# zzbuzzard/PATHS

Hardware: AMD Instinct MI355X
Metric: slides_per_sec_5level_K2048_D1024 (higher is better)
Workload: dtype f32 (products as 2 fp16 planes per operand = 22 bits, 3 fp16 MFMAs per block, fp32 accumulate); 1 GPU; 5-level PATHS recursion (forward, eval): K=2048 patches/level (level-0 grid 32x64, top_k 512, 10% background), D=1024 features, trans_dim 128 x 4 heads x 2 layers, LSTM ctx 256; 8 HBM-resident slides per GPU; slides_per_gpu=8, global_batch=8, levels=5, resident_batches_rotated=3, parallelism=slide-sharded x1 (no data-path collective)

## Files before the change

### include/paths_hip.h

```cpp
#ifndef PATHS_HIP_H
#define PATHS_HIP_H

#include <stddef.h>
#include <stdint.h>

#ifdef __cplusplus
extern "C" {
#endif

typedef void* paths_stream_t;

const char* paths_last_error(void);
const char* paths_build_info(void);
int paths_abi_version(void);

void* paths_event_create(void);
void* paths_stream_create_masked(const uint32_t* cu_mask, int words);
int paths_event_destroy(void* event);
int paths_stream_wait(paths_stream_t dst, paths_stream_t src, void* event);
int paths_set_stop_event(void* event);
int paths_flush_stop_event(paths_stream_t src);
int paths_stop_event_pending(void);
int paths_clear_stop_event(void);
int paths_record_event(void* event, paths_stream_t stream);
int paths_stream_wait_event(paths_stream_t dst, void* event);
int paths_memset_zero(void* p, size_t bytes, paths_stream_t stream);

int paths_lstm_cell(const float* x, int64_t ldx, const float* h0, int64_t ldh0, const float* c0, int64_t ldc0,
                    const float* w_gates, const float* b_gates, const float* w_mem, const float* b_mem,
                    float* state_out, int64_t ldso, float* y, int64_t ldy, float* ws_o, float* save_frm, float* save_tc,
                    const float* hp, const int* hp_row,
                    int M, int D, int Hc, const int64_t* num_ims, int rows_per_slide, int phases, paths_stream_t stream);

int paths_pe_table(const float* div_term, int pe_mode, int d, int rows, float* out, paths_stream_t stream);
int paths_importance_proj(const float* y, int64_t ldy, const float* w_ip, const float* b1, const float* w2, const float* b2 ,
                          const float* bp, const float* special, const float* div_term, const float* pe_table, int pe_rows,
                          const int64_t* locs,
                          const int64_t* num_ims, int rows_per_slide, int patch_size, int pe_mode, int imp_mul,
                          float* importance, float* tokens, float* save_hid, float* save_pproj, int M, int D, int Hi, int d,
                          int skip_padding, paths_stream_t stream);

int64_t paths_x6_packed_bytes(int Npad, int K, int planes);
int paths_x6_pack_weights(const float* w, int64_t ldw, void* out, int N, int Npad, int K, int planes, float w_scale,
                          paths_stream_t stream);
int paths_x6_pack_weights_t(const float* w, int64_t ldw, void* out, int N, int Npad, int K, int Kvalid, int planes, paths_stream_t stream);
int paths_lstm_cell_x6(const float* x, int64_t ldx, const int64_t* x_rows, const float* h0, int64_t ldh0, const float* c0, int64_t ldc0,
                       const void* w_gates_x6, const float* b_gates, const void* w_mem_x6, const float* b_mem,
                       float* state_out, int64_t ldso, float* y, int64_t ldy, float* ws_o, float* save_frm, float* save_tc,
                       const float* hp, const int* hp_row,
                       int M, int D, int Hc, const int64_t* num_ims, int rows_per_slide, int phases,
                       int planes, float wg_scale, float wm_scale, float a_scale, paths_stream_t stream);
int paths_lstm_cell_x6_h16(const float* x, int64_t ldx, const int64_t* x_rows, const float* h0, int64_t ldh0, const float* c0, int64_t ldc0,
                           const void* w_gates_x6, const float* b_gates, const void* w_mem_x6, const float* b_mem,
                           float* state_out, int64_t ldso, float* y, int64_t ldy, float* ws_o, float* save_frm, float* save_tc,
                           const float* hp, const int* hp_row,
                           int M, int D, int Hc, const int64_t* num_ims, int rows_per_slide, int phases,
                           int planes, float wg_scale, float wm_scale, float a_scale, paths_stream_t stream);
int paths_importance_proj_x6(const float* y, int64_t ldy, const int64_t* y_rows, const float* y_add, int64_t ldya, const void* w_ip_x6, const float* b1, const float* w2, const float* b2 ,
                             const float* bp, const float* special, const float* div_term, const float* pe_table, int pe_rows,
                             const int64_t* locs,
                             const int64_t* num_ims, int rows_per_slide, int patch_size, int pe_mode, int imp_mul,
                             float* importance, float* tokens, float* save_hid, float* save_pproj, int M, int D, int Hi, int d,
                             int skip_padding, int planes, float w_scale, float a_scale, float* splitk_ws, paths_stream_t stream);
int paths_importance_proj_x6_h16(const float* y, int64_t ldy, const int64_t* y_rows, const float* y_add, int64_t ldya, const void* w_ip_x6, const float* b1, const float* w2, const float* b2 ,
                                 const float* bp, const float* special, const float* div_term, const float* pe_table, int pe_rows,
                                 const int64_t* locs,
                                 const int64_t* num_ims, int rows_per_slide, int patch_size, int pe_mode, int imp_mul,
                                 float* importance, float* tokens, float* save_hid, float* save_pproj, int M, int D, int Hi, int d,
                                 int skip_padding, int planes, float w_scale, float a_scale, float* splitk_ws, paths_stream_t stream);
int64_t paths_importance_proj_x6_workspace(int M);
int paths_importance_qkv_x6(const float* y, int64_t ldy, const int64_t* y_rows, const float* y_add, int64_t ldya, const void* w_ip_x6,
                            const float* b1, const float* w2, const float* b2 , const float* bp, const float* special,
                            const float* pe_table, int pe_rows, const int64_t* locs, const int64_t* num_ims, int B, int N,
                            int patch_size, int pe_mode, int imp_mul, float* importance, float* tokens, int D, int skip_padding,
                            float w_scale, float a_scale, float* splitk_ws, const void* w_qkv, const float* bqkv, float s_wqkv,
                            float qscale, void* qkv_images, int phases, int alpha_from_importance, paths_stream_t stream);
int paths_importance_qkv_x6_h16(const float* y, int64_t ldy, const int64_t* y_rows, const float* y_add, int64_t ldya, const void* w_ip_x6,
                                const float* b1, const float* w2, const float* b2 , const float* bp, const float* special,
                                const float* pe_table, int pe_rows, const int64_t* locs, const int64_t* num_ims, int B, int N,
                                int patch_size, int pe_mode, int imp_mul, float* importance, float* tokens, int D, int skip_padding,
                                float w_scale, float a_scale, float* splitk_ws, const void* w_qkv, const float* bqkv, float s_wqkv,
                                float qscale, void* qkv_images, int phases, int alpha_from_importance, paths_stream_t stream);
int paths_gemm_nt_x6(const float* a, int64_t lda, const void* w_x6, int Kpacked, int k0, const float* b, float* out, int64_t ldo,
                     int M, int N, int Npad, int K, int act, const float* residual, int64_t ldr, const float* mask,
                     int64_t ldm, int accumulate, int planes, float w_scale, float a_scale, paths_stream_t stream);
int paths_gemm_add_nt_x6(const float* a, int64_t lda, const int64_t* a_rows, const float* a_add, int64_t ld_add, const void* w_x6, int Kpacked,
                         const float* b, float* out, int64_t ldo, int M, int N, int Npad, int K, int act, const int64_t* num_ims,
                         int rows_per_slide, float w_scale, float a_scale, paths_stream_t stream);
int paths_gemm_add_nt_x6_h16(const float* a, int64_t lda, const int64_t* a_rows, const float* a_add, int64_t ld_add, const void* w_x6, int Kpacked,
                             const float* b, float* out, int64_t ldo, int M, int N, int Npad, int K, int act, const int64_t* num_ims,
                             int rows_per_slide, float w_scale, float a_scale, paths_stream_t stream);
int paths_gemm_rows_nt_x6(const int64_t* a_rows, const void* w_x6, int Kpacked, int k0, float* out, int64_t ldo,
                          int M, int Npad, int K, int planes, float w_scale, float a_scale, paths_stream_t stream);

int paths_gemm_nt_f32(const float* a, int64_t lda, const float* w, int64_t ldw, const float* b, float* out, int64_t ldo,
                      int M, int N, int Npad, int K, int act, const float* residual, int64_t ldr, const float* mask,
                      int64_t ldm, int accumulate, paths_stream_t stream);
int64_t paths_gemm_tn_workspace(int N1, int N2, int splits);
int paths_gemm_tn_f32(const float* a, int64_t lda, const float* b0, int64_t ldb0, int nb0, const float* b1, int64_t ldb1,
                      float* out, int64_t ldo, int M, int N1, int N2, int splits, int accumulate, float* workspace,
                      paths_stream_t stream);
int paths_gemm_tn_x6(const float* a, int64_t lda, const float* b0, int64_t ldb0, int nb0, const float* b1, int64_t ldb1,
                     float* out, int64_t ldo, int M, int N1, int N2, int splits, int accumulate, float* workspace, int planes,
                     paths_stream_t stream);
int paths_colsum_f32(const float* a, int64_t lda, int M, int N, float* out, int splits, int accumulate, float* workspace,
                     paths_stream_t stream);
int paths_transpose_f32(const float* in, int64_t ldi, int R, int C, float* out, int64_t ldo, paths_stream_t stream);

int paths_adamw_chunk(void);
int paths_adamw_multi(const int64_t* table, const int64_t* numel, const int32_t* blocks, int nblocks, const float* step_size,
                      const float* bc2_sqrt, float wd_scale, int has_wd, float lerp_w, float beta2, float value, float eps, int flavor,
                      paths_stream_t stream);

int paths_lstm_bwd_a(const float* dh1, int64_t ldd, const float* dh1b, int64_t lddb, const float* o, const float* tc,
                     const int64_t* num_ims, int rows_per_slide, int64_t M, int D, float* dpre_o, int64_t ldo,
                     float* dpre_h, paths_stream_t stream);
int paths_lstm_bwd_b(const float* dc1_h, const float* dc1_ext, int64_t lde, const float* frm, const float* c0, int64_t ldc0,
                     const int64_t* num_ims, int rows_per_slide, int64_t M, int Hc, float* dg, int64_t ldg, float* dc0,
                     int64_t lddc0, paths_stream_t stream);
int paths_importance_bwd(const float* dtok, const float* pproj, const float* hid, const float* alpha, const float* w2,
                         const int64_t* num_ims, int rows_per_slide, int64_t M, int imp_mul, float* du, float* da, float* dah,
                         paths_stream_t stream);
int paths_layernorm_fwd_stats(const float* x, const float* add, const float* gamma, const float* beta, float* y, float* xhat,
                              float* rstd, int64_t rows, int d, float eps, paths_stream_t stream);
int paths_layernorm_bwd(const float* dy, const float* xhat, const float* rstd, const float* gamma, float* dx, float* dyxhat,
                        int64_t rows, int d, paths_stream_t stream);
int paths_layernorm_bwd_sums(const float* dy, const float* xhat, const float* rstd, const float* gamma, float* dx, float* slabs,
                             int64_t rows, int d, int rows_per_block, paths_stream_t stream);
int paths_reduce_slabs_f32(const float* slabs, int splits, int n, float* out, int accumulate, paths_stream_t stream);
int paths_defer_reductions(int on);
int paths_flush_reductions(int* n_entries, paths_stream_t stream);

int paths_attention_bwd_f32(const float* q, const float* k, const float* v, const float* o, const float* d_o, const float* lse,
                            const int64_t* num_ims, float* dqkv, float* ws_dsum, int B, int T, int H, int head_dim,
                            paths_stream_t stream);
int64_t paths_attention_token0_workspace(int B, int T, int H);
int paths_attention_token0_any(const float* qkv, int64_t ld, const int64_t* num_ims, float* a0, float* ws, int B, int T, int H, int head_dim,
                               float qscale, paths_stream_t stream);
int paths_attention_token0_fwd(const float* q, const float* k, const float* v, const int64_t* num_ims, float* a0, float* lse0, float* ws,
                               int B, int T, int H, int head_dim, uint64_t drop_key, float drop_p, paths_stream_t stream);
int paths_attention_token0_bwd(const float* q, const float* k, const float* v, const float* a0, const float* da0, const float* lse0,
                               const int64_t* num_ims, float* dqkv, float* ws, int B, int T, int H, int head_dim, uint64_t drop_key,
                               float drop_p, paths_stream_t stream);
int64_t paths_token0_attention_workspace(int B, int T, int d, int H);
int paths_token0_attention(const float* x, const int64_t* num_ims, const float* in_proj_weight, const float* in_proj_bias, float* attn_patch,
                           int64_t patch_ld, float* attn_self, int64_t self_ld, float* ws, int B, int T, int d, int H, int special_last,
                           paths_stream_t stream);
int64_t paths_attention_rollout_workspace(int B, int T, int d, int H);
int paths_attention_rollout_prepare(const float* x, const int64_t* num_ims, const float* in_proj_weight, const float* in_proj_bias, float* ws,
                                    int B, int T, int d, int H, int special_last, paths_stream_t stream);
int paths_attention_rollout_seed(const float* attn_patch, int64_t patch_ld, const float* attn_self, int64_t self_ld, const int64_t* num_ims,
                                 float* r, float* rollout, int64_t rollout_ld, float* rollout_self, int B, int T, int H, paths_stream_t stream);
int paths_attention_rollout_step(const float* ws, const int64_t* num_ims, const float* r_in, float* r_out, float* rollout, int64_t rollout_ld,
                                 float* rollout_self, int B, int T, int d, int H, paths_stream_t stream);

int paths_linear_f32(const float* a, int64_t lda, const float* w, const float* b, float* out, int64_t ldo,
                     int M, int N, int Npad, int K, int act, paths_stream_t stream);

int paths_attention_f32(const float* q, const float* k, const float* v, float* o, float* lse, const int64_t* num_ims,
                        int B, int T, int H, int head_dim, int max_queries, paths_stream_t stream);

int64_t paths_attention_x6_workspace(int B, int T, int H, int head_dim, int planes);
int paths_attention_x6(const float* q, const float* k, const float* v, float* o, float* lse, const int64_t* num_ims,
                       int B, int T, int H, int head_dim, int max_queries, void* workspace, int planes, int images_ready,
                       paths_stream_t stream);

int paths_token_layer_f32(const float* x_in, const float* attn, float* x_out,
                          const float* wo, const float* bo, const float* ln1g, const float* ln1b, const float* cab,
                          const float* ln2g, const float* ln2b, const float* w1, const float* b1, const float* w2,
                          const float* b2, const float* ln3g, const float* ln3b, const float* wqkv, const float* bqkv,
                          float* q, float* k, float* v, const int64_t* num_ims, int B, int T, int d, int H,
                          int do_post, int do_qkv, int skip_padding, float qscale, float eps, int max_tokens,
                          paths_stream_t stream);

int64_t paths_tlayer_h3_image_bytes(int part);
int paths_tlayer_pack_h3(int part, const float* wa, const float* wb, const float* wc, float s_a, float s_b, float s_c, void* out,
                         paths_stream_t stream);
int paths_token_layer_h3(const float* x_in, const float* attn, float* x_out, const void* w_post, const void* w_qkv,
                         const float* bo, const float* ln1g, const float* ln1b, const float* cab, const float* ln2g, const float* ln2b,
                         const float* b1, const float* b2, const float* ln3g, const float* ln3b, const float* bqkv,
                         float s_wo, float s_w1, float s_w2, float s_wqkv,
                         float* q, float* k, float* v, const int64_t* num_ims, int B, int T, int d, int H,
                         int do_post, int do_qkv, int skip_padding, float qscale, float eps, int max_tokens, void* qkv_images,
                         paths_stream_t stream);

int64_t paths_tlayer_ws_image_bytes(int part, int d);
int paths_tlayer_pack_ws(int part, const float* wa, const float* wb, const float* wc, float s_a, float s_b, float s_c, void* out, int d,
                         paths_stream_t stream);
int paths_token_layer_ws(const float* x_in, const float* attn, const void* attn_img, float* x_out, const void* w_post, const void* w_qkv,
                         const float* bo, const float* ln1g, const float* ln1b, const float* cab, const float* ln2g, const float* ln2b,
                         const float* b1, const float* b2, const float* ln3g, const float* ln3b, const float* bqkv,
                         float s_wo, float s_w1, float s_w2, float s_wqkv, void* qkv_images, const int64_t* num_ims,
                         int B, int T, int d, int H, int do_post, int do_qkv, int skip_padding, float qscale, float eps,
                         int* zero_words, int n_zero, paths_stream_t stream);
int paths_token_layer_ws_rows(const float* x_in, const float* attn, float* x_out, const void* w_post, const void* w_qkv,
                              const float* bo, const float* ln1g, const float* ln1b, const float* cab, const float* ln2g, const float* ln2b,
                              const float* b1, const float* b2, const float* ln3g, const float* ln3b, const float* bqkv,
                              float s_wo, float s_w1, float s_w2, float s_wqkv, float* qkv_rows, int64_t ld_qkv, const int64_t* num_ims,
                              int B, int T, int d, int do_post, int do_qkv, int skip_padding, float eps, paths_stream_t stream);
int paths_attention_h3_img(void* o_img, const int64_t* num_ims, int B, int T, int H, int head_dim, void* workspace, paths_stream_t stream);

int64_t paths_token0_ws_image_bytes(void);
int64_t paths_token0_ws_image_bytes_d(int d);
int64_t paths_token0_ws_partials(int B, int T);
int64_t paths_token0_ws_partials_d(int B, int T, int d);
int paths_token0_ws_supported(int B, int T, int d, int H);
int paths_token0_pack_ws(const float* wqkv, const float* bqkv, const float* wo, const float* bo, const float* w1, const float* w2, float qscale,
                         void* out, paths_stream_t stream);
int paths_token0_pack_ws_d(const float* wqkv, const float* bqkv, const float* wo, const float* bo, const float* w1, const float* w2, float qscale,
                           int d, void* out, paths_stream_t stream);
int paths_token0_tail_ws(const float* x1, const int64_t* num_ims, const void* img, const float* bv, const float* bo,
                         const float* ln1g, const float* ln1b, const float* cab, const float* ln2g, const float* ln2b,
                         const float* b1, const float* b2, const float* ln3g, const float* ln3b, const float* lnfg, const float* lnfb,
                         const float* ctx_prev, int64_t ctx_stride, const float* ctx_all, int ctx_depth,
                         const float* wcls, const float* bcls, int num_logits, int cls_in,
                         float* ctx_out, float* logits, float* partials, int* counters, int* status, int B, int T, int d, int H,
                         float eps, float eps_final, int special_last , paths_stream_t stream);

int paths_attention_any(const float* qkv, int64_t ld, float* o, const int64_t* num_ims, int B, int T, int H, int head_dim, float qscale,
                        int max_queries, paths_stream_t stream);
int64_t paths_attention_h3_any_workspace(int B, int T, int H, int head_dim);
int paths_attention_h3_any(const float* qkv, int64_t ld, float* o, const int64_t* num_ims, int B, int T, int H, int head_dim, float qscale,
                           void* workspace, paths_stream_t stream);
int paths_attention_h3_any_img(float* o, const int64_t* num_ims, int B, int T, int H, int head_dim, void* workspace, paths_stream_t stream);
int paths_layernorm_rows(const float* x, int64_t ldx, const float* add, const float* gamma, const float* beta, float* y, int64_t ldy,
                         int64_t rows, int d, float eps, paths_stream_t stream);
int paths_layernorm2_rows(const float* x, int64_t ldx, const float* g1, const float* b1, const float* add, const float* g2, const float* b2,
                          float* y, int64_t ldy, int64_t rows, int d, float eps, paths_stream_t stream);
int paths_importance_rows(const float* hid, int64_t ldh, const float* w2, const float* b2, const int64_t* num_ims, int rows_per_slide,
                          int64_t M, int Hi, float* importance, int relu , paths_stream_t stream);
int paths_tokens_assemble(const float* P, int64_t ldp, const float* importance, int imp_mul, const float* bp, const float* special,
                          const float* div_term, const int64_t* locs, int rows_per_slide, int patch_size, int pe_mode, int d, int B,
                          float* tokens, paths_stream_t stream);
int paths_importance_tokens_rows(const float* hid, int64_t ldh, const float* w2, const float* b2, const int64_t* num_ims, int rows_per_slide,
                                 int64_t M, int Hi, float* importance, int relu, int imp_mul, const float* bp, const float* special,
                                 const float* pe_table, int pe_rows, const int64_t* locs, int patch_size, int pe_mode, int d, float* tokens,
                                 paths_stream_t stream);
int paths_final_head_any(const float* x, int64_t slide_stride, const float* lng, const float* lnb, const float* ctx_prev, int64_t ctx_stride,
                         const float* ctx_all, int ctx_depth, const float* wcls, const float* bcls, int num_logits, int cls_in,
                         float* ctx_out, float* logits, int B, int d, float eps, paths_stream_t stream);

int paths_attention_any_train(const float* qkv, int64_t ld, float* o, float* lse, const int64_t* num_ims, int B, int T, int H, int head_dim,
                              float qscale, int max_queries, uint64_t drop_key, float drop_p, paths_stream_t stream);
int paths_attention_bwd_any(const float* qkv, int64_t ld, const float* o, const float* d_o, const float* lse, const int64_t* num_ims,
                            float* dqkv, float* ws_dsum, int B, int T, int H, int head_dim, float qscale, int max_queries,
                            uint64_t drop_key, float drop_p, paths_stream_t stream);
// ... 168 lines not shown
```

### paths_amd/_lib.py

```python
from __future__ import annotations

import ctypes as C
import os
from typing import Optional

import torch

_HERE = os.path.dirname(os.path.abspath(__file__))
LIB_PATH = os.environ.get("PATHS_HIP_LIB") or os.path.join(_HERE, "libpaths_hip.so")

_i64, _i32, _f32, _vp, _u32, _u64 = C.c_int64, C.c_int, C.c_float, C.c_void_p, C.c_uint32, C.c_uint64

SIGNATURES = {
    "paths_lstm_cell": [_vp, _i64, _vp, _i64, _vp, _i64, _vp, _vp, _vp, _vp, _vp, _i64, _vp, _i64, _vp, _vp, _vp, _vp, _vp,
                        _i32, _i32, _i32, _vp, _i32, _i32, _vp],
    "paths_pe_table": [_vp, _i32, _i32, _i32, _vp, _vp],
    "paths_importance_proj": [_vp, _i64, _vp, _vp, _vp, _vp, _vp, _vp, _vp, _vp, _i32, _vp, _vp, _i32, _i32, _i32, _i32,
                              _vp, _vp, _vp, _vp, _i32, _i32, _i32, _i32, _i32, _vp],
    "paths_gemm_nt_f32": [_vp, _i64, _vp, _i64, _vp, _vp, _i64, _i32, _i32, _i32, _i32, _i32, _vp, _i64, _vp, _i64, _i32, _vp],
    "paths_x6_pack_weights": [_vp, _i64, _vp, _i32, _i32, _i32, _i32, _f32, _vp],
    "paths_x6_pack_weights_t": [_vp, _i64, _vp, _i32, _i32, _i32, _i32, _i32, _vp],
    "paths_lstm_cell_x6": [_vp, _i64, _vp, _vp, _i64, _vp, _i64, _vp, _vp, _vp, _vp, _vp, _i64, _vp, _i64, _vp, _vp, _vp, _vp, _vp,
                           _i32, _i32, _i32, _vp, _i32, _i32, _i32, _f32, _f32, _f32, _vp],
    "paths_importance_proj_x6": [_vp, _i64, _vp, _vp, _i64, _vp, _vp, _vp, _vp, _vp, _vp, _vp, _vp, _i32, _vp, _vp, _i32, _i32, _i32, _i32,
                                 _vp, _vp, _vp, _vp, _i32, _i32, _i32, _i32, _i32, _i32, _f32, _f32, _vp, _vp],
    "paths_importance_qkv_x6": [_vp, _i64, _vp, _vp, _i64, _vp, _vp, _vp, _vp, _vp, _vp, _vp, _i32, _vp, _vp, _i32, _i32, _i32, _i32, _i32,
                                _vp, _vp, _i32, _i32, _f32, _f32, _vp, _vp, _vp, _f32, _f32, _vp, _i32, _i32, _vp],
    "paths_gemm_nt_x6": [_vp, _i64, _vp, _i32, _i32, _vp, _vp, _i64, _i32, _i32, _i32, _i32, _i32, _vp, _i64, _vp, _i64, _i32,
                         _i32, _f32, _f32, _vp],
    "paths_gemm_add_nt_x6": [_vp, _i64, _vp, _vp, _i64, _vp, _i32, _vp, _vp, _i64, _i32, _i32, _i32, _i32, _i32, _vp, _i32, _f32, _f32, _vp],
    "paths_gemm_tn_f32": [_vp, _i64, _vp, _i64, _i32, _vp, _i64, _vp, _i64, _i32, _i32, _i32, _i32, _i32, _vp, _vp],
    "paths_attention_fp8": [_vp, _vp, _vp, _vp, _vp, _i32, _i32, _i32, _i32, _vp, _vp],
    "paths_gemm_tn_x6": [_vp, _i64, _vp, _i64, _i32, _vp, _i64, _vp, _i64, _i32, _i32, _i32, _i32, _i32, _vp, _i32, _vp],
    "paths_colsum_f32": [_vp, _i64, _i32, _i32, _vp, _i32, _i32, _vp, _vp],
    "paths_transpose_f32": [_vp, _i64, _i32, _i32, _vp, _i64, _vp],
    "paths_attention_wide_fwd": [_vp, _i64, _vp, _vp, _vp, _i32, _i32, _i32, _i32, _f32, _i32, _u64, _f32, _vp, _vp],
    "paths_attention_wide_bwd": [_vp, _i64, _vp, _vp, _vp, _vp, _vp, _i32, _i32, _i32, _i32, _f32, _i32, _u64, _f32, _vp, _vp],
    "paths_sibling_sum": [_vp, _i64, _vp, _vp, _vp, _i64, _i64, _i32, _vp, _i64, _i64, _i32, _vp],
    "paths_scatter_kept_rows": [_vp, _i64, _i64, _vp, _vp, _vp, _i64, _i64, _i32, _i32, _vp],
    "paths_adamw_multi": [_vp, _vp, _vp, _i32, _vp, _vp, _f32, _i32, _f32, _f32, _f32, _f32, _i32, _vp],
    "paths_lstm_bwd_a": [_vp, _i64, _vp, _i64, _vp, _vp, _vp, _i32, _i64, _i32, _vp, _i64, _vp, _vp],
    "paths_lstm_bwd_b": [_vp, _vp, _i64, _vp, _vp, _i64, _vp, _i32, _i64, _i32, _vp, _i64, _vp, _i64, _vp],
    "paths_importance_bwd": [_vp, _vp, _vp, _vp, _vp, _vp, _i32, _i64, _i32, _vp, _vp, _vp, _vp],
    "paths_layernorm_fwd_stats": [_vp, _vp, _vp, _vp, _vp, _vp, _vp, _i64, _i32, _f32, _vp],
    "paths_attention_bwd_f32": [_vp, _vp, _vp, _vp, _vp, _vp, _vp, _vp, _vp, _i32, _i32, _i32, _i32, _vp],
    "paths_attention_token0_any": [_vp, _i64, _vp, _vp, _vp, _i32, _i32, _i32, _i32, _f32, _vp],
    "paths_attention_token0_fwd": [_vp, _vp, _vp, _vp, _vp, _vp, _vp, _i32, _i32, _i32, _i32, _u64, _f32, _vp],
    "paths_attention_token0_bwd": [_vp, _vp, _vp, _vp, _vp, _vp, _vp, _vp, _vp, _i32, _i32, _i32, _i32, _u64, _f32, _vp],
    "paths_token0_attention": [_vp, _vp, _vp, _vp, _vp, _i64, _vp, _i64, _vp, _i32, _i32, _i32, _i32, _i32, _vp],
    "paths_attention_rollout_prepare": [_vp, _vp, _vp, _vp, _vp, _i32, _i32, _i32, _i32, _i32, _vp],
    "paths_attention_rollout_seed": [_vp, _i64, _vp, _i64, _vp, _vp, _vp, _i64, _vp, _i32, _i32, _i32, _vp],
    "paths_attention_rollout_step": [_vp, _vp, _vp, _vp, _vp, _i64, _vp, _i32, _i32, _i32, _i32, _vp],
    "paths_layernorm_bwd": [_vp, _vp, _vp, _vp, _vp, _vp, _i64, _i32, _vp],
    "paths_layernorm_bwd_sums": [_vp, _vp, _vp, _vp, _vp, _vp, _i64, _i32, _i32, _vp],
    "paths_reduce_slabs_f32": [_vp, _i32, _i32, _vp, _i32, _vp],
    "paths_defer_reductions": [_i32],
    "paths_flush_reductions": [_vp, _vp],
    "paths_linear_f32": [_vp, _i64, _vp, _vp, _vp, _i64, _i32, _i32, _i32, _i32, _i32, _vp],
    "paths_attention_f32": [_vp, _vp, _vp, _vp, _vp, _vp, _i32, _i32, _i32, _i32, _i32, _vp],
    "paths_attention_x6": [_vp, _vp, _vp, _vp, _vp, _vp, _i32, _i32, _i32, _i32, _i32, _vp, _i32, _i32, _vp],
    "paths_tlayer_pack_h3": [_i32, _vp, _vp, _vp, _f32, _f32, _f32, _vp, _vp],
    "paths_token_layer_h3": [_vp] * 16 + [_f32, _f32, _f32, _f32, _vp, _vp, _vp, _vp, _i32, _i32, _i32, _i32, _i32, _i32, _i32, _f32, _f32, _i32, _vp, _vp],
    "paths_tlayer_pack_ws": [_i32, _vp, _vp, _vp, _f32, _f32, _f32, _vp, _i32, _vp],
    "paths_token_layer_ws": [_vp] * 17 + [_f32, _f32, _f32, _f32, _vp, _vp, _i32, _i32, _i32, _i32, _i32, _i32, _i32, _f32, _f32, _vp, _i32, _vp],
    "paths_token_layer_ws_rows": [_vp] * 16 + [_f32, _f32, _f32, _f32, _vp, _i64, _vp, _i32, _i32, _i32, _i32, _i32, _i32, _f32, _vp],
    "paths_token0_pack_ws": [_vp, _vp, _vp, _vp, _vp, _vp, _f32, _vp, _vp],
    "paths_token0_pack_ws_d": [_vp, _vp, _vp, _vp, _vp, _vp, _f32, _i32, _vp, _vp],
    "paths_token0_tail_ws": [_vp] * 16 + [_vp, _i64, _vp, _i32, _vp, _vp, _i32, _i32, _vp, _vp, _vp, _vp, _vp, _i32, _i32, _i32, _i32, _f32, _f32, _i32, _vp],
    "paths_attention_any": [_vp, _i64, _vp, _vp, _i32, _i32, _i32, _i32, _f32, _i32, _vp],
    "paths_attention_any_train": [_vp, _i64, _vp, _vp, _vp, _i32, _i32, _i32, _i32, _f32, _i32, _u64, _f32, _vp],
    "paths_layernorm_fwd_stats_any": [_vp, _vp, _vp, _vp, _vp, _vp, _vp, _i64, _i32, _f32, _vp],
    "paths_layernorm_bwd_any": [_vp, _vp, _vp, _vp, _vp, _vp, _i64, _i32, _vp],
    "paths_layernorm_bwd_sums_any": [_vp, _vp, _vp, _vp, _vp, _vp, _i64, _i32, _i32, _vp],
    "paths_importance_bwd_any": [_vp, _vp, _vp, _vp, _vp, _vp, _i32, _i64, _i32, _i32, _i32, _i64, _vp, _vp, _vp, _vp],
    "paths_importance_rows_bwd_any": [_vp, _vp, _i32, _vp, _vp, _vp, _vp, _i32, _i64, _i32, _vp, _vp, _vp, _vp],
    "paths_attention_bwd_any": [_vp, _i64, _vp, _vp, _vp, _vp, _vp, _vp, _i32, _i32, _i32, _i32, _f32, _i32, _u64, _f32, _vp],
    "paths_fp8_scale": [_vp, _i64, _i64, _i32, _vp, _vp, _vp, _i32, _vp],
    "paths_fp8_pack_weight": [_vp, _i64, _i32, _i32, _vp, _vp, _vp, _vp],
    "paths_fp8_quantize": [_vp, _i64, _i32, _i32, _vp, _vp, _vp],
    "paths_gemm_nt_fp8_out8": [_vp, _vp, _vp, _vp, _vp, _vp, _vp, _vp, _i32, _i32, _i32, _i32, _vp],
    "paths_gemm_nt_fp8": [_vp, _vp, _vp, _vp, _vp, _vp, _i64, _i32, _i32, _i32, _i32, _vp, _i64, _vp],
    "paths_attention_fp8_qkv": [_vp, _i64, _vp, _vp, _i32, _i32, _i32, _i32, _f32, _vp, _vp],
    "paths_attention_h3_any": [_vp, _i64, _vp, _vp, _i32, _i32, _i32, _i32, _f32, _vp, _vp],
    "paths_attention_h3_any_img": [_vp, _vp, _i32, _i32, _i32, _i32, _vp, _vp],
    "paths_layernorm_rows": [_vp, _i64, _vp, _vp, _vp, _vp, _i64, _i64, _i32, _f32, _vp],
    "paths_layernorm2_rows": [_vp, _i64, _vp, _vp, _vp, _vp, _vp, _vp, _i64, _i64, _i32, _f32, _vp],
    "paths_importance_rows": [_vp, _i64, _vp, _vp, _vp, _i32, _i64, _i32, _vp, _i32, _vp],
    "paths_importance_tokens_rows": [_vp, _i64, _vp, _vp, _vp, _i32, _i64, _i32, _vp, _i32, _i32, _vp, _vp, _vp, _i32, _vp, _i32, _i32, _i32, _vp, _vp],
    "paths_tokens_assemble": [_vp, _i64, _vp, _i32, _vp, _vp, _vp, _vp, _i32, _i32, _i32, _i32, _i32, _vp, _vp],
    "paths_final_head_any": [_vp, _i64, _vp, _vp, _vp, _i64, _vp, _i32, _vp, _vp, _i32, _i32, _vp, _vp, _i32, _i32, _f32, _vp],
    "paths_attention_h3_img": [_vp, _vp, _i32, _i32, _i32, _i32, _vp, _vp],
    "paths_token_layer_f32": [_vp] * 21 + [_vp, _i32, _i32, _i32, _i32, _i32, _i32, _i32, _f32, _f32, _i32, _vp],
    "paths_token0_tail": [_vp] * 20 + [_vp, _i64, _vp, _i32, _vp, _vp, _i32, _i32, _vp, _vp, _vp, _i32, _i32, _i32, _i32, _f32, _f32, _vp],
    "paths_final_head": [_vp, _i64, _vp, _vp, _vp, _i64, _vp, _i32, _vp, _vp, _i32, _i32, _vp, _vp, _i32, _i32, _f32, _vp],
    "paths_layernorm_f32": [_vp, _vp, _vp, _vp, _i64, _i32, _f32, _vp],
    "paths_topk": [_vp, _i64, _vp, _i32, _i32, _i32, _vp, _i64, _vp, _vp],
    "paths_topk_rows": [_vp, _i64, _vp, _i32, _i32, _i32, _vp, _i64, _vp, _vp, _i64, _i64, _vp, _vp, _vp],
    "paths_gemm_rows_nt_x6": [_vp, _vp, _i32, _i32, _vp, _i64, _i32, _i32, _i32, _i32, _f32, _f32, _vp],
    "paths_expand_children": [_vp, _i64, _vp, _vp, _i64, _i32, _vp, _vp, _vp, _i32, _i64, _vp, _vp, _vp, _vp, _vp, _vp, _vp, _vp, _vp],
    "paths_candidate_children": [_vp, _i64, _vp, _vp, _i64, _i32, _vp, _vp, _i32, _vp, _vp, _vp, _vp],
    "paths_admit_children": [_vp, _vp, _vp, _vp, _vp, _i64, _vp, _i32, _i32, _i64, _vp, _vp, _vp, _vp, _vp, _vp, _vp, _vp, _vp],
    "paths_gather_kept_rows": [_vp, _i64, _i64, _vp, _i64, _vp, _i32, _i32, _vp, _vp],
    "paths_gather_rows_bwd": [_vp, _i64, _vp, _vp, _vp, _i64, _i32, _vp, _i64, _i32, _vp],
    "paths_fallback_all_cells": [_vp, _vp, _vp, _i32, _i32, _i64, _vp, _vp, _vp, _vp, _vp, _vp, _vp, _vp],
    "paths_gather_rows": [_vp, _vp, _i32, _vp, _i64, _i64, _vp, _i32, _vp, _i32, _i64, _vp, _vp, _i32, _vp, _vp, _vp],
    "paths_level0_batch": [_vp, _vp, _vp, _i32, _i32, _i32, _i64, _vp, _vp, _vp, _vp, _i32, _vp, _vp, _vp],
    "paths_scale_add_rows": [_vp, _vp, _vp, _vp, _i32, _i32, _i64, _i32, _vp, _vp],
    "paths_importance_rows_bwd": [_vp, _vp, _i32, _vp, _vp, _vp, _vp, _i32, _i64, _vp, _vp, _vp, _vp],
    "paths_dropout_rows": [_vp, _i64, _vp, _vp, _i64, _vp, _i64, _i64, _i32, _u64, _f32, _vp],
    "paths_dropout_mask": [_vp, _i64, _u64, _f32, _vp],
    "paths_attention_x6_dropout": [_vp, _vp, _vp, _vp, _vp, _vp, _i32, _i32, _i32, _i32, _i32, _vp, _i32, _u64, _f32, _vp],
    "paths_attention_bwd_f32_dropout": [_vp, _vp, _vp, _vp, _vp, _vp, _vp, _vp, _vp, _i32, _i32, _i32, _i32, _u64, _f32, _vp],
    "paths_attention_bwd_x6_dropout": [_vp, _vp, _vp, _vp, _vp, _vp, _vp, _vp, _vp, _vp, _i32, _i32, _i32, _i32, _u64, _f32, _vp],
    "paths_attention_bwd_x6_planes": [_vp, _vp, _vp, _vp, _vp, _vp, _vp, _vp, _vp, _vp, _i32, _i32, _i32, _i32, _u64, _f32, _i32, _vp],
    "paths_stream_wait": [_vp, _vp, _vp],
    "paths_set_stop_event": [_vp],
    "paths_flush_stop_event": [_vp],
    "paths_stream_wait_event": [_vp, _vp],
    "paths_record_event": [_vp, _vp],
    "paths_event_destroy": [_vp],
    "paths_memset_zero": [_vp, C.c_size_t, _vp],
    "paths_tissue_mask": [_vp, _i64, _i32, _vp, _vp],
    "paths_tissue_mask_absmax": [_vp, _i64, _i32, _vp, _vp, _vp],
    "paths_synth_grid": [_vp, _i32, _i32, _i32, _u32, _i32, _u64, _vp],
    "paths_stage_rows": [_vp, _i64, _i32, _vp, _vp, _vp],
    "paths_saliency_rows": [_vp, _i64, _vp, _i64, _vp, _i32, _i32, _i32, _vp, _vp, _vp],
    "paths_path_points": [_vp, _i64, _vp, _vp, _vp, _vp, _vp, _i32, _i32, _i32, _i32, _vp, _vp],
    "paths_path_accumulate": [_vp, _i64, _vp, _i64, _vp, _vp, _vp, _i32, _i32, _i32, _i32, _i32, _vp, _vp, _vp, _vp],
    "paths_rank_joint": [_vp, _vp, _vp, _vp, _i32, _i32, _i32, _i32, _vp, _vp, _vp],
    "paths_path_mask_points": [_vp, _i64, _vp, _vp, _i64, _vp, _vp, _vp, _i32, _i32, _i32, _i32, _vp, _vp],
    "paths_removal_masks": [_vp, _vp, _vp, _i64, _vp, _i32, _vp, _vp, _i64, _vp, _i32, _i32, _i32, _i32, _vp, _i64, _vp, _vp],
    "paths_visited_overlap": [_vp, _i64, _vp, _vp, _vp, _vp, _i32, _i32, _i32, _i32, _vp, _vp],
    "paths_level0_mask_rows": [_vp, _vp, _vp, _i32, _i32, _i64, _vp, _vp, _vp, _vp],
}
for _n in ("paths_lstm_cell_x6", "paths_importance_proj_x6", "paths_importance_qkv_x6", "paths_gemm_add_nt_x6", "paths_gather_rows",
           "paths_level0_batch", "paths_tissue_mask_absmax", "paths_synth_grid"):
    SIGNATURES[_n + "_h16"] = SIGNATURES[_n]
_PLAIN = {"paths_gemm_tn_workspace": (C.c_int64, [_i32, _i32, _i32]), "paths_x6_packed_bytes": (C.c_int64, [_i32, _i32, _i32]), "paths_tlayer_h3_image_bytes": (C.c_int64, [_i32]), "paths_tlayer_ws_image_bytes": (C.c_int64, [_i32, _i32]), "paths_token0_ws_image_bytes": (C.c_int64, []), "paths_token0_ws_partials": (C.c_int64, [_i32, _i32]), "paths_token0_ws_image_bytes_d": (C.c_int64, [_i32]), "paths_token0_ws_partials_d": (C.c_int64, [_i32, _i32, _i32]), "paths_token0_ws_supported": (_i32, [_i32, _i32, _i32, _i32]), "paths_attention_x6_workspace": (C.c_int64, [_i32, _i32, _i32, _i32, _i32]), "paths_attention_fp8_workspace": (C.c_int64, [_i32, _i32, _i32, _i32]), "paths_attention_bwd_x6_workspace": (C.c_int64, [_i32, _i32, _i32, _i32]), "paths_attention_token0_workspace": (C.c_int64, [_i32, _i32, _i32]), "paths_token0_attention_workspace": (C.c_int64, [_i32, _i32, _i32, _i32]), "paths_attention_rollout_workspace": (C.c_int64, [_i32, _i32, _i32, _i32]), "paths_attention_h3_any_workspace": (C.c_int64, [_i32, _i32, _i32, _i32]), "paths_importance_proj_x6_workspace": (C.c_int64, [_i32]), "paths_last_error": (C.c_char_p, []), "paths_build_info": (C.c_char_p, []), "paths_abi_version": (_i32, []), "paths_stop_event_pending": (_i32, []), "paths_clear_stop_event": (_i32, []), "paths_adamw_chunk": (_i32, []), "paths_rank_joint_tile": (_i32, []), "paths_attention_wide_workspace": (C.c_int64, [_i32, _i32]), "paths_event_create": (_vp, []), "paths_stream_create_masked": (_vp, [_vp, _i32])}

ABI_VERSION = 3
_lib: Optional[C.CDLL] = None


class PathsHipError(RuntimeError):
    pass


def load() -> C.CDLL:
    global _lib
    if _lib is None:
        if not os.path.isfile(LIB_PATH):
            raise PathsHipError(f"{LIB_PATH} not found: the HIP extension is not built (run __graft_entry__.build()); "
                                "paths_amd has no CPU fallback")
        lib = C.CDLL(LIB_PATH)
        lib.paths_abi_version.restype = _i32
        if lib.paths_abi_version() != ABI_VERSION:
            raise PathsHipError(f"{LIB_PATH} has ABI version {lib.paths_abi_version()}, this binding needs {ABI_VERSION}: rebuild it "
                                "(__graft_entry__.build())")
        for name, args in SIGNATURES.items():
            fn = getattr(lib, name)
            fn.argtypes, fn.restype = args, _i32
        for name, (res, args) in _PLAIN.items():
            fn = getattr(lib, name)
            fn.argtypes, fn.restype = args, res
        _lib = lib
    return _lib


def ptr(t):
    if t is None or type(t) is int:
        return t
    return t.data_ptr()


_RAW_STREAM = getattr(torch._C, "_cuda_getCurrentRawStream", None)
_GET_DEVICE = getattr(torch._C, "_cuda_getDevice", None)


def stream() -> int:
    if _RAW_STREAM is not None and _GET_DEVICE is not None:
        return _RAW_STREAM(_GET_DEVICE())
    return torch.cuda.current_stream().cuda_stream


TAPE = None
TAPE_EVENTS = None


def call(name: str, *args):
    lib = load()
    fn = getattr(lib, name)
    rc = fn(*args)
    if rc != 0:
        raise PathsHipError(f"{name} failed ({rc}): {lib.paths_last_error().decode()}")
    if TAPE is not None:
        TAPE.append((fn, args, name))
        fb = fork_behind.active
        if fb is not None and fb.taken_at is None and name != "paths_set_stop_event" and not lib.paths_stop_event_pending():
            fb.taken_at = len(TAPE) - 1


def stream_wait(dst: "torch.cuda.Stream", src: "torch.cuda.Stream"):
    dst.wait_stream(src)
    if TAPE is not None:
        lib = load()
        pool = TAPE_EVENTS if TAPE_EVENTS is not None else [[], 0]
        if pool[1] == len(pool[0]):
            ev = lib.paths_event_create()
            if not ev:
                raise PathsHipError("paths_event_create failed")
            pool[0].append(ev)
        ev = pool[0][pool[1]]
        pool[1] += 1
        TAPE.append((lib.paths_stream_wait, (dst.cuda_stream, src.cuda_stream, ev), "paths_stream_wait"))


STOP_EVENTS = __import__("os").environ.get("PATHS_STOP_EVENTS", "1") != "0"


_TAPE_PLUMBING = {"paths_set_stop_event", "paths_flush_stop_event", "paths_stream_wait_event", "paths_stream_wait", "paths_record_event",
                  "paths_clear_stop_event"}


class fork_behind:

    active = None

    def __init__(self, dsts, src):
        self.dsts, self.src = list(dsts), src
        self.ev = None
        self.taken_at = None

    def __enter__(self):
        if TAPE is not None and STOP_EVENTS:
            lib = load()
            pool = TAPE_EVENTS if TAPE_EVENTS is not None else [[], 0]
            if pool[1] == len(pool[0]):
                e = lib.paths_event_create()
                if not e:
                    raise PathsHipError("paths_event_create failed")
                pool[0].append(e)
            self.ev = pool[0][pool[1]]
            pool[1] += 1
            call("paths_set_stop_event", self.ev)
            self.prev, fork_behind.active = fork_behind.active, self
        return self

    def __exit__(self, et, ev, tb):
        if self.ev is not None:
            fork_behind.active = self.prev
            if et is not None:
                load().paths_clear_stop_event()
                return False
            call("paths_flush_stop_event", self.src.cuda_stream)
            if self.taken_at is not None and any(nm not in _TAPE_PLUMBING for _, _, nm in TAPE[self.taken_at + 1:]):
                call("paths_record_event", self.ev, self.src.cuda_stream)
            for d in self.dsts:
                call("paths_stream_wait_event", d.cuda_stream, self.ev)
        elif et is None:
            for d in self.dsts:
                stream_wait(d, self.src)
        return False


def zeros(shape, **kw) -> torch.Tensor:
    t = torch.zeros(shape, **kw)
    if TAPE is not None:
        TAPE.append((load().paths_memset_zero, (t.data_ptr(), t.numel() * t.element_size(), stream()), "paths_memset_zero"))
    return t


def require_cuda(*tensors: torch.Tensor):
    for t in tensors:
        if t is not None and not t.is_cuda:
            raise PathsHipError("paths_amd runs on the GPU only: got a CPU tensor (no CPU fallback)")


def float_from_bits(bits: int) -> float:
    import struct
    bits &= 0xFFFFFFFF
    return float("inf") if bits >= 0x7F800000 else struct.unpack("<f", struct.pack("<I", bits))[0]


def absmax(t: torch.Tensor) -> float:
    require_cuda(t)
    assert t.dtype == torch.float32 and t.is_contiguous() and t.numel() % 4 == 0
    bits = torch.zeros((1,), dtype=torch.int32, device=t.device)
    D = t.shape[-1] if (t.dim() > 1 and t.shape[-1] % 4 == 0) else 4
# ... 3 lines not shown
```

### paths_amd/csrc/gemm_epi.h

```cpp
#pragma once
#include "common.h"

namespace paths_epi {



struct TileView {
  char* base; int64_t ldb; uint32_t lane_off;
  __device__ TileView(const float* p, int64_t ld, int lane)
      : base(reinterpret_cast<char*>(const_cast<float*>(p))), ldb(ld * 4), lane_off((uint32_t)((4 * (lane >> 5)) * ld + (lane & 31)) * 4u) {}
  __device__ float* at(int trow, int tcol, int r) const {
    char* tile = base + (int64_t)trow * ldb + (int64_t)tcol * 4;
    const uint32_t off = lane_off + (uint32_t)((r & 3) + 8 * (r >> 2)) * (uint32_t)ldb;
    return reinterpret_cast<float*>(tile + off);
  }
  __device__ char* tile(int trow, int tcol) const { return base + (int64_t)trow * ldb + (int64_t)tcol * 4; }
  __device__ float* elem(char* tile_origin, int r) const {
    return reinterpret_cast<float*>(tile_origin + (lane_off + (uint32_t)((r & 3) + 8 * (r >> 2)) * (uint32_t)ldb));
  }
  __device__ float* at_clamped(int trow, int tcol, int r, int lane, int M) const {
    const int row = min(trow + c32_row(r, lane), M - 1);
    return reinterpret_cast<float*>(base + (int64_t)row * ldb + (int64_t)(tcol + (lane & 31)) * 4);
  }
};
template <bool FULL>
__device__ __forceinline__ float* tile_elem(const TileView& v, int trow, int tcol, int r, int lane, int M) {
  if constexpr (FULL) return v.at(trow, tcol, r);
  else return v.at_clamped(trow, tcol, r, lane, M);
}
template <bool FULL>
__device__ __forceinline__ float* tile_elem_o(const TileView& v, char* origin, int trow, int tcol, int r, int lane, int M) {
  if constexpr (FULL) return v.elem(origin, r);
  else return v.at_clamped(trow, tcol, r, lane, M);
}
template <bool FULL>
__device__ __forceinline__ bool tile_row_ok(int trow, int r, int lane, int M) {
  if constexpr (FULL) return true;
  else return trow + c32_row(r, lane) < M;
}

struct EpiLstmC {
  const float* bias;
  const float* c0; int64_t ldc0;
  float* c1; int64_t ldc1;
  float* frm; int64_t ldfrm;
  const float* hp; int64_t ldhp; const int* hp_row;
  float acc_scale = 1.0f;
  template <int WTM, int WTN>
  __device__ __forceinline__ void init(f32x16 (&acc)[WTM][WTN], int row0, int col0, int lane, int M) const {
    const int jj = lane & 31;
    const float seed = 1.0f / acc_scale;
    if (hp == nullptr) {
#pragma unroll
      for (int i = 0; i < WTM; ++i)
#pragma unroll
        for (int r = 0; r < 16; ++r) { acc[i][0][r] = 0.f; acc[i][1][r] = 0.f; acc[i][2][r] = 0.f; }
      return;
    }
    int pr[WTM][16];
#pragma unroll
    for (int i = 0; i < WTM; ++i)
#pragma unroll
      for (int r = 0; r < 16; ++r) pr[i][r] = hp_row[min(row0 + 32 * i + c32_row(r, lane), M - 1)];
    float t[2][3][16];
    auto issue = [&](auto ic) __attribute__((always_inline)) {
      constexpr int i = decltype(ic)::value;
#pragma unroll
      for (int r = 0; r < 16; ++r) {
        const float* ph = hp + (int64_t)max(pr[i][r], 0) * ldhp + col0 + jj;
        t[i & 1][0][r] = ph[0]; t[i & 1][1][r] = ph[32]; t[i & 1][2][r] = ph[64];
      }
    };
    issue(std::integral_constant<int, 0>{});
    static_for<0, WTM>([&](auto ic) __attribute__((always_inline)) {
      constexpr int i = decltype(ic)::value;
      __builtin_amdgcn_sched_barrier(0);
      if constexpr (i + 1 < WTM) issue(std::integral_constant<int, i + 1>{});
      __builtin_amdgcn_sched_barrier(0);
#pragma unroll
      for (int r = 0; r < 16; ++r) {
        const bool has = pr[i][r] >= 0;
        acc[i][0][r] = has ? t[i & 1][0][r] * seed : 0.f; acc[i][1][r] = has ? t[i & 1][1][r] * seed : 0.f; acc[i][2][r] = has ? t[i & 1][2][r] * seed : 0.f;
      }
    });
    __builtin_amdgcn_sched_barrier(0);
  }
  template <bool FULL, bool WITH_FRM, int WTM, int WTN>
  __device__ __forceinline__ void run_impl(f32x16 (&acc)[WTM][WTN], int row0, int col0, int lane, int M) const {
    const int jj = lane & 31;
    const int tcol = (col0 / 96) * 32;
    const float bf = bias[col0 + jj], br = bias[col0 + 32 + jj], bm = bias[col0 + 64 + jj];
    const TileView c0v(c0, ldc0, lane), c1v(c1, ldc1, lane), fv(frm, ldfrm, lane);
    static_for<0, WTM>([&](auto ic) __attribute__((always_inline)) {
      constexpr int i = decltype(ic)::value;
      const int trow = row0 + 32 * i;
      char* o0 = c0v.tile(trow, tcol); char* o1 = c1v.tile(trow, tcol); char* of = fv.tile(trow, col0);
      float cp[16];
#pragma unroll
      for (int r = 0; r < 16; ++r) cp[r] = c0 ? *tile_elem_o<FULL>(c0v, o0, trow, tcol, r, lane, M) : 0.f;
#pragma unroll
      for (int r = 0; r < 16; ++r) {
        const float f = sigmoid_acc(fmaf(acc[i][0][r], acc_scale, bf));
        const float rg = sigmoid_acc(fmaf(acc[i][1][r], acc_scale, br));
        const float mp = tanh_acc(fmaf(acc[i][2][r], acc_scale, bm));
        const float v = cp[r] * f + rg * mp;
        if (tile_row_ok<FULL>(trow, r, lane, M)) {
          *tile_elem_o<FULL>(c1v, o1, trow, tcol, r, lane, M) = v;
          if constexpr (WITH_FRM) {
            float* fr = tile_elem_o<FULL>(fv, of, trow, col0, r, lane, M);
            fr[0] = f; fr[32] = rg; fr[64] = mp;
          }
        }
      }
      __builtin_amdgcn_sched_barrier(0);
    });
  }
  template <int WTM, int WTN, int WGM, int WGN>
  __device__ __forceinline__ void run(f32x16 (&acc)[WTM][WTN], int row0, int col0, int lane, int, int, int M, float*) const {
    static_assert(WTN == 3, "LSTM c epilogue wants f|r|m tiles");
    const bool full = row0 + 32 * WTM <= M;
    if (frm == nullptr) {
      if (full) run_impl<true, false>(acc, row0, col0, lane, M);
      else run_impl<false, false>(acc, row0, col0, lane, M);
    } else {
      if (full) run_impl<true, true>(acc, row0, col0, lane, M);
      else run_impl<false, true>(acc, row0, col0, lane, M);
    }
  }
};

template <bool RAW>
struct EpiLstmO_ {
  const float* bias; float* o; int64_t ldo; int N;
  const float* hp; int64_t ldhp; const int* hp_row; int hp_col0;
  float acc_scale = 1.0f;
  template <int WTM, int WTN>
  __device__ __forceinline__ void init(f32x16 (&acc)[WTM][WTN], int row0, int col0, int lane, int M) const {
    const float seed = 1.0f / acc_scale;
    if (hp == nullptr) {
#pragma unroll
      for (int i = 0; i < WTM; ++i)
#pragma unroll
        for (int j = 0; j < WTN; ++j)
#pragma unroll
          for (int r = 0; r < 16; ++r) acc[i][j][r] = 0.f;
      return;
    }
    int pr[WTM][16];
#pragma unroll
    for (int i = 0; i < WTM; ++i)
#pragma unroll
      for (int r = 0; r < 16; ++r) pr[i][r] = hp_row[min(row0 + 32 * i + c32_row(r, lane), M - 1)];
    float t[2][WTN][16];
    auto issue = [&](auto ic) __attribute__((always_inline)) {
      constexpr int i = decltype(ic)::value;
#pragma unroll
      for (int r = 0; r < 16; ++r) {
        const float* ph = hp + (int64_t)max(pr[i][r], 0) * ldhp + hp_col0 + (lane & 31);
#pragma unroll
        for (int j = 0; j < WTN; ++j) t[i & 1][j][r] = ph[min(col0 + 32 * j, N - 32)];
      }
    };
    issue(std::integral_constant<int, 0>{});
    static_for<0, WTM>([&](auto ic) __attribute__((always_inline)) {
      constexpr int i = decltype(ic)::value;
      __builtin_amdgcn_sched_barrier(0);
      if constexpr (i + 1 < WTM) issue(std::integral_constant<int, i + 1>{});
      __builtin_amdgcn_sched_barrier(0);
#pragma unroll
      for (int r = 0; r < 16; ++r)
#pragma unroll
        for (int j = 0; j < WTN; ++j) acc[i][j][r] = pr[i][r] >= 0 ? t[i & 1][j][r] * seed : 0.f;
    });
    __builtin_amdgcn_sched_barrier(0);
  }
  template <bool FULL, int WTM, int WTN>
  __device__ __forceinline__ void run_impl(f32x16 (&acc)[WTM][WTN], int row0, int col0, int lane, int M) const {
    const TileView ov(o, ldo, lane);
    static_for<0, WTM * WTN>([&](auto tc) __attribute__((always_inline)) {
      constexpr int t = decltype(tc)::value, i = t % WTM, j = t / WTM;
      const int trow = row0 + 32 * i, tcol = col0 + 32 * j;
      if (tcol < N) {
        const float b = bias[tcol + (lane & 31)];
        char* origin = ov.tile(trow, tcol);
#pragma unroll
        for (int r = 0; r < 16; ++r) {
          const float v = sigmoid_acc(fmaf(acc[i][j][r], acc_scale, b));
          if (tile_row_ok<FULL>(trow, r, lane, M)) *tile_elem_o<FULL>(ov, origin, trow, tcol, r, lane, M) = v;
        }
      }
    });
  }
  template <int WTM, int WTN, int WGM, int WGN>
  __device__ __forceinline__ void run(f32x16 (&acc)[WTM][WTN], int row0, int col0, int lane, int, int, int M, float*) const {
    if constexpr (RAW) {
      const int ntn = N >> 5;
#pragma unroll
      for (int j = 0; j < WTN; ++j) {
        const int tcol = col0 + 32 * j;
        if (tcol < N) {
          const float b = bias[tcol + (lane & 31)];
#pragma unroll
          for (int i = 0; i < WTM; ++i) {
            f32x4* t = reinterpret_cast<f32x4*>(o + ((int64_t)((row0 >> 5) + i) * ntn + (tcol >> 5)) * 1024) + lane;
#pragma unroll
            for (int q = 0; q < 4; ++q)
              t[64 * q] = f32x4{fmaf(acc[i][j][4 * q], acc_scale, b), fmaf(acc[i][j][4 * q + 1], acc_scale, b),
                                fmaf(acc[i][j][4 * q + 2], acc_scale, b), fmaf(acc[i][j][4 * q + 3], acc_scale, b)};
          }
        }
      }
    } else {
      if (row0 + 32 * WTM <= M) run_impl<true>(acc, row0, col0, lane, M);
      else run_impl<false>(acc, row0, col0, lane, M);
    }
  }
};
typedef EpiLstmO_<false> EpiLstmO;
typedef EpiLstmO_<true> EpiLstmORaw;

template <bool WITH_Y, bool WITH_TC = false, bool RAW_O = false>
struct EpiLstmH {
  template <int WTM, int WTN>
  __device__ __forceinline__ void init(f32x16 (&acc)[WTM][WTN], int, int, int, int) const {
#pragma unroll
    for (int i = 0; i < WTM; ++i)
#pragma unroll
      for (int j = 0; j < WTN; ++j)
#pragma unroll
        for (int r = 0; r < 16; ++r) acc[i][j][r] = 0.f;
  }

  const float* bias; const float* o; int64_t ldo; const float* x; int64_t ldx;
  float* h1; int64_t ldh; float* y; int64_t ldy; int N;
  float* tc_out;
  float acc_scale = 1.0f;
  template <bool FULL, int WTM, int WTN>
  __device__ __forceinline__ void run_impl(f32x16 (&acc)[WTM][WTN], int row0, int col0, int lane, int M) const {
    constexpr int NT = WTM * WTN, PD = (NT >= 4 && !WITH_Y) ? 3 : 1, NB = PD + 1;
    const TileView ovw(o, ldo, lane), xvw(x, ldx, lane), hv(h1, ldh, lane), yv(y, ldy, lane), tv(tc_out, N, lane);
    float ov[NB][16], xv[WITH_Y ? NB : 1][16];
    auto load = [&](auto tc) __attribute__((always_inline)) {
      constexpr int t = decltype(tc)::value, i = t % WTM, j = t / WTM, s = t % NB;
      const int trow = row0 + 32 * i, tcol = min(col0 + 32 * j, N - 32);
      char* to = ovw.tile(trow, tcol); char* tx = xvw.tile(trow, tcol);
      if constexpr (RAW_O) {
        const f32x4* t4 = reinterpret_cast<const f32x4*>(o + ((int64_t)(trow >> 5) * (N >> 5) + (tcol >> 5)) * 1024) + lane;
#pragma unroll
        for (int q = 0; q < 4; ++q) {
          const f32x4 v = t4[64 * q];
          ov[s][4 * q] = v[0]; ov[s][4 * q + 1] = v[1]; ov[s][4 * q + 2] = v[2]; ov[s][4 * q + 3] = v[3];
        }
      }
      static_for<0, 16>([&](auto rc) __attribute__((always_inline)) {
        constexpr int r = decltype(rc)::value;
        if constexpr (FULL) {
          if constexpr (!RAW_O) ov[s][r] = *ovw.elem(to, r);
          if constexpr (WITH_Y) xv[s][r] = *xvw.elem(tx, r);
        } else {
          if constexpr (!RAW_O) ov[s][r] = *ovw.at_clamped(trow, tcol, r, lane, M);
          if constexpr (WITH_Y) xv[s][r] = *xvw.at_clamped(trow, tcol, r, lane, M);
        }
      });
    };
    static_for<0, (PD < NT ? PD : NT)>([&](auto tc) __attribute__((always_inline)) { load(tc); });
    static_for<0, NT>([&](auto tc) __attribute__((always_inline)) {
      constexpr int t = decltype(tc)::value, i = t % WTM, j = t / WTM, s = t % NB;
      if constexpr (t + PD < NT) load(std::integral_constant<int, t + PD>{});
      const int trow = row0 + 32 * i, tcol = col0 + 32 * j;
      if (tcol < N) {
        const float b = bias[tcol + (lane & 31)];
        char* th = hv.tile(trow, tcol); char* ty = yv.tile(trow, tcol); char* tt = tv.tile(trow, tcol);
        static_for<0, 16>([&](auto rc) __attribute__((always_inline)) {
          constexpr int r = decltype(rc)::value;
          const float tcv = tanh_acc(fmaf(acc[i][j][r], acc_scale, b));
          const float h = (RAW_O ? sigmoid_acc(ov[s][r]) : ov[s][r]) * tcv;
          if constexpr (FULL) {
            if constexpr (WITH_TC) *tv.elem(tt, r) = tcv;
            *hv.elem(th, r) = h;
            if constexpr (WITH_Y) *yv.elem(ty, r) = xv[s][r] + h;
          } else if (tile_row_ok<false>(trow, r, lane, M)) {
            if constexpr (WITH_TC) *tv.at_clamped(trow, tcol, r, lane, M) = tcv;
            *hv.at_clamped(trow, tcol, r, lane, M) = h;
            if constexpr (WITH_Y) *yv.at_clamped(trow, tcol, r, lane, M) = xv[s][r] + h;
          }
        });
      }
      __builtin_amdgcn_sched_barrier(0);
    });
  }
  template <int WTM, int WTN, int WGM, int WGN>
  __device__ __forceinline__ void run(f32x16 (&acc)[WTM][WTN], int row0, int col0, int lane, int, int, int M, float*) const {
    if (row0 + 32 * WTM <= M) run_impl<true>(acc, row0, col0, lane, M);
    else run_impl<false>(acc, row0, col0, lane, M);
  }
};

struct EpiBias {
// ... 240 lines not shown
```

### paths_amd/csrc/gemm_x6.hip

```cpp
#include "common.h"
#include "gemm_epi.h"
#include "finish_qkv.h"
#include "split.h"

#ifndef PATHS_X6_PART
#define PATHS_X6_PART 0
#endif

namespace {
using namespace paths_epi;

constexpr int FRAG = 1024;
template <int NP> constexpr int planes_of() { return NP == 4 ? 2 : NP; }
template <int NP> constexpr int subt() { return planes_of<NP>() * FRAG; }

struct X6Operands {
  const float* A0; int64_t lda0; int K0;
  const int64_t* A0rows;
  const float* A1; int64_t lda1; int K1;
  const float* Aadd; int64_t ldadd;
  const char* Wt;
  int64_t w_group_stride;
  int M;
  const int64_t* num_ims;
// ... 341 lines not shown
  const int64_t i = blockIdx.x * (int64_t)blockDim.x + threadIdx.x;
  if (i >= (int64_t)Npad * (K >> 3)) return;
  const int n = (int)(i % Npad), k0 = (int)(i / Npad) * 8;
  uint16_t h[8], m[8], l[8];
#pragma unroll
  for (int j = 0; j < 8; ++j) {
    const int k = k0 + j;
    const float v = (n < N && k < Kvalid) ? w[(int64_t)k * ldw + n] : 0.f;
    const __bf16 hh = (__bf16)v; const float r1 = v - (float)hh;
    const __bf16 mm = (__bf16)r1; const float r2 = r1 - (float)mm;
    const __bf16 ll = (__bf16)r2;
    h[j] = __builtin_bit_cast(uint16_t, hh); m[j] = __builtin_bit_cast(uint16_t, mm); l[j] = __builtin_bit_cast(uint16_t, ll);
  }
  uint16_t* o = out + ((int64_t)(n >> 5) * (K >> 4) + (k0 >> 4)) * (subt<NP>() / 2) + ((k0 >> 3) & 1) * 256 + (n & 31) * 8;
  typedef uint16_t u16x8 __attribute__((ext_vector_type(8)));
  *reinterpret_cast<u16x8*>(o) = u16x8{h[0], h[1], h[2], h[3], h[4], h[5], h[6], h[7]};
  *reinterpret_cast<u16x8*>(o + FRAG / 2) = u16x8{m[0], m[1], m[2], m[3], m[4], m[5], m[6], m[7]};
  if constexpr (NP == 3) *reinterpret_cast<u16x8*>(o + FRAG) = u16x8{l[0], l[1], l[2], l[3], l[4], l[5], l[6], l[7]};
}

template <int NP, int WTM, int WTN, int PF, bool ADD, bool ROWS, class Epi, int OCC = 1, bool A16 = false>
int launch_x6_np(const X6Operands& g, int Npad, const Epi& epi, hipStream_t stream, const char* name) {
  constexpr int BM = WTM * 64, BN = WTN * 64;
  constexpr size_t lds = 2ull * (2 * WTM * ((A16 && !ADD) ? FRAG : subt<NP>()) + 2 * WTN * subt<NP>());
  const int K = g.K0 + g.K1;
  PATHS_REQUIRE(g.M > 0, "%s: M must be > 0", name);
  PATHS_REQUIRE(g.K0 > 0 && g.K0 % 16 == 0 && g.K1 % 16 == 0 && K % 32 == 0 && K >= 128, "%s: K panels (%d,%d): multiples of 16, total a multiple of 32, >= 128", name, g.K0, g.K1);
  PATHS_REQUIRE(Npad % BN == 0, "%s: packed N (%d) must be a multiple of %d", name, Npad, BN);
  PATHS_REQUIRE(g.lda0 % 4 == 0 && g.lda1 % 4 == 0, "%s: leading dims must be multiples of 4 floats", name);
  PATHS_REQUIRE(((uintptr_t)g.A0 % 16 == 0) && ((uintptr_t)g.A1 % 16 == 0) && ((uintptr_t)g.Wt % 16 == 0), "%s: operands must be 16-byte aligned", name);
  PATHS_REQUIRE(ROWS == (g.A0rows != nullptr) && (!ROWS || g.K1 == 0), "%s: row-pointer form is single-panel", name);
  PATHS_REQUIRE((int64_t)g.M * (g.lda0 > g.lda1 ? (g.lda0 > g.ldadd ? g.lda0 : g.ldadd) : (g.lda1 > g.ldadd ? g.lda1 : g.ldadd)) * 4 < (int64_t)1 << 32, "%s: A panel larger than 4 GiB", name);
  auto kern = gemm_x6_kernel<NP, WTM, WTN, PF, ADD, ROWS, Epi, OCC, A16>;
  PATHS_LDS_OPT_IN(kern, lds, name);
  PATHS_REQUIRE(g.ksplit == 1 || (g.ksplit > 1 && g.K1 == 0 && g.K0 % (32 * g.ksplit) == 0 && g.K0 / g.ksplit >= 128), "%s: split-K needs a single panel and k windows that are multiples of 32, >= 128", name);
  dim3 grid(Npad / BN, (g.M + BM - 1) / BM, g.ksplit);
  hipLaunchKernelGGL(kern, grid, dim3(256), lds, stream, g, epi);
  PATHS_LAUNCH_CHECK(name);
  return PATHS_OK;
}

struct EpiRaw {
  float* ws; int64_t zstride; int ntn;
  template <int WTM, int WTN>
  __device__ __forceinline__ void init(f32x16 (&acc)[WTM][WTN], int, int, int, int) const {
#pragma unroll
    for (int i = 0; i < WTM; ++i)
#pragma unroll
      for (int j = 0; j < WTN; ++j)
#pragma unroll
        for (int r = 0; r < 16; ++r) acc[i][j][r] = 0.f;
  }
  template <int WTM, int WTN, int WGM, int WGN>
  __device__ __forceinline__ void run(f32x16 (&acc)[WTM][WTN], int row0, int col0, int lane, int, int, int, float*) const {
    float* base = ws + (int64_t)blockIdx.z * zstride;
#pragma unroll
    for (int i = 0; i < WTM; ++i)
#pragma unroll
      for (int j = 0; j < WTN; ++j) {
        f32x4* t = reinterpret_cast<f32x4*>(base + ((int64_t)((row0 >> 5) + i) * ntn + (col0 >> 5) + j) * 1024) + lane;
#pragma unroll
        for (int q = 0; q < 4; ++q) {
          const f32x4 v = f32x4{acc[i][j][4 * q], acc[i][j][4 * q + 1], acc[i][j][4 * q + 2], acc[i][j][4 * q + 3]};
          t[64 * q] = v;
        }
      }
  }
};

template <int NZ, class Epi>
__global__ void __launch_bounds__(256)
x6_finish_kernel(const float* __restrict__ ws, int64_t zstride, int ntn, int M, const int64_t* __restrict__ num_ims, int rows_per_slide, Epi epi) {
  extern __shared__ __attribute__((aligned(16))) char smem[];
  const int tid = threadIdx.x, lane = tid & 63, wave = __builtin_amdgcn_readfirstlane(tid >> 6), wm = wave >> 1, wn = wave & 1;
  const int m0 = blockIdx.x * 64;
  if (block_all_padding(num_ims, rows_per_slide, m0, 64, M)) return;
  const int row0 = m0 + wm * 32, col0 = wn * 128;
  f32x16 acc[1][4];
#pragma unroll
  for (int j = 0; j < 4; ++j) {
    const f32x4* t = reinterpret_cast<const f32x4*>(ws + ((int64_t)(row0 >> 5) * ntn + (col0 >> 5) + j) * 1024) + lane;
#pragma unroll
    for (int q = 0; q < 4; ++q) {
      f32x4 v = t[64 * q];
#pragma unroll
      for (int z = 1; z < NZ; ++z) v += *reinterpret_cast<const f32x4*>(reinterpret_cast<const float*>(t + 64 * q) + z * zstride);
      acc[0][j][4 * q] = v[0]; acc[0][j][4 * q + 1] = v[1]; acc[0][j][4 * q + 2] = v[2]; acc[0][j][4 * q + 3] = v[3];
    }
  }
  epi.template run<1, 4, 2, 2>(acc, row0, col0, lane, wm, wn, M, reinterpret_cast<float*>(smem));
}

template <int WTM, int WTN, int PF, bool ADD, class Epi>
int launch_x6(int planes, const X6Operands& g, int Npad, const Epi& epi, hipStream_t stream, const char* name) {
  if (g.A0rows != nullptr) {
    if (planes == 2) return launch_x6_np<2, WTM, WTN, PF, ADD, true>(g, Npad, epi, stream, name);
    return paths_set_error(PATHS_EUNSUPPORTED, "%s: row pointers need planes = 2", name);
  }
  if constexpr (std::is_same<Epi, EpiBias>::value && !ADD) {
    if (planes == 4) return launch_x6_np<4, WTM, WTN, PF, ADD, false>(g, Npad, epi, stream, name);
  }
  if (planes == 3) return launch_x6_np<3, WTM, WTN, PF, ADD, false>(g, Npad, epi, stream, name);
  if (planes == 2) return launch_x6_np<2, WTM, WTN, PF, ADD, false>(g, Npad, epi, stream, name);
  return paths_set_error(PATHS_EINVAL, "%s: planes must be 3 (bf16 x6) or 2 (fp16 x3), got %d", name, planes);
}

constexpr int H_OCC = 3;
constexpr int H_TRAIN_OCC = 2;

inline int plane_count(int planes) { return planes == 4 ? 2 : planes; }
inline int64_t group_stride(int planes, int Kpacked) { return (int64_t)(Kpacked / 16) * plane_count(planes) * FRAG; }
inline bool pow2(float x) { int e; return x > 0.f && frexpf(x, &e) == 0.5f; }
inline bool h16_scale_ok(float a_scale) { return pow2(a_scale) && a_scale >= 1.0f && a_scale <= 32768.0f; }

}

extern "C" {

#if PATHS_X6_PART == 0 || PATHS_X6_PART == 1
int64_t paths_x6_packed_bytes(int Npad, int K, int planes) { return (int64_t)Npad * K * 2 * plane_count(planes); }

int paths_x6_pack_weights(const float* w, int64_t ldw, void* out, int N, int Npad, int K, int planes, float w_scale, hipStream_t stream) {
  PATHS_REQUIRE(N > 0 && Npad >= N && Npad % 32 == 0 && K % 16 == 0, "x6_pack_weights: bad shape N=%d Npad=%d K=%d", N, Npad, K);
  PATHS_REQUIRE((uintptr_t)out % 16 == 0, "x6_pack_weights: out must be 16-byte aligned");
  PATHS_REQUIRE(((planes == 3 || planes == 4) && w_scale == 1.0f) || (planes == 2 && pow2(w_scale)), "x6_pack_weights: planes 3 / 4 (bf16) with w_scale 1, or planes 2 with a power-of-two w_scale");
  const int64_t n = (int64_t)Npad * K;
  const dim3 grid((unsigned)((n + 255) / 256));
  if (planes == 4) hipLaunchKernelGGL(x6_pack_kernel<4>, grid, dim3(256), 0, stream, w, ldw, reinterpret_cast<uint16_t*>(out), N, Npad, K, 1.0f);
  else if (planes == 3) hipLaunchKernelGGL(x6_pack_kernel<3>, grid, dim3(256), 0, stream, w, ldw, reinterpret_cast<uint16_t*>(out), N, Npad, K, 1.0f);
  else hipLaunchKernelGGL(x6_pack_kernel<2>, grid, dim3(256), 0, stream, w, ldw, reinterpret_cast<uint16_t*>(out), N, Npad, K, w_scale);
  PATHS_LAUNCH_CHECK("x6_pack_weights");
  return PATHS_OK;
}

int paths_x6_pack_weights_t(const float* w, int64_t ldw, void* out, int N, int Npad, int K, int Kvalid, int planes, hipStream_t stream) {
  PATHS_REQUIRE(N > 0 && Npad >= N && Npad % 32 == 0 && K % 16 == 0 && Kvalid > 0 && Kvalid <= K, "x6_pack_weights_t: bad shape N=%d Npad=%d K=%d Kvalid=%d", N, Npad, K, Kvalid);
  PATHS_REQUIRE(w != nullptr && out != nullptr && (uintptr_t)out % 16 == 0, "x6_pack_weights_t: null / unaligned operand");
  PATHS_REQUIRE(planes == 3 || planes == 4, "x6_pack_weights_t: planes 3 or 4 (bf16)");
  const int64_t n = (int64_t)Npad * (K / 8);
  const dim3 grid((unsigned)((n + 255) / 256));
  if (planes == 4) hipLaunchKernelGGL(x6_pack_t_kernel<4>, grid, dim3(256), 0, stream, w, ldw, reinterpret_cast<uint16_t*>(out), N, Npad, K, Kvalid);
  else hipLaunchKernelGGL(x6_pack_t_kernel<3>, grid, dim3(256), 0, stream, w, ldw, reinterpret_cast<uint16_t*>(out), N, Npad, K, Kvalid);
  PATHS_LAUNCH_CHECK("x6_pack_weights_t");
  return PATHS_OK;
}

}
namespace {
template <bool A16>
int lstm_cell_x6(const float* x, int64_t ldx, const int64_t* x_rows, const float* h0, int64_t ldh0, const float* c0, int64_t ldc0,
                 const void* w_gates_x6, const float* b_gates, const void* w_mem_x6, const float* b_mem,
                 float* state_out, int64_t ldso, float* y, int64_t ldy, float* ws_o, float* save_frm, float* save_tc,
                 const float* hp, const int* hp_row, int M, int D, int Hc, const int64_t* num_ims, int rows_per_slide,
                 int phases, int planes, float wg_scale, float wm_scale, float a_scale, hipStream_t stream) {
  PATHS_REQUIRE(D % 256 == 0 && Hc % 64 == 0, "lstm_cell_x6: D (%d) must be a multiple of 256 and Hc (%d) of 64", D, Hc);
  if constexpr (A16) {
    PATHS_REQUIRE(x_rows != nullptr && x == nullptr && planes == 2, "lstm_cell_x6_h16: fp16 rows are given as x_rows (planes = 2)");
    PATHS_REQUIRE(h16_scale_ok(a_scale), "lstm_cell_x6_h16: a_scale must be a power of two in [1, 2^15]");
  }
  PATHS_REQUIRE(hp != nullptr || (h0 == nullptr) == (c0 == nullptr), "lstm_cell_x6: h0 and c0 must both be given or both be null");
  PATHS_REQUIRE((hp == nullptr) == (hp_row == nullptr) && (hp == nullptr || h0 == nullptr),
                "lstm_cell_x6: hp/hp_row come together and replace h0 (the h half of the gate GEMM was done per parent)");
  PATHS_REQUIRE(planes == 3 || (pow2(wg_scale) && pow2(wm_scale) && pow2(a_scale)), "lstm_cell_x6: scales must be powers of two");
  PATHS_REQUIRE(x_rows == nullptr || (h0 == nullptr && y == nullptr && save_tc == nullptr), "lstm_cell_x6: x_rows (rows addressed in place) excludes h0, y and the training saves");
  if (planes == 3) wg_scale = wm_scale = a_scale = 1.0f;
  const char* wg = reinterpret_cast<const char*>(w_gates_x6);
  const int64_t gs = group_stride(planes, 2 * D);
  const float sg = 1.0f / (wg_scale * a_scale), sm = 1.0f / (wm_scale * a_scale);
  X6Operands g{x, ldx, D, x_rows, h0, h0 ? ldh0 : 0, h0 ? D : 0, nullptr, 0, wg, gs, M, num_ims, rows_per_slide, a_scale};
  const bool small_m = planes == 2 && M <= 8192 && (h0 == nullptr);
  if (phases & 1) {
    EpiLstmC e{b_gates, c0, ldc0, state_out + D, ldso, save_frm, (int64_t)3 * Hc, hp, (int64_t)3 * Hc + D, hp_row, sg};
    int rc;
    if constexpr (A16) {
      rc = small_m ? launch_x6_np<2, 2, 3, 2, false, true, decltype(e), 1, true>(g, 3 * Hc, e, stream, "lstm_cell_x6_h16(c, 128-row tiles)")
                   : launch_x6_np<2, 4, 3, 1, false, true, decltype(e), 1, true>(g, 3 * Hc, e, stream, "lstm_cell_x6_h16(c)");
    } else if (small_m) rc = x_rows ? launch_x6_np<2, 2, 3, 2, false, true>(g, 3 * Hc, e, stream, "lstm_cell_x6(c, 128-row tiles)")
                             : launch_x6_np<2, 2, 3, 2, false, false>(g, 3 * Hc, e, stream, "lstm_cell_x6(c, 128-row tiles)");
    else rc = launch_x6<4, 3, 1, false>(planes, g, 3 * Hc, e, stream, "lstm_cell_x6(c)");
    if (rc) return rc;
  }
  const bool o_raw = y == nullptr && save_tc == nullptr && save_frm == nullptr;
  if (phases & 2) {
    X6Operands go = g;
    go.Wt = wg + (int64_t)(3 * Hc / 32) * gs;
    int rc;
    if (o_raw) {
      EpiLstmORaw e{b_gates + 3 * Hc, ws_o, D, D, hp, (int64_t)3 * Hc + D, hp_row, 3 * Hc, sg};
      if constexpr (A16) {
        rc = small_m ? launch_x6_np<2, 2, 4, 2, false, true, decltype(e), 1, true>(go, D, e, stream, "lstm_cell_x6_h16(o, raw, 128-row tiles)")
                     : launch_x6_np<2, 4, 4, 1, false, true, decltype(e), 1, true>(go, D, e, stream, "lstm_cell_x6_h16(o, raw)");
      } else if (small_m) rc = x_rows ? launch_x6_np<2, 2, 4, 2, false, true>(go, D, e, stream, "lstm_cell_x6(o, raw, 128-row tiles)")
                               : launch_x6_np<2, 2, 4, 2, false, false>(go, D, e, stream, "lstm_cell_x6(o, raw, 128-row tiles)");
      else rc = launch_x6<4, 4, 1, false>(planes, go, D, e, stream, "lstm_cell_x6(o, raw)");
    } else {
      EpiLstmO e{b_gates + 3 * Hc, ws_o, D, D, hp, (int64_t)3 * Hc + D, hp_row, 3 * Hc, sg};
      if constexpr (A16) rc = launch_x6_np<2, 4, 4, 1, false, true, decltype(e), 1, true>(go, D, e, stream, "lstm_cell_x6_h16(o)");
      else rc = launch_x6<4, 4, 1, false>(planes, go, D, e, stream, "lstm_cell_x6(o)");
    }
    if (rc) return rc;
  }
  if (phases & 4) {
    X6Operands gh{state_out + D, ldso, Hc, nullptr, nullptr, 0, 0, nullptr, 0, reinterpret_cast<const char*>(w_mem_x6), group_stride(planes, Hc), M, num_ims, rows_per_slide, a_scale};
    int rc;
    PATHS_REQUIRE(save_tc == nullptr || y != nullptr, "lstm_cell_x6: save_tc (training) needs y");
    PATHS_REQUIRE(planes == 2 || planes == 3, "lstm_cell_x6: planes must be 3 (bf16 x6) or 2 (fp16 x3), got %d", planes);
    if (save_tc != nullptr) {
      EpiLstmH<true, true> e{b_mem, ws_o, D, x, ldx, state_out, ldso, y, ldy, D, save_tc, sm};
      if (planes == 2) rc = launch_x6_np<2, 2, 2, 2, false, false, decltype(e), H_TRAIN_OCC>(gh, D, e, stream, "lstm_cell_x6(h, save, 128x128)");
      else rc = launch_x6_np<3, 4, 4, 1, false, false>(gh, D, e, stream, "lstm_cell_x6(h, save)");
    } else if (y != nullptr) {
      EpiLstmH<true, false> e{b_mem, ws_o, D, x, ldx, state_out, ldso, y, ldy, D, nullptr, sm};
      rc = launch_x6<4, 4, 1, false>(planes, gh, D, e, stream, "lstm_cell_x6(h)");
    } else if (o_raw) {
      EpiLstmH<false, false, true> e{b_mem, ws_o, D, x, ldx, state_out, ldso, nullptr, 0, D, nullptr, sm};
      if (planes == 2) rc = launch_x6_np<2, 2, 2, 2, false, false, decltype(e), H_OCC>(gh, D, e, stream, "lstm_cell_x6(h, raw o, 128x128)");
      else rc = launch_x6_np<3, 4, 4, 1, false, false>(gh, D, e, stream, "lstm_cell_x6(h, raw o)");
    } else {
      EpiLstmH<false, false> e{b_mem, ws_o, D, x, ldx, state_out, ldso, nullptr, 0, D, nullptr, sm};
      if (planes == 2) rc = launch_x6_np<2, 2, 2, 2, false, false, decltype(e), H_OCC>(gh, D, e, stream, "lstm_cell_x6(h, no y, 128x128)");
      else rc = launch_x6_np<3, 4, 4, 1, false, false>(gh, D, e, stream, "lstm_cell_x6(h, no y)");
    }
    if (rc) return rc;
  }
  return PATHS_OK;
}
}
extern "C" {

int paths_lstm_cell_x6(const float* x, int64_t ldx, const int64_t* x_rows, const float* h0, int64_t ldh0, const float* c0, int64_t ldc0,
                       const void* w_gates_x6, const float* b_gates, const void* w_mem_x6, const float* b_mem,
                       float* state_out, int64_t ldso, float* y, int64_t ldy, float* ws_o, float* save_frm, float* save_tc,
                       const float* hp, const int* hp_row, int M, int D, int Hc, const int64_t* num_ims, int rows_per_slide,
                       int phases, int planes, float wg_scale, float wm_scale, float a_scale, hipStream_t stream) {
  return lstm_cell_x6<false>(x, ldx, x_rows, h0, ldh0, c0, ldc0, w_gates_x6, b_gates, w_mem_x6, b_mem, state_out, ldso, y, ldy, ws_o, save_frm,
                             save_tc, hp, hp_row, M, D, Hc, num_ims, rows_per_slide, phases, planes, wg_scale, wm_scale, a_scale, stream);
}

int paths_lstm_cell_x6_h16(const float* x, int64_t ldx, const int64_t* x_rows, const float* h0, int64_t ldh0, const float* c0, int64_t ldc0,
                           const void* w_gates_x6, const float* b_gates, const void* w_mem_x6, const float* b_mem,
                           float* state_out, int64_t ldso, float* y, int64_t ldy, float* ws_o, float* save_frm, float* save_tc,
                           const float* hp, const int* hp_row, int M, int D, int Hc, const int64_t* num_ims, int rows_per_slide,
                           int phases, int planes, float wg_scale, float wm_scale, float a_scale, hipStream_t stream) {
  return lstm_cell_x6<true>(x, ldx, x_rows, h0, ldh0, c0, ldc0, w_gates_x6, b_gates, w_mem_x6, b_mem, state_out, ldso, y, ldy, ws_o, save_frm,
                            save_tc, hp, hp_row, M, D, Hc, num_ims, rows_per_slide, phases, planes, wg_scale, wm_scale, a_scale, stream);
}

#endif
#if PATHS_X6_PART == 0 || PATHS_X6_PART == 2
int64_t paths_importance_proj_x6_workspace(int M) { return 2ll * ((M + 127) / 128 * 4) * 8 * 1024 * 4; }

}
namespace {
template <bool A16>
int importance_proj_x6(const float* y, int64_t ldy, const int64_t* y_rows, const float* y_add, int64_t ldya, const void* w_ip_x6, const float* b1, const float* w2, const float* b2,
                       const float* bp, const float* special, const float* div_term, const float* pe_table, int pe_rows, const int64_t* locs,
                       const int64_t* num_ims, int rows_per_slide, int patch_size, int pe_mode, int imp_mul,
                       float* importance, float* tokens, float* save_hid, float* save_pproj, int M, int D, int Hi, int d,
                       int skip_padding, int planes, float w_scale, float a_scale, float* splitk_ws, hipStream_t stream) {
  if constexpr (A16) {
    PATHS_REQUIRE(y == nullptr && y_rows != nullptr && y_add != nullptr && splitk_ws != nullptr && planes == 2 && D % 64 == 0 && D >= 256,
                  "importance_proj_x6_h16: fp16 rows (y_rows) + y_add on the split-K form (splitk_ws, planes = 2, D %% 64 == 0, D >= 256)");
  }
  PATHS_REQUIRE(Hi == 128 && d == 128, "importance_proj_x6: this build supports importance_mlp_hidden_dim=128, trans_dim=128 (got %d, %d)", Hi, d);
  PATHS_REQUIRE(pe_mode == 1 || pe_mode == 2, "importance_proj_x6: pe_mode must be 1 (1d) or 2 (2d)");
  PATHS_REQUIRE(pe_mode == 1 || locs != nullptr, "importance_proj_x6: 2d positional encoding needs locs");
  PATHS_REQUIRE(num_ims != nullptr && rows_per_slide > 0 && M % rows_per_slide == 0, "importance_proj_x6: bad slide layout");
  PATHS_REQUIRE(b1 != nullptr && w2 != nullptr && b2 != nullptr, "importance_proj_x6: b1, w2 and b2 (device scalar) are required");
  PATHS_REQUIRE(y_add == nullptr || (ldya % 4 == 0 && (uintptr_t)y_add % 16 == 0), "importance_proj_x6: y_add must be 16-byte aligned with ldya %% 4 == 0");
  PATHS_REQUIRE(planes == 3 || (pow2(w_scale) && pow2(a_scale)), "importance_proj_x6: scales must be powers of two");
  if (planes == 3) w_scale = a_scale = 1.0f;
  const float sc = 1.0f / (w_scale * a_scale);
  X6Operands g{y, ldy, D, y_rows, nullptr, 0, 0, y_add, ldya, reinterpret_cast<const char*>(w_ip_x6), group_stride(planes, D), M, skip_padding ? num_ims : nullptr, rows_per_slide, a_scale};
  PATHS_REQUIRE((save_hid == nullptr) == (save_pproj == nullptr), "importance_proj_x6: save_hid and save_pproj come together");
  PATHS_REQUIRE(pe_table == nullptr || pe_rows > 0, "importance_proj_x6: pe_rows must be > 0 with a pe_table");
  auto go = [&](auto epi) {
    decltype(epi) e{b1, w2, b2, bp, special, div_term, locs, num_ims, rows_per_slide, patch_size, pe_mode, imp_mul, importance, tokens,
                    save_hid, save_pproj, pe_table, pe_table ? pe_rows : 0, sc};
    {
      if (splitk_ws != nullptr && planes == 2 && (y_add != nullptr || y_rows == nullptr) && D % 64 == 0 && D >= 256) {
        const int mt = (M + 127) / 128 * 4;
        const int64_t zstride = (int64_t)mt * 8 * 1024;
        int rc;
        if constexpr (A16) {
          X6Operands gs = g; gs.ksplit = 2;
          EpiRaw raw{splitk_ws, zstride, 8};
          rc = launch_x6_np<2, 2, 4, 2, true, true, EpiRaw, 1, true>(gs, 256, raw, stream, "importance_proj_x6_h16(split-k)");
        } else {
          X6Operands gs = g; gs.ksplit = 2;
          EpiRaw raw{splitk_ws, zstride, 8};
          rc = y_add == nullptr ? launch_x6_np<2, 2, 4, 2, false, false>(gs, 256, raw, stream, "importance_proj_x6(split-k, stored y)")
               : y_rows ? launch_x6_np<2, 2, 4, 2, true, true>(gs, 256, raw, stream, "importance_proj_x6(split-k)")
                        : launch_x6_np<2, 2, 4, 2, true, false>(gs, 256, raw, stream, "importance_proj_x6(split-k)");
        }
        if (rc != PATHS_OK) return rc;
        const int fblk = (M + 63) / 64, fdepth = (fblk + 255) / 256;
        const int flds = fdepth == 1 ? 84 * 1024 : fdepth == 2 ? 54 * 1024 : fdepth == 3 ? 41 * 1024 : 1024;
        PATHS_LDS_OPT_IN((x6_finish_kernel<2, decltype(epi)>), 84 * 1024, "importance_proj_x6(finish)");
        PATHS_LAUNCH_STOP((x6_finish_kernel<2, decltype(epi)>), dim3(fblk), dim3(256), flds, stream, splitk_ws, zstride, 8, M,
                          skip_padding ? num_ims : nullptr, rows_per_slide, e);
        PATHS_LAUNCH_CHECK("importance_proj_x6(finish)");
        return PATHS_OK;
      }
    }
    if constexpr (A16) {
      return paths_set_error(PATHS_EUNSUPPORTED, "importance_proj_x6_h16: split-K form only");
    } else {
      if (y_add != nullptr) return launch_x6<2, 4, 2, true>(planes, g, 256, e, stream, "importance_proj_x6(sum)");
      return launch_x6<2, 4, 2, false>(planes, g, 256, e, stream, "importance_proj_x6");
    }
  };
  if (pe_table != nullptr) return save_hid ? go(EpiImpProj<true, true>{}) : go(EpiImpProj<true, false>{});
  return save_hid ? go(EpiImpProj<false, true>{}) : go(EpiImpProj<false, false>{});
}
}
extern "C" {

int paths_importance_proj_x6(const float* y, int64_t ldy, const int64_t* y_rows, const float* y_add, int64_t ldya, const void* w_ip_x6, const float* b1, const float* w2, const float* b2,
                             const float* bp, const float* special, const float* div_term, const float* pe_table, int pe_rows, const int64_t* locs,
                             const int64_t* num_ims, int rows_per_slide, int patch_size, int pe_mode, int imp_mul,
                             float* importance, float* tokens, float* save_hid, float* save_pproj, int M, int D, int Hi, int d,
                             int skip_padding, int planes, float w_scale, float a_scale, float* splitk_ws, hipStream_t stream) {
  return importance_proj_x6<false>(y, ldy, y_rows, y_add, ldya, w_ip_x6, b1, w2, b2, bp, special, div_term, pe_table, pe_rows, locs, num_ims,
                                   rows_per_slide, patch_size, pe_mode, imp_mul, importance, tokens, save_hid, save_pproj, M, D, Hi, d,
                                   skip_padding, planes, w_scale, a_scale, splitk_ws, stream);
}

int paths_importance_proj_x6_h16(const float* y, int64_t ldy, const int64_t* y_rows, const float* y_add, int64_t ldya, const void* w_ip_x6, const float* b1, const float* w2, const float* b2,
                                 const float* bp, const float* special, const float* div_term, const float* pe_table, int pe_rows, const int64_t* locs,
                                 const int64_t* num_ims, int rows_per_slide, int patch_size, int pe_mode, int imp_mul,
                                 float* importance, float* tokens, float* save_hid, float* save_pproj, int M, int D, int Hi, int d,
                                 int skip_padding, int planes, float w_scale, float a_scale, float* splitk_ws, hipStream_t stream) {
  return importance_proj_x6<true>(y, ldy, y_rows, y_add, ldya, w_ip_x6, b1, w2, b2, bp, special, div_term, pe_table, pe_rows, locs, num_ims,
                                  rows_per_slide, patch_size, pe_mode, imp_mul, importance, tokens, save_hid, save_pproj, M, D, Hi, d,
                                  skip_padding, planes, w_scale, a_scale, splitk_ws, stream);
}


}
namespace {
template <bool A16>
int importance_qkv_x6(const float* y, int64_t ldy, const int64_t* y_rows, const float* y_add, int64_t ldya, const void* w_ip_x6,
                      const float* b1, const float* w2, const float* b2, const float* bp, const float* special,
                      const float* pe_table, int pe_rows, const int64_t* locs, const int64_t* num_ims, int B, int N,
                      int patch_size, int pe_mode, int imp_mul, float* importance, float* tokens, int D, int skip_padding,
                      float w_scale, float a_scale, float* splitk_ws, const void* w_qkv, const float* bqkv, float s_wqkv,
                      float qscale, void* qkv_images, int phases, int alpha_from_importance, hipStream_t stream) {
  PATHS_REQUIRE(!A16 || (phases & 1) == 0 || (y == nullptr && y_rows != nullptr), "importance_qkv_x6_h16: fp16 rows are given as y_rows");
  PATHS_REQUIRE(B > 0 && N > 0 && N % 64 == 0 && D % 64 == 0 && D >= 256, "importance_qkv_x6: bad shape B=%d N=%d (a multiple of 64) D=%d", B, N, D);
  PATHS_REQUIRE(pe_mode == 1 || pe_mode == 2, "importance_qkv_x6: pe_mode must be 1 (1d) or 2 (2d)");
  PATHS_REQUIRE(pe_table != nullptr && pe_rows > 0 && (pe_mode == 1 || locs != nullptr), "importance_qkv_x6: needs the positional-encoding table (and locs in 2d mode)");
  PATHS_REQUIRE(num_ims != nullptr && splitk_ws != nullptr && (uintptr_t)splitk_ws % 16 == 0, "importance_qkv_x6: num_ims and a 16-byte aligned workspace are required");
  PATHS_REQUIRE(phases > 0 && (phases & ~7) == 0, "importance_qkv_x6: phases is a mask of 1 (GEMM), 2 (importance finish), 4 (tokens + in_proj finish)");
  PATHS_REQUIRE(pow2(w_scale) && pow2(a_scale), "importance_qkv_x6: scales must be powers of two");
  const int64_t M64 = (int64_t)B * N;
  PATHS_REQUIRE(M64 < (1ll << 24), "importance_qkv_x6: B * N must stay below 2^24 rows");
  const int M = (int)M64, T = N + 1, Tp = (T + 63) / 64 * 64;
  const int mt = (M + 127) / 128 * 4;
  const int64_t zstride = (int64_t)mt * 8 * 1024;
  if (phases & 1) {
    PATHS_REQUIRE(w_ip_x6 != nullptr && y_add != nullptr && (y != nullptr) != (y_rows != nullptr), "importance_qkv_x6: the GEMM takes (y or y_rows) + y_add");
    PATHS_REQUIRE(ldya % 4 == 0 && (uintptr_t)y_add % 16 == 0, "importance_qkv_x6: y_add must be 16-byte aligned with ldya %% 4 == 0");
    X6Operands g{y, ldy, D, y_rows, nullptr, 0, 0, y_add, ldya, reinterpret_cast<const char*>(w_ip_x6), group_stride(2, D), M, skip_padding ? num_ims : nullptr, N, a_scale};
    g.ksplit = 2;
    EpiRaw raw{splitk_ws, zstride, 8};
    int rc;
    if constexpr (A16) rc = launch_x6_np<2, 2, 4, 2, true, true, EpiRaw, 1, true>(g, 256, raw, stream, "importance_qkv_x6_h16(split-k)");
    else rc = y_rows ? launch_x6_np<2, 2, 4, 2, true, true>(g, 256, raw, stream, "importance_qkv_x6(split-k)")
                     : launch_x6_np<2, 2, 4, 2, true, false>(g, 256, raw, stream, "importance_qkv_x6(split-k)");
    if (rc != PATHS_OK) return rc;
  }
  if (phases & 6) {
    PATHS_REQUIRE(b1 && w2 && b2 && importance, "importance_qkv_x6: b1, w2, b2 (device scalar) and importance are required");
    FinQkvParams f{splitk_ws, zstride, 2, b1, w2, b2, bp, special, pe_table, pe_rows, locs, num_ims, N, T, Tp, B, patch_size, pe_mode, imp_mul,
                   skip_padding, 1.0f / (w_scale * a_scale), alpha_from_importance, importance, tokens, w_qkv, bqkv, 1.0f / s_wqkv, qscale, qkv_images,
                   (B % 8 == 0 && (M / 128) % 8 == 0 && M % 128 == 0) ? 1 : 0};
    if (phases & 2) {
      const int rc = paths_launch_finish_importance(f, stream);
      if (rc != PATHS_OK) return rc;
    }
    if (phases & 4) {
      PATHS_REQUIRE(bp && special && tokens && w_qkv && bqkv && qkv_images && pow2(s_wqkv), "importance_qkv_x6: null operand (tokens + in_proj finish)");
      PATHS_REQUIRE(((uintptr_t)tokens | (uintptr_t)w_qkv | (uintptr_t)qkv_images) % 16 == 0, "importance_qkv_x6: buffers must be 16-byte aligned");
      return paths_launch_finish_qkv(f, stream);
    }
  }
  return PATHS_OK;
}
}
extern "C" {

int paths_importance_qkv_x6(const float* y, int64_t ldy, const int64_t* y_rows, const float* y_add, int64_t ldya, const void* w_ip_x6,
                            const float* b1, const float* w2, const float* b2, const float* bp, const float* special,
                            const float* pe_table, int pe_rows, const int64_t* locs, const int64_t* num_ims, int B, int N,
                            int patch_size, int pe_mode, int imp_mul, float* importance, float* tokens, int D, int skip_padding,
                            float w_scale, float a_scale, float* splitk_ws, const void* w_qkv, const float* bqkv, float s_wqkv,
                            float qscale, void* qkv_images, int phases, int alpha_from_importance, hipStream_t stream) {
  return importance_qkv_x6<false>(y, ldy, y_rows, y_add, ldya, w_ip_x6, b1, w2, b2, bp, special, pe_table, pe_rows, locs, num_ims, B, N, patch_size,
                                  pe_mode, imp_mul, importance, tokens, D, skip_padding, w_scale, a_scale, splitk_ws, w_qkv, bqkv, s_wqkv, qscale,
                                  qkv_images, phases, alpha_from_importance, stream);
}

int paths_importance_qkv_x6_h16(const float* y, int64_t ldy, const int64_t* y_rows, const float* y_add, int64_t ldya, const void* w_ip_x6,
                                const float* b1, const float* w2, const float* b2, const float* bp, const float* special,
                                const float* pe_table, int pe_rows, const int64_t* locs, const int64_t* num_ims, int B, int N,
                                int patch_size, int pe_mode, int imp_mul, float* importance, float* tokens, int D, int skip_padding,
                                float w_scale, float a_scale, float* splitk_ws, const void* w_qkv, const float* bqkv, float s_wqkv,
                                float qscale, void* qkv_images, int phases, int alpha_from_importance, hipStream_t stream) {
  return importance_qkv_x6<true>(y, ldy, y_rows, y_add, ldya, w_ip_x6, b1, w2, b2, bp, special, pe_table, pe_rows, locs, num_ims, B, N, patch_size,
                                 pe_mode, imp_mul, importance, tokens, D, skip_padding, w_scale, a_scale, splitk_ws, w_qkv, bqkv, s_wqkv, qscale,
                                 qkv_images, phases, alpha_from_importance, stream);
}

#endif
#if PATHS_X6_PART == 0 || PATHS_X6_PART == 3
int paths_gemm_nt_x6(const float* a, int64_t lda, const void* w_x6, int Kpacked, int k0, const float* b, float* out, int64_t ldo,
                     int M, int N, int Npad, int K, int act, const float* residual, int64_t ldr, const float* mask,
                     int64_t ldm, int accumulate, int planes, float w_scale, float a_scale, hipStream_t stream) {
  PATHS_REQUIRE(k0 % 16 == 0 && k0 >= 0 && k0 + K <= Kpacked, "gemm_nt_x6: bad k window");
  PATHS_REQUIRE(planes == 3 || planes == 4 || (planes == 2 && pow2(w_scale) && pow2(a_scale)), "gemm_nt_x6: planes 3 / 4 (bf16), or planes 2 with power-of-two scales");
  if (planes != 2) w_scale = a_scale = 1.0f;
  X6Operands g{a, lda, K, nullptr, nullptr, 0, 0, nullptr, 0, reinterpret_cast<const char*>(w_x6) + (int64_t)(k0 / 16) * plane_count(planes) * FRAG, group_stride(planes, Kpacked), M, nullptr, 0, a_scale};
  EpiBias e{b, out, ldo, N, act, residual, ldr, mask, ldm, accumulate, 1.0f / (w_scale * a_scale)};
  if (Npad % 256 != 0) {
    if (planes == 4) return launch_x6_np<4, 2, 2, 2, false, false, EpiBias, 2>(g, Npad, e, stream, "gemm_nt_x6(n128, bf16 x 2)");
    if (planes == 3) return launch_x6_np<3, 2, 2, 2, false, false, EpiBias, 2>(g, Npad, e, stream, "gemm_nt_x6(n128)");
    return launch_x6_np<2, 2, 2, 2, false, false, EpiBias, 2>(g, Npad, e, stream, "gemm_nt_x6(n128)");
  }
  return launch_x6<2, 4, 2, false>(planes, g, Npad, e, stream, "gemm_nt_x6");
}

int paths_gemm_rows_nt_x6(const int64_t* a_rows, const void* w_x6, int Kpacked, int k0, float* out, int64_t ldo,
                          int M, int Npad, int K, int planes, float w_scale, float a_scale, hipStream_t stream) {
  PATHS_REQUIRE(a_rows != nullptr && planes == 2 && pow2(w_scale) && pow2(a_scale), "gemm_rows_nt_x6: row addresses need planes = 2 with power-of-two scales");
  PATHS_REQUIRE(k0 % 16 == 0 && k0 >= 0 && k0 + K <= Kpacked, "gemm_rows_nt_x6: bad k window");
  X6Operands g{nullptr, K, K, a_rows, nullptr, 0, 0, nullptr, 0,
               reinterpret_cast<const char*>(w_x6) + (int64_t)(k0 / 16) * planes * FRAG, group_stride(planes, Kpacked), M, nullptr, 0, a_scale};
  EpiBias e{nullptr, out, ldo, Npad, 0, nullptr, 0, nullptr, 0, 0, 1.0f / (w_scale * a_scale)};
  return launch_x6<2, 4, 2, false>(planes, g, Npad, e, stream, "gemm_rows_nt_x6");
}

int paths_gemm_add_nt_x6(const float* a, int64_t lda, const int64_t* a_rows, const float* a_add, int64_t ld_add, const void* w_x6, int Kpacked,
                         const float* b, float* out, int64_t ldo, int M, int N, int Npad, int K, int act, const int64_t* num_ims,
                         int rows_per_slide, float w_scale, float a_scale, hipStream_t stream) {
  PATHS_REQUIRE((a != nullptr) != (a_rows != nullptr), "gemm_add_nt_x6: exactly one of a / a_rows");
  PATHS_REQUIRE(a_add != nullptr && ld_add % 4 == 0 && (uintptr_t)a_add % 16 == 0, "gemm_add_nt_x6: a_add must be 16-byte aligned with ld_add %% 4 == 0");
  PATHS_REQUIRE(pow2(w_scale) && pow2(a_scale) && K == Kpacked && (Npad % 256 == 0 || Npad % 192 == 0),
                "gemm_add_nt_x6: power-of-two scales, whole-K image, Npad a multiple of 256 or of 192");
  X6Operands g{a, lda, K, a_rows, nullptr, 0, 0, a_add, ld_add, reinterpret_cast<const char*>(w_x6), group_stride(2, Kpacked), M, num_ims, rows_per_slide, a_scale};
  EpiBias e{b, out, ldo, N, act, nullptr, 0, nullptr, 0, 0, 1.0f / (w_scale * a_scale)};
  if (Npad % 256 != 0) {
    return a_rows ? launch_x6_np<2, 2, 3, 2, true, true>(g, Npad, e, stream, "gemm_add_nt_x6(rows, 192-wide tiles)")
                  : launch_x6_np<2, 2, 3, 2, true, false>(g, Npad, e, stream, "gemm_add_nt_x6(192-wide tiles)");
  }
  return a_rows ? launch_x6_np<2, 2, 4, 2, true, true>(g, Npad, e, stream, "gemm_add_nt_x6(rows)")
                : launch_x6_np<2, 2, 4, 2, true, false>(g, Npad, e, stream, "gemm_add_nt_x6");
}

int paths_gemm_add_nt_x6_h16(const float* a, int64_t lda, const int64_t* a_rows, const float* a_add, int64_t ld_add, const void* w_x6, int Kpacked,
                             const float* b, float* out, int64_t ldo, int M, int N, int Npad, int K, int act, const int64_t* num_ims,
                             int rows_per_slide, float w_scale, float a_scale, hipStream_t stream) {
  PATHS_REQUIRE(a == nullptr && a_rows != nullptr, "gemm_add_nt_x6_h16: fp16 rows are given as a_rows");
  PATHS_REQUIRE(a_add != nullptr && ld_add % 4 == 0 && (uintptr_t)a_add % 16 == 0, "gemm_add_nt_x6_h16: a_add must be 16-byte aligned with ld_add %% 4 == 0");
  PATHS_REQUIRE(pow2(w_scale) && pow2(a_scale) && K == Kpacked && (Npad % 256 == 0 || Npad % 192 == 0),
                "gemm_add_nt_x6_h16: power-of-two scales, whole-K image, Npad a multiple of 256 or of 192");
  X6Operands g{nullptr, lda, K, a_rows, nullptr, 0, 0, a_add, ld_add, reinterpret_cast<const char*>(w_x6), group_stride(2, Kpacked), M, num_ims, rows_per_slide, a_scale};
  EpiBias e{b, out, ldo, N, act, nullptr, 0, nullptr, 0, 0, 1.0f / (w_scale * a_scale)};
  if (Npad % 256 != 0) return launch_x6_np<2, 2, 3, 2, true, true, EpiBias, 1, true>(g, Npad, e, stream, "gemm_add_nt_x6_h16(rows, 192-wide tiles)");
  return launch_x6_np<2, 2, 4, 2, true, true, EpiBias, 1, true>(g, Npad, e, stream, "gemm_add_nt_x6_h16(rows)");
}

#endif

}
```

### paths_amd/ops.py

```python
from __future__ import annotations

import math
import os
from typing import Dict, List, Optional

import torch

from . import _lib

LOG2E = 1.4426950408889634
QKV_IMAGES = os.environ.get("PATHS_QKV_IMAGES", "1") != "0"
TAIL_WS = os.environ.get("PATHS_TAIL_WS", "1") != "0"
TLAYER_WS = os.environ.get("PATHS_TLAYER_WS", "1") != "0"
SPLITK_IMPORTANCE = os.environ.get("PATHS_SPLITK_IMPORTANCE", "1") != "0"
FUSE_QKV = int(os.environ.get("PATHS_FUSE_QKV", "2"))
KERNEL_TIMER = None
TIMER_ALL = False


def timed(name: str, fn, meta=None, detail: bool = True):
    if KERNEL_TIMER is None or (detail and not TIMER_ALL):
        return fn()
    return KERNEL_TIMER(name, fn, meta or {})
GEMM_MODE = os.environ.get("PATHS_GEMM_MODE", "h3")
A_SCALE = float(os.environ.get("PATHS_H3_A_SCALE", "16"))
AGG_FP8 = os.environ.get("PATHS_AGG_FP8", "0") != "0"
ATTN_FP8 = os.environ.get("PATHS_ATTN_FP8", "0") != "0"
TRAIN_PLANES = int(os.environ.get("PATHS_TRAIN_PLANES", "4"))
assert TRAIN_PLANES in (3, 4), "PATHS_TRAIN_PLANES must be 3 (exact) or 4 (two bf16 planes)"
TRAIN_FWD_PLANES = int(os.environ.get("PATHS_TRAIN_FWD_PLANES", "2"))


H3_STATE_MARGIN = 8.0


def h3_in_range(feat_absmax: float) -> bool:
    return math.isfinite(feat_absmax) and (feat_absmax + H3_STATE_MARGIN) * A_SCALE < 65504.0


RANGE_FALLBACKS = [0]


class range_guard:

    def __init__(self, feat_absmax: float):
        self.amax = float(feat_absmax)
        self.saved = None

    def __enter__(self):
        global GEMM_MODE, TRAIN_FWD_PLANES
        if not math.isfinite(self.amax):
            raise _lib.PathsHipError("input features contain inf or NaN")
        if not h3_in_range(self.amax) and (GEMM_MODE == "h3" or TRAIN_FWD_PLANES == 2):
            self.saved = (GEMM_MODE, TRAIN_FWD_PLANES)
            RANGE_FALLBACKS[0] += 1
            GEMM_MODE, TRAIN_FWD_PLANES = ("x6" if GEMM_MODE == "h3" else GEMM_MODE), 3
        return self

    def __exit__(self, *exc):
        global GEMM_MODE, TRAIN_FWD_PLANES
        if self.saved is not None:
            GEMM_MODE, TRAIN_FWD_PLANES = self.saved
        return False


def split_planes() -> int:
    if GEMM_MODE not in ("h3", "x6", "f32"):
        raise ValueError(f"PATHS_GEMM_MODE must be 'h3', 'x6' or 'f32' (got {GEMM_MODE!r})")
    return 2 if GEMM_MODE == "h3" else 3


def a_scale() -> float:
    return A_SCALE if GEMM_MODE == "h3" else 1.0


def x6_pack(w: torch.Tensor, n_pad: Optional[int] = None, planes: Optional[int] = None, w_scale: Optional[float] = None):
    assert w.is_cuda and w.dtype == torch.float32 and w.dim() == 2 and w.stride(1) == 1
    planes = split_planes() if planes is None else planes
    N, K = w.shape
    n_pad = N if n_pad is None else n_pad
    if planes != 2:
        w_scale = 1.0
    elif w_scale is None:
        w_scale = _pow2_scale(w)
    out = torch.empty((n_pad * K * 2 * (2 if planes == 4 else planes),), device=w.device, dtype=torch.uint8)
    _lib.call("paths_x6_pack_weights", _lib.ptr(w), w.stride(0), _lib.ptr(out), N, n_pad, K, planes, w_scale, _lib.stream())
    return out, w_scale


def _pow2_scale(w: torch.Tensor) -> float:
    amax = float(w.abs().max())
    return 2.0 ** max(-14, min(24, math.floor(math.log2(16384.0 / amax)))) if amax > 0 and math.isfinite(amax) else 1.0


_LAGGED_EPOCH = [0]


def _lagged_store(owner) -> Dict[object, list]:
    st = owner.__dict__.get("_paths_lagged")
    if st is None or st.get("_epoch") != _LAGGED_EPOCH[0]:
        st = {"_epoch": _LAGGED_EPOCH[0]}
        object.__setattr__(owner, "_paths_lagged", st)
    return st


def _pow2_scale_lagged(w: torch.Tensor, owner, key) -> float:
    store = _lagged_store(owner)
    ent = store.get(key)
    if ent is None:
        ent = store[key] = [_pow2_scale(w), None, torch.empty((1,), dtype=torch.float32).pin_memory()]
    elif ent[1] is not None and ent[1].query():
        amax = float(ent[2][0])
        if not math.isfinite(amax) or amax * ent[0] >= 65504.0:
            store.pop(key, None)
            raise _lib.PathsHipError(f"weight {key!r}: max|w| = {amax} left the fp16 range of its lagged scale {ent[0]}; "
                                     "call paths_amd.ops.reset_lagged_scales() after replacing weights")
        if amax > 0:
            ent[0] = 2.0 ** max(-14, min(24, math.floor(math.log2(16384.0 / amax))))
        ent[1] = None
    if ent[1] is None:
        ent[2].copy_(w.detach().abs().max().reshape(1), non_blocking=True)
        ev = torch.cuda.Event()
        ev.record()
        ent[1] = ev
    return ent[0]


def reset_lagged_scales():
    _LAGGED_EPOCH[0] += 1


def _tlayer_images(layer: Dict[str, object], part: int, kind: str):
    key = f"{kind}_image_{part}"
    if key not in layer:
        ws = [layer["wo"], layer["w1"], layer["w2"]] if part == 0 else [layer["wqkv"]]
        scales = tuple(_pow2_scale(w) for w in ws)
        dims = (layer["wo"].shape[0],) if kind == "ws" else ()
        img = torch.empty((int(getattr(_lib.load(), f"paths_tlayer_{kind}_image_bytes")(part, *dims)),), device=ws[0].device, dtype=torch.uint8)
        pw = [_lib.ptr(w) for w in ws] + [None] * (3 - len(ws))
        sc = list(scales) + [1.0] * (3 - len(scales))
        _lib.call(f"paths_tlayer_pack_{kind}", part, pw[0], pw[1], pw[2], sc[0], sc[1], sc[2], _lib.ptr(img), *dims, _lib.stream())
        layer[key] = (img, scales)
    return layer[key]


def tlayer_h3_images(layer: Dict[str, object], part: int):
    return _tlayer_images(layer, part, "h3")


def tlayer_ws_images(layer: Dict[str, object], part: int):
    return _tlayer_images(layer, part, "ws")


def token0_ws_image(layer: Dict[str, object], qscale: float) -> torch.Tensor:
    if "t0_image" not in layer:
        d = int(layer["wo"].shape[0])
        img = torch.empty((int(_lib.load().paths_token0_ws_image_bytes_d(d)),), device=layer["wo"].device, dtype=torch.uint8)
        _lib.call("paths_token0_pack_ws_d", _lib.ptr(layer["wqkv"]), _lib.ptr(layer["bqkv"]), _lib.ptr(layer["wo"]), _lib.ptr(layer["bo"]),
                  _lib.ptr(layer["w1"]), _lib.ptr(layer["w2"]), qscale, d, _lib.ptr(img), _lib.stream())
        layer["t0_image"] = img
    return layer["t0_image"]


_T0_COUNTERS: Dict[tuple, torch.Tensor] = {}
_T0_RETIRED: List[torch.Tensor] = []


def token0_counters(dev, B: int) -> torch.Tensor:
    key = (dev.index if dev.index is not None else torch.cuda.current_device(), _lib.stream())
    t = _T0_COUNTERS.get(key)
    if t is None or t.numel() < 3 * B:
        if t is not None:
            _T0_RETIRED.append(t)
        t = _T0_COUNTERS[key] = torch.zeros((max(768, 3 * B),), device=dev, dtype=torch.int32)
    return t


def _x6_of(pack: Dict[str, object], key: str, planes: Optional[int] = None, lagged: bool = False):
    planes = split_planes() if planes is None else planes
    k6 = f"{key}_split{planes}"
    if k6 not in pack:
        ws = _pow2_scale_lagged(pack[key], pack["_owner"], key) if (lagged and planes == 2) else None
        pack[k6] = x6_pack(pack[key], planes=planes, w_scale=ws)
    return pack[k6]


def pe_table(lvl_pack: Dict[str, object], pe_mode: int, d: int, rows: int) -> torch.Tensor:
    div = lvl_pack["div_2d" if pe_mode == 2 else "div_1d"]
    key = (pe_mode, d, div.device)
    tab = _PE_TABLES.get(key)
    if tab is None or tab.shape[0] < rows:
        cap = 1 << max(6, (rows - 1).bit_length())
        tab = torch.empty((cap, d // 2 if pe_mode == 2 else d), device=div.device, dtype=torch.float32)
        _lib.call("paths_pe_table", _lib.ptr(div), pe_mode, d, cap, _lib.ptr(tab), _lib.stream())
        if key in _PE_TABLES:
            _PE_RETIRED.append(_PE_TABLES[key])
        _PE_TABLES[key] = tab
    return tab


_PE_TABLES: Dict[tuple, torch.Tensor] = {}
_PE_RETIRED: List[torch.Tensor] = []
_PE_DIVS: Dict[tuple, tuple] = {}


def _pe_divs(d: int, dev) -> tuple:
    key = (d, dev)
    if key not in _PE_DIVS:
        k = 10000.0
        _PE_DIVS[key] = (torch.exp(torch.arange(0, d, 2) * (-math.log(k) / d)).float().to(dev),
                         torch.exp(torch.arange(0, d // 2, 2) * (-math.log(k) / d)).float().to(dev))
    return _PE_DIVS[key]


def use_x6(D: int, Hc: int = 64) -> bool:
    split_planes()
    return GEMM_MODE != "f32" and D % 256 == 0 and Hc % 64 == 0


def _versions(params):
    return tuple((p.data_ptr(), p._version) for p in params)


def _cached_pack(owner, list_params):
    params = getattr(owner, "_paths_param_list", None)
    if params is None:
        params = list_params()
        object.__setattr__(owner, "_paths_param_list", params)
    key = _versions(params)
    cache = getattr(owner, "_paths_pack", None)
    return key, (cache[1] if cache is not None and cache[0] == key else None)


def pack_lstm(lstm) -> Dict[str, torch.Tensor]:
    srcs = [lstm.forget_gate[0], lstm.remember_gate[0], lstm.remember_map[0], lstm.out_select_gate[0], lstm.mem_to_out[0]]
    key, packed = _cached_pack(lstm, lambda: [t for m in srcs for t in (m.weight, m.bias)])
    if packed is not None:
        return packed
    with torch.no_grad():
        f, r, m, o, mo = srcs
        Hc = f.weight.shape[0]
        assert Hc % 64 == 0, "hierarchical_ctx_mlp_hidden_dim must be a multiple of 64 for this build"
        wc = torch.stack([f.weight.view(Hc // 32, 32, -1), r.weight.view(Hc // 32, 32, -1), m.weight.view(Hc // 32, 32, -1)], dim=1)
        bc = torch.stack([f.bias.view(Hc // 32, 32), r.bias.view(Hc // 32, 32), m.bias.view(Hc // 32, 32)], dim=1)
        packed = {
            "w_gates": torch.cat([wc.reshape(3 * Hc, -1), o.weight], dim=0).float().contiguous(),
            "b_gates": torch.cat([bc.reshape(3 * Hc), o.bias], dim=0).float().contiguous(),
            "w_mem": mo.weight.detach().float().contiguous(),
            "b_mem": mo.bias.detach().float().contiguous(),
            "Hc": Hc,
            "_owner": lstm,
        }
    lstm._paths_pack = (key, packed)
    return packed


def pack_level(proc) -> Dict[str, object]:
    agg = proc.global_agg
    key, packed = _cached_pack(proc, lambda: (
        list(proc.importance_mlp.parameters()) + [agg.proj_in.weight, agg.proj_in.bias, agg.special_token]
        + list(agg.transformer.decoder.parameters()) + list(proc.classification_layer.parameters())
        + (list(proc.hctx_mlp.parameters()) if hasattr(proc, "hctx_mlp") else [])))
    if packed is not None:
        return packed
    with torch.no_grad():
        c = lambda t: t.detach().float().contiguous()
        d = agg.dim
        layers = _pack_decoder_layers(agg)
        dev = agg.proj_in.weight.device
        div_1d, div_2d = _pe_divs(d, dev)
        packed = {
            "w_ip": torch.cat([proc.importance_mlp[0].weight, agg.proj_in.weight], dim=0).float().contiguous(),
            "w_ip_fwd": torch.cat([proc.importance_mlp[0].weight[:64], agg.proj_in.weight[:64],
                                   proc.importance_mlp[0].weight[64:], agg.proj_in.weight[64:]], dim=0).float().contiguous(),
            "b1": c(proc.importance_mlp[0].bias), "w2": c(proc.importance_mlp[2].weight.view(-1)),
            "b2": c(proc.importance_mlp[2].bias.view(-1)),
            "bp": c(agg.proj_in.bias), "special": c(agg.special_token),
            "div_1d": div_1d, "div_2d": div_2d,
            "layers": layers,
            "lnfg": c(agg.transformer.decoder.norm.weight), "lnfb": c(agg.transformer.decoder.norm.bias),
            "lnf_eps": float(agg.transformer.decoder.norm.eps),
            "wcls": c(proc.classification_layer.weight), "bcls": c(proc.classification_layer.bias),
            "_owner": proc,
        }
        if hasattr(proc, "hctx_mlp"):
            packed.update({"wh1": c(proc.hctx_mlp[0].weight), "bh1": c(proc.hctx_mlp[0].bias),
                           "wh2": c(proc.hctx_mlp[2].weight), "bh2": c(proc.hctx_mlp[2].bias)})
    proc._paths_pack = (key, packed)
    return packed


def _pack_decoder_layers(agg) -> List[Dict[str, object]]:
    c = lambda t: t.detach().float().contiguous()
    layers = []
    d, H = agg.dim, agg.nhead
    hd = d // H
    hdp = padded_head_dim(hd)
    pad = None
    if hdp != hd:
        dev = agg.proj_in.weight.device
        col = (torch.arange(d, device=dev) // hd) * hdp + torch.arange(d, device=dev) % hd
        row = torch.cat([col + k * H * hdp for k in range(3)])
        pad = (row, col, H * hdp)
    for lyr in agg.transformer.decoder.layers:
        layers.append({
            "wqkv": c(lyr.self_attn.in_proj_weight), "bqkv": c(lyr.self_attn.in_proj_bias),
            "wo": c(lyr.self_attn.out_proj.weight), "bo": c(lyr.self_attn.out_proj.bias),
            "cab": c(lyr.multihead_attn.out_proj.bias),
            "ln1g": c(lyr.norm1.weight), "ln1b": c(lyr.norm1.bias),
            "ln2g": c(lyr.norm2.weight), "ln2b": c(lyr.norm2.bias),
            "ln3g": c(lyr.norm3.weight), "ln3b": c(lyr.norm3.bias),
            "w1": c(lyr.linear1.weight), "b1": c(lyr.linear1.bias),
            "w2": c(lyr.linear2.weight), "b2": c(lyr.linear2.bias),
            "eps": float(lyr.norm1.eps),
        })
        layers[-1]["w_in"], layers[-1]["b_in"] = layers[-1]["wqkv"], layers[-1]["bqkv"]
        if pad is not None:
            row, col, di = pad
            lay = layers[-1]
            wq = torch.zeros((3 * di, d), device=row.device, dtype=torch.float32)
            wq[row] = lay["wqkv"]
            bq = torch.zeros((3 * di,), device=row.device, dtype=torch.float32)
            bq[row] = lay["bqkv"]
            wo = torch.zeros((d, di), device=row.device, dtype=torch.float32)
            wo[:, col] = lay["wo"]
            lay.update({"wqkv": wq, "bqkv": bq, "wo": wo, "_unpad": (row, col)})
    return layers


def pack_aggregator(agg) -> Dict[str, object]:
    key, packed = _cached_pack(agg, lambda: [agg.proj_in.weight, agg.proj_in.bias, agg.special_token] + list(agg.transformer.decoder.parameters()))
    if packed is not None:
        return packed
    with torch.no_grad():
        c = lambda t: t.detach().float().contiguous()
        d = agg.dim
        dev = agg.proj_in.weight.device
# ... 434 lines not shown


def level_forward(mc, lstm_pack, lvl_pack, fts: torch.Tensor, locs: torch.Tensor, num_ims: torch.Tensor,
                  state_prev: Optional[torch.Tensor], ctx_prev: Optional[torch.Tensor], ctx_all: Optional[torch.Tensor],
                  skip_padding: bool, return_attention: bool = False, return_rollout: bool = False) -> Dict[str, torch.Tensor]:
    sel = selection_forward(mc, lstm_pack, lvl_pack, fts, locs, num_ims, state_prev, skip_padding)
    status = torch.zeros((1,), device=fts.device, dtype=torch.int32)
    (B, N), LH = locs.shape[:2], (mc.trans_layers, mc.trans_heads)
    pair = lambda *lead: (torch.empty((B, *lead, N), device=fts.device, dtype=torch.float32), torch.empty((B, *lead), device=fts.device, dtype=torch.float32))
    attention = pair(*LH) if return_attention else None
    rollout = pair() if return_rollout else None
    agg = aggregator_forward(mc, lvl_pack, sel["tokens"], sel["num_ims"], ctx_prev, ctx_all, status=status, qkv=sel, attention=attention,
                             rollout=rollout)
    if int(status.item()) & 4:
        raise _lib.PathsHipError("a bounded in-launch hand-off wait of the token-0 tail gave up (csrc/token0_ws.hip): results invalid")
    out = {"logits": agg["logits"], "ctx_slide": agg["ctx_slide"], "ctx_patch": sel["ctx_patch"], "importance": sel["importance"]}
    if attention is not None:
        out["attention"], out["attention_self"] = attention
    if rollout is not None:
        out["rollout"], out["rollout_self"] = rollout
    return out


def selection_forward(mc, lstm_pack, lvl_pack, fts, locs, num_ims, state_prev, skip_padding: bool,
                      parent=None, max_pos: int = 0, x_rows=None, feat_dim: Optional[int] = None,
                      importance_out: Optional[torch.Tensor] = None, last_level: bool = False,
                      x_rows_h16: bool = False) -> Dict[str, torch.Tensor]:
    _lib.require_cuda(fts, locs, num_ims, state_prev, x_rows)
    if x_rows is not None:
        assert fts is None and feat_dim is not None and state_prev is None and x_rows.dtype == torch.int64 and x_rows.is_contiguous()
        (B, N), D = x_rows.shape, int(feat_dim)
    else:
        B, N, D = fts.shape
    d, H, L = mc.trans_dim, mc.trans_heads, mc.trans_layers
    T = N + 1
    M = B * N
    dev = locs.device
    st = _lib.stream()
    p = _lib.ptr
    f32 = dict(device=dev, dtype=torch.float32)
    assert fts is None or (fts.is_contiguous() and fts.dtype == torch.float32)
    locs = locs.contiguous()
    num_ims = num_ims.contiguous()
    assert locs.dtype == torch.int64 and num_ims.dtype == torch.int64
    pe_mode = 2 if mc.pos_encoding_mode == "2d" else 1
    tokens = torch.empty((B, T, d), **f32)

    x6 = use_x6(D, lstm_pack["Hc"] if mc.lstm else 64)
    assert x_rows is None or (x6 and split_planes() == 2 and mc.lstm), "row pointers need the default split mode and lstm=true"
    assert not x_rows_h16 or x_rows is not None, "x_rows_h16 describes x_rows"
    h16 = "_h16" if x_rows_h16 else ""
    pe_rows = N if pe_mode == 1 else int(max_pos)
    if pe_rows == 0 and FUSE_QKV in (1, 2) and fast_path(mc) and N % 64 == 0 and not torch.is_grad_enabled():
        top = int(locs.max().item()) // int(mc.patch_size) + 1 if locs.numel() else 0
        pe_rows = top if 0 < top <= (1 << 16) else 0
    pe_tab = pe_table(lvl_pack, pe_mode, d, pe_rows) if pe_rows > 0 else None

    generic = not fast_path(mc)
    fuse_qkv = (FUSE_QKV in (1, 2) and not generic and x6 and split_planes() == 2 and mc.lstm and GEMM_MODE == "h3" and TLAYER_WS and QKV_IMAGES
                and L > 1 and pe_tab is not None and not (ATTN_FP8 or AGG_FP8) and D % 64 == 0 and D >= 256 and N % 64 == 0 and TAIL_WS)
    fused: Dict[str, object] = {}
    generic_add = generic and x6 and split_planes() == 2 and mc.lstm and GENERIC_ADD and GENERIC_SPLIT and D % 128 == 0

    def imp_proj(src, imp_mul, imp_out, add=None):
        if generic:
            assert add is None and src is not None
            return importance_proj_generic(mc, lvl_pack, src, D, locs, num_ims, B, N, D, imp_mul, imp_out, tokens)
        splitk = x6 and SPLITK_IMPORTANCE and add is not None and split_planes() == 2 and (M + 127) // 128 <= 160
        splitk = splitk or (x6 and x_rows_h16 and src is None)
        if splitk and fuse_qkv and imp_out is importance:
            wip, wip_s = _x6_of(lvl_pack, "w_ip_fwd")
            lay0 = lvl_pack["layers"][0]
            iq, sq = tlayer_ws_images(lay0, 1)
            hd = d // H
            ws = torch.empty((int(_lib.load().paths_importance_proj_x6_workspace(M)),), device=dev, dtype=torch.uint8)
            qkv_img = torch.empty((int(_lib.load().paths_attention_x6_workspace(B, T, H, hd, 2)),), device=dev, dtype=torch.uint8)
            args = (p(src), D, p(x_rows) if src is None else None, p(add), add.stride(1), p(wip), p(lvl_pack["b1"]), p(lvl_pack["w2"]),
                    p(lvl_pack["b2"]), p(lvl_pack["bp"]), p(lvl_pack["special"]), p(pe_tab), pe_tab.shape[0], p(locs), p(num_ims), B, N,
                    mc.patch_size, pe_mode, imp_mul, p(imp_out), p(tokens), D, 1 if skip_padding else 0, wip_s, a_scale(), p(ws),
                    p(iq), p(lay0["bqkv"]), sq[0], LOG2E / math.sqrt(hd), p(qkv_img))
            if FUSE_QKV == 2 and not last_level:
                _lib.call("paths_importance_qkv_x6" + h16, *args, 3, 0, st)
                fused["finish"] = lambda: _lib.call("paths_importance_qkv_x6", *args, 4, 1, _lib.stream())
            else:
                _lib.call("paths_importance_qkv_x6" + h16, *args, 5, 0, st)
            fused["qkv_img"], fused["ws"] = qkv_img, ws
            return
        assert x6 or add is None
        importance_proj(mc, lvl_pack, src, x_rows, add, locs, num_ims, pe_tab, imp_mul, imp_out, tokens, None, None, B, N, D, skip_padding,
                        planes=split_planes() if x6 else 0, splitk=splitk, h16=h16)

    if importance_out is not None:
        assert importance_out.shape == (B, N) and importance_out.is_contiguous() and importance_out.dtype == torch.float32
        importance = importance_out
    else:
        importance = torch.zeros((B, N), **f32) if skip_padding else torch.empty((B, N), **f32)
    if mc.lstm:
        Hc = lstm_pack["Hc"]
        Dp = D + Hc
        state_out = torch.empty((B, N, Dp), **f32)
        y = None if (x6 and (not generic or generic_add)) else torch.empty((B, N, D), **f32)
        ws_o = torch.empty(((M + 255) // 256 * 256, D), **f32)
        prev = prev_state_operands(parent, state_prev, B, N, D, Hc, parent["hp"] if parent is not None else None)

        def lstm(phases):
            lstm_cell(lstm_pack, fts, x_rows, prev, state_out, y, ws_o, None, None, N, num_ims if skip_padding else None, phases,
                      planes=split_planes() if x6 else 0, h16=h16)

        if KERNEL_TIMER is None:
            lstm(7)
        else:
            timed("lstm_gate_c", lambda: lstm(1))
            timed("lstm_gate_o", lambda: lstm(2), {"rows": N, "B": B, "K": D if prev[1] is None else 2 * D, "Ncols": D, "parent_partials": parent is not None,
                                                   "x6": x6, "planes": split_planes() if x6 else 0}, detail=False)
            timed("lstm_mem_to_out", lambda: lstm(4))
        if generic_add:
            timed("importance_proj", lambda: importance_proj_generic_add(mc, lvl_pack, fts, x_rows, state_out, locs, num_ims, B, N, D,
                                                                         1 if mc.importance_mode == "mul" else 0, importance, tokens, skip_padding, pe_tab=pe_tab,
                                                                         x_rows_h16=x_rows_h16))
        elif x6 and not generic:
            timed("importance_proj", lambda: imp_proj(fts, 1 if mc.importance_mode == "mul" else 0, importance, add=state_out))
        else:
            timed("importance_proj", lambda: imp_proj(y, 1 if mc.importance_mode == "mul" else 0, importance))
        del ws_o
    else:
        imp_proj(fts, 0, importance)
        hctx = None
        if state_prev is not None and mc.hierarchical_ctx:
            assert state_prev.shape == (B, N, D) and state_prev.stride(2) == 1 and state_prev.stride(0) == N * state_prev.stride(1)
            Hh = lvl_pack["wh1"].shape[0]
            assert Hh % 128 == 0, "hierarchical_ctx_mlp_hidden_dim must be a multiple of 128 for lstm=false"
            hid = torch.empty((B, N, Hh), **f32)
            hctx = torch.empty((B, N, D), **f32)
            _lib.call("paths_linear_f32", p(state_prev), state_prev.stride(1), p(lvl_pack["wh1"]), p(lvl_pack["bh1"]), p(hid), Hh,
                      M, Hh, Hh, D, 1, st)
            _lib.call("paths_linear_f32", p(hid), Hh, p(lvl_pack["wh2"]), p(lvl_pack["bh2"]), p(hctx), D, M, D, D, Hh, 0, st)
        state_out = torch.empty((B, N, D), **f32)
        _lib.call("paths_scale_add_rows", p(fts), p(importance), p(hctx) if hctx is not None else None, p(num_ims), N, D, M,
                  1 if mc.importance_mode == "mul" else 0, p(state_out), st)
        scratch_imp = torch.empty((B, N), **f32)
        imp_proj(state_out, 0, scratch_imp)

    out = {"ctx_patch": state_out, "importance": importance, "tokens": tokens, "num_ims": num_ims}
    if "qkv_img" in fused:
        out["qkv_img"], out["qkv_finish"], out["_qkv_ws"] = fused["qkv_img"], fused.get("finish"), fused["ws"]
    return out


def prev_state_operands(parent, state_prev, B: int, N: int, D: int, Hc: int, hp=None):
    if parent is not None:
        assert state_prev is None
        c0t = parent["c0"]
        assert c0t.shape == (B, N, Hc) and c0t.is_contiguous()
        return Hc, None, c0t.data_ptr(), _lib.ptr(hp), _lib.ptr(parent["hp_row"])
    if state_prev is not None:
        assert state_prev.shape[:2] == (B, N) and state_prev.shape[2] == D + Hc and state_prev.stride(2) == 1
        assert state_prev.stride(0) == N * state_prev.stride(1), "state rows must be uniformly strided"
        return state_prev.stride(1), state_prev.data_ptr(), state_prev.data_ptr() + 4 * D, None, None
    return 0, None, None, None, None


def lstm_cell(lstm_pack, fts, x_rows, prev, state_out, y, o, frm, tc, N: int, num_ims, phases: int, planes: int = 0, lagged: bool = False,
              h16: str = ""):
    p = _lib.ptr
    ld, h0, c0, hp, hp_row = prev
    Dp = state_out.shape[2]
    Hc = lstm_pack["Hc"]
    D = Dp - Hc
    M = state_out.shape[0] * N
    if planes:
        (wg, wg_s), (wm, wm_s) = _x6_of(lstm_pack, "w_gates", planes, lagged=lagged), _x6_of(lstm_pack, "w_mem", planes, lagged=lagged)
        _lib.call("paths_lstm_cell_x6" + h16, p(fts), D, p(x_rows), h0, ld, c0, ld, p(wg), p(lstm_pack["b_gates"]), p(wm), p(lstm_pack["b_mem"]),
                  p(state_out), Dp, p(y), D, p(o), p(frm), p(tc), hp, hp_row, M, D, Hc, p(num_ims), N, phases,
                  planes, wg_s, wm_s, A_SCALE if planes == 2 else 1.0, _lib.stream())
    else:
        _lib.call("paths_lstm_cell", p(fts), D, h0, ld, c0, ld, p(lstm_pack["w_gates"]), p(lstm_pack["b_gates"]),
                  p(lstm_pack["w_mem"]), p(lstm_pack["b_mem"]), p(state_out), Dp, p(y), D,
                  p(o), p(frm), p(tc), hp, hp_row, M, D, Hc, p(num_ims), N, phases, _lib.stream())


def parent_gate_product(lstm_pack, hk, hp, planes: int = 0, lagged: bool = False):
    p = _lib.ptr
    rows, D = hk.shape
    G = hp.shape[1]
    if planes and G % 256 == 0:
        wg, wg_s = _x6_of(lstm_pack, "w_gates", planes, lagged=lagged)
        _lib.call("paths_gemm_nt_x6", p(hk), D, p(wg), 2 * D, D, None, p(hp), G, rows, G, G, D, 0, None, 0, None, 0, 0, planes, wg_s,
                  A_SCALE if planes == 2 else 1.0, _lib.stream())
    else:
        _lib.call("paths_gemm_nt_f32", p(hk), D, lstm_pack["w_gates"].data_ptr() + 4 * D, 2 * D, None, p(hp), G, rows, G, G, D, 0,
                  None, 0, None, 0, 0, _lib.stream())


def parent_partials(lstm_pack, state_out: torch.Tensor, keep_idx: torch.Tensor, keep_count: torch.Tensor,
                    kept_rows: Optional[torch.Tensor] = None) -> torch.Tensor:
    B, N, Dp = state_out.shape
    Hc = lstm_pack["Hc"]
    D = Dp - Hc
    G = 3 * Hc + D
    cap = keep_idx.shape[1]
    f32 = dict(device=state_out.device, dtype=torch.float32)
    st = _lib.stream()
    p = _lib.ptr
    hp = torch.empty((B * cap, G), **f32)
    if kept_rows is not None:
        assert use_x6(D, Hc) and G % 256 == 0 and split_planes() == 2 and kept_rows.shape == (B, cap) and kept_rows.dtype == torch.int64
        wg, wg_s = _x6_of(lstm_pack, "w_gates")
        timed("parent_gemm", lambda: _lib.call("paths_gemm_rows_nt_x6", p(kept_rows), p(wg), 2 * D, D, p(hp), G, B * cap, G, D, 2, wg_s, a_scale(), st))
        return hp
    hk = torch.empty((B * cap, D), **f32)
    _lib.call("paths_gather_kept_rows", p(state_out), N, Dp, p(keep_idx), cap, p(keep_count), D, B, p(hk), st)
    parent_gate_product(lstm_pack, hk, hp, planes=split_planes() if use_x6(D, Hc) else 0)
    return hp


def _export_attention(attention, lvl_pack, l: int, x, num_ims, H: int, special_last: int, slot: Optional[int] = None):
    patch, self_ = attention
    B, L, _, N = patch.shape
    T = N + 1
    slot = l if slot is None else slot
    lay = lvl_pack["layers"][l]
    d = lay["w_in"].shape[1]
    ws = torch.empty((int(_lib.load().paths_token0_attention_workspace(B, T, d, H)),), device=x.device, dtype=torch.float32)
    _lib.call("paths_token0_attention", _lib.ptr(x), _lib.ptr(num_ims), _lib.ptr(lay["w_in"]), _lib.ptr(lay["b_in"]),
              patch.data_ptr() + 4 * slot * H * N, L * H * N, self_.data_ptr() + 4 * slot * H, L * H, _lib.ptr(ws), B, T, d, H, special_last,
              _lib.stream())


class _Rollout:

    def __init__(self, rollout, attention, lvl_pack, tokens, num_ims, H: int, L: int):
        self.out, self.out_self = rollout
        self.attention, self.lvl_pack, self.num_ims, self.H, self.L = attention, lvl_pack, num_ims, H, L
        self.B, self.T, self.d = tokens.shape
        self.prepared: Dict[int, torch.Tensor] = {}

    def layer(self, l: int, x, special_last: int):
        B, T, d, H, L = self.B, self.T, self.d, self.H, self.L
        p = _lib.ptr
        f32 = dict(device=x.device, dtype=torch.float32)
        if l < L - 1:
            lay = self.lvl_pack["layers"][l]
            ws = torch.empty((int(_lib.load().paths_attention_rollout_workspace(B, T, d, H)),), **f32)
            _lib.call("paths_attention_rollout_prepare", p(x), p(self.num_ims), p(lay["w_in"]), p(lay["b_in"]), p(ws), B, T, d, H,
                      special_last, _lib.stream())
            self.prepared[l] = ws
            return
        att, slot = self.attention, L - 1
        if att is None:
            N = T - 1
            att, slot = (torch.empty((B, 1, H, N), **f32), torch.empty((B, 1, H), **f32)), 0
            _export_attention(att, self.lvl_pack, L - 1, x, self.num_ims, H, special_last, slot=0)
        La = att[0].shape[1]
        a_patch, a_self = att[0].data_ptr() + 4 * slot * H * (T - 1), att[1].data_ptr() + 4 * slot * H
        out, out_self = p(self.out) if T > 1 else None, p(self.out_self)
        if L == 1:
            _lib.call("paths_attention_rollout_seed", a_patch, La * H * (T - 1), a_self, La * H, p(self.num_ims), None, out, T - 1, out_self,
                      B, T, H, _lib.stream())
            return
        r = [torch.empty((B, T), **f32), torch.empty((B, T), **f32)]
        _lib.call("paths_attention_rollout_seed", a_patch, La * H * (T - 1), a_self, La * H, p(self.num_ims), p(r[0]), None, 0, None,
                  B, T, H, _lib.stream())
        for i, l2 in enumerate(range(L - 2, -1, -1)):
            last = l2 == 0
            _lib.call("paths_attention_rollout_step", p(self.prepared.pop(l2)), p(self.num_ims), p(r[i % 2]),
                      None if last else p(r[(i + 1) % 2]), out if last else None, T - 1, out_self if last else None, B, T, d, H,
                      _lib.stream())


class _Export:

    def __init__(self, attention, rollout, lvl_pack, num_ims, H: int):
        self.attention, self.rollout, self.lvl_pack, self.num_ims, self.H = attention, rollout, lvl_pack, num_ims, H

    def layer(self, l: int, x, special_last: int):
        if self.attention is not None:
            _export_attention(self.attention, self.lvl_pack, l, x, self.num_ims, self.H, special_last)
        if self.rollout is not None:
            self.rollout.layer(l, x, special_last)


def _check_attention(attention, mc, tokens):
    B, T, _ = tokens.shape
    patch, self_ = attention
    H, L = mc.trans_heads, mc.trans_layers
    assert patch.shape == (B, L, H, T - 1) and self_.shape == (B, L, H), "attention: ([B, L, H, N], [B, L, H]) tensors"
    assert all(t.dtype == torch.float32 and t.is_contiguous() and t.device == tokens.device for t in attention)
    assert tokens.is_contiguous()


def _check_rollout(rollout, tokens):
    B, T, _ = tokens.shape
    out, out_self = rollout
    assert out.shape == (B, T - 1) and out_self.shape == (B,), "rollout: ([B, N], [B]) tensors"
    assert all(t.dtype == torch.float32 and t.is_contiguous() and t.device == tokens.device for t in rollout)
    assert tokens.is_contiguous()


def aggregator_forward(mc, lvl_pack, tokens, num_ims, ctx_prev, ctx_all, status=None, qkv=None, attention=None,
                       rollout=None) -> Dict[str, torch.Tensor]:
    qkv_img, qkv_finish = (qkv.get("qkv_img"), qkv.get("qkv_finish")) if qkv is not None else (None, None)
    if attention is not None:
        _check_attention(attention, mc, tokens)
    ro = None
    if rollout is not None:
        _check_rollout(rollout, tokens)
        ro = _Rollout(rollout, attention, lvl_pack, tokens, num_ims, mc.trans_heads, mc.trans_layers)
    if qkv_finish is not None:
        timed("agg_tokens_qkv", qkv_finish)
    return timed("aggregator", lambda: _aggregator_forward(mc, lvl_pack, tokens, num_ims, ctx_prev, ctx_all, status, qkv_img, attention, ro),
                 {"T": tokens.shape[1], "d": tokens.shape[2], "L": mc.trans_layers, "planes": split_planes() if GEMM_MODE != "f32" else 0},
                 detail=False)


def _aggregator_forward_ws(mc, lvl_pack, tokens, num_ims, head, qkv_img, xb, tail_f32, export, status=None, qkv_ready: bool = False):
    B, T, d = tokens.shape
    H, L = mc.trans_heads, mc.trans_layers
    hd = d // H
    st = _lib.stream()
    p = _lib.ptr
    layers = lvl_pack["layers"]
    qscale = LOG2E / math.sqrt(hd)
    Tp = (T + 63) // 64 * 64
    o_img = torch.empty((B * Tp * d * 4,), device=tokens.device, dtype=torch.uint8)

    def token_layer(x_in, x_out, post, nxt):
        token_layer_ws(x_in, x_out, o_img, post, nxt, qkv_img, num_ims, B, T, d, H, qscale)

    xa = tokens
    if not qkv_ready:
        timed("agg_in_proj", lambda: token_layer(xa, None, None, layers[0]))
    order = 1 if qkv_ready else 0
    for l in range(L - 1):
        export.layer(l, xa, order)
        timed("agg_attention", lambda: _lib.call("paths_attention_h3_img", p(o_img), p(num_ims), B, T, H, hd, p(qkv_img), st))
        last = l + 1 == L - 1
        timed("agg_token_chain", lambda: token_layer(xa, xb, layers[l], None if last else layers[l + 1]))
        xa, xb = xb, xa
    export.layer(L - 1, xa, order)
    if TAIL_WS:
        timed("agg_token0_tail", lambda: token0_tail_ws(lvl_pack, xa, num_ims, head, status, B, T, d, H, qscale, order))
    else:
        timed("agg_token0_tail", lambda: tail_f32(xa, True))
    return {"logits": head[4], "ctx_slide": head[3]}


def _aggregator_forward(mc, lvl_pack, tokens, num_ims, ctx_prev, ctx_all, status=None, qkv_img=None, attention=None,
                        rollout=None) -> Dict[str, torch.Tensor]:
    _lib.require_cuda(tokens, num_ims, ctx_prev, ctx_all)
    export = _Export(attention, rollout, lvl_pack, num_ims, mc.trans_heads)
    if AGG_FP8:
        return _aggregator_forward_generic(mc, lvl_pack, tokens, num_ims, ctx_prev, ctx_all, export, fp8=True)
    if not fast_path(mc):
        return _aggregator_forward_generic(mc, lvl_pack, tokens, num_ims, ctx_prev, ctx_all, export, status=status)
    B, T, d = tokens.shape
    H, L = mc.trans_heads, mc.trans_layers
    st = _lib.stream()
    p = _lib.ptr
    f32 = dict(device=tokens.device, dtype=torch.float32)
    hd = d // H
    q = torch.empty((B, H, T, hd), **f32)
    k = torch.empty((B, H, T, hd), **f32)
# ... 54 lines not shown
```

### paths_amd/utils.py

```python
from __future__ import annotations

import os
from types import SimpleNamespace
from typing import Dict, List, Optional, Sequence

import contextlib
import math
import torch
import torch.nn.functional as F

from . import _lib, ops
from .data_utils.slide import DeviceSlide, DeviceSlideBatch, HostSlide, slide_batch

OVERLAP_AGGREGATOR = os.environ.get("PATHS_OVERLAP_AGGREGATOR", "1") != "0"
ROCTX_RANGES = os.environ.get("PATHS_ROCTX", "0") != "0"
ROWS_IN_PLACE = os.environ.get("PATHS_ROWS_IN_PLACE", "1") != "0"
TRAIN_PARENT = os.environ.get("PATHS_TRAIN_PARENT", "1") != "0"
STREAM_LANE = 0
_STREAMS: Dict[int, tuple] = {}


def nll_loss(hazards, y, c, alpha=0.4, eps=1e-7):
    B = hazards.shape[0]
    surv = torch.cumprod(1 - hazards, dim=1)
# ... 292 lines not shown

def _child_capacity(n: int, keep: int):
    cap_keep = n if keep < 0 else min(n, keep)
    return cap_keep, 4 * cap_keep


def _level_sizes(n0: int, keep_patches, num_levels: int) -> List[int]:
    sizes = [n0]
    for i in range(num_levels - 1):
        sizes.append(_child_capacity(sizes[-1], int(keep_patches[i]))[1])
    return sizes


def _expand_children(batch, nxt: int, patch_size: int, keep_idx, keep_count, locs, N: int, Nn: int, status, stream: int, careful: bool,
                     want_child_pos: bool, want_hp_row: bool):
    B, cap_keep, p = len(batch), keep_idx.shape[1], _lib.ptr
    i32 = dict(device=batch.device, dtype=torch.int32)
    i64 = dict(device=batch.device, dtype=torch.int64)
    child_pos = torch.empty((B, 4 * cap_keep), **i32) if want_child_pos else None
    if batch.on_demand:
        return (Nn, *_expand_on_demand(batch, nxt, patch_size, keep_idx, keep_count, locs, N, Nn, status, stream, child_pos, want_hp_row))
    gx, gy, masks = p(batch.gx[nxt]), p(batch.gy[nxt]), p(batch.mask_ptrs[nxt])

    def expand(cap):
        bufs = (torch.empty((B,), **i64), torch.empty((B, cap, 2), **i64), torch.empty((B, cap), **i64),
                torch.empty((B, cap), **i32), torch.empty((B, cap), **i32), torch.empty((B, cap), **i32) if want_hp_row else None)
        _lib.call("paths_expand_children", p(keep_idx), cap_keep, p(keep_count), p(locs), N, patch_size, gx, gy, masks, B, cap,
                  *(p(t) for t in bufs[:5]), p(status), p(child_pos), p(bufs[5]), stream)
        return bufs

    bufs = ops.timed("expand", lambda: expand(Nn))
    if careful:
        empty = (bufs[0] == 0).cpu()
        if bool(empty.any()):
            need = Nn
            for b in torch.nonzero(empty).flatten().tolist():
                tissue = int(batch.slides[b].masks[nxt].sum().item())
                X, Y = batch.slides[b].shape(nxt)
                need = max(need, tissue if tissue > 0 else X * Y)
            if need > Nn:
                Nn = need
                bufs = expand(Nn)
            _lib.call("paths_fallback_all_cells", gx, gy, masks, patch_size, B, Nn, *(p(t) for t in bufs[:5]), p(status), p(bufs[5]), stream)
    return (Nn, *bufs[:5], child_pos, bufs[5])


def _mask_supplied(batch, buf, want_mask: bool, stream: int):
    B, cap, D = buf.shape
    mask = torch.empty((B, cap), device=batch.device, dtype=torch.uint8) if want_mask else None
    _lib.call("paths_tissue_mask_absmax_h16" if batch.dtype == torch.float16 else "paths_tissue_mask_absmax", buf.data_ptr(), B * cap, D,
              _lib.ptr(mask), batch.absmax_bits.data_ptr(), stream)
    return mask


def _note_range(batch, amax_before: float):
    if batch.feat_absmax > amax_before:
        batch.guards.enter_context(ops.range_guard(batch.feat_absmax))


def _expand_on_demand(batch, nxt: int, patch_size: int, keep_idx, keep_count, locs, N: int, Nn: int, status, stream: int, child_pos,
                      want_hp_row: bool):
    assert stream == _lib.stream(), "the on-demand expansion synchronises with torch's current stream"
    B, cap_keep, p = len(batch), keep_idx.shape[1], _lib.ptr
    i32 = dict(device=batch.device, dtype=torch.int32)
    i64 = dict(device=batch.device, dtype=torch.int64)
    Nc = 4 * cap_keep
    cand_count, cand_cells, cand_slot = torch.empty((B,), **i32), torch.empty((B, Nc, 2), **i64), torch.empty((B, Nc), **i32)
    ops.timed("candidates", lambda: _lib.call("paths_candidate_children", p(keep_idx), cap_keep, p(keep_count), p(locs), N, patch_size,
                                              p(batch.gx[nxt]), p(batch.gy[nxt]), B, p(cand_count), p(cand_cells), p(cand_slot), stream))
    counts = cand_count.cpu().tolist()
    buf = batch.supply(nxt, [cand_cells[b, :counts[b]] for b in range(B)], Nc)
    mask = _mask_supplied(batch, buf, True, stream)
    bufs = (torch.empty((B,), **i64), torch.empty((B, Nn, 2), **i64), torch.empty((B, Nn), **i64),
            torch.empty((B, Nn), **i32), torch.empty((B, Nn), **i32), torch.empty((B, Nn), **i32) if want_hp_row else None)
    ops.timed("admit", lambda: _lib.call("paths_admit_children", p(cand_count), p(cand_cells), p(cand_slot), p(mask), p(keep_idx), cap_keep,
                                         p(keep_count), patch_size, B, Nn, *(p(t) for t in bufs[:5]), p(status), p(child_pos), p(bufs[5]), stream))
    before = batch.feat_absmax
    num_out = batch.read_back(bufs[0])
    empty = [b for b in range(B) if num_out[b] == 0]
    if empty:
        names = ", ".join(repr(batch.slides[b].slide_id or f"#{b}") for b in empty)
        raise _lib.PathsHipError(
            f"on-demand slide {names}: none of the {[counts[b] for b in empty]} cells requested at level {nxt} is tissue.  The reference "
            "would continue with every cell of that level's grid (data_utils/slide.py:336-352), i.e. encode the whole grid - what "
            "on-demand slides exist to avoid; preprocess such a slide (DeviceSlide / HostSlide) or keep more patches")
    _note_range(batch, before)
    return (*bufs[:5], child_pos, bufs[5])


def _stage_rows(batch, rows, n: int, zero_row, stream: int):
    buf = torch.empty((len(batch), n, batch.dim), device=batch.device, dtype=batch.dtype)
    p = _lib.ptr
    ops.timed("stage", lambda: _lib.call("paths_stage_rows", p(rows), len(batch) * n, batch.dim * buf.element_size(), p(buf), p(zero_row), stream))
    return buf


def _rows_in_place(r) -> bool:
    mc, D, Dp = r.mc, r.D, r.Dp
    return bool(r.share_parent and ops.use_x6(D, Dp - D) and ops.split_planes() == 2 and ROWS_IN_PLACE
                and (ops.fast_path(mc) or (ops.GENERIC_ADD and ops.GENERIC_SPLIT and D % 128 == 0)))


def _level0(r) -> SimpleNamespace:
    B, N, D, p = r.B, r.batch.n0, r.D, _lib.ptr
    lv = SimpleNamespace(N=N, state_prev=None, parent=None, staged=None)
    lv.fts = None if r.rows_in_place else torch.empty((B, N, D), **r.f32)
    lv.x_rows = torch.empty((B, N), **r.i64) if r.rows_in_place else None
    lv.locs = torch.empty((B, N, 2), **r.i64)
    lv.parent_inds = torch.empty((B, N), **r.i64)
    lv.num_ims = torch.empty((B,), **r.i64)
    _lib.call("paths_level0_batch" + r.sfx, p(r.batch.grid_ptrs[0]), p(r.batch.gx[0]), p(r.batch.gy[0]), B, D, r.mc.patch_size, N,
              p(lv.fts), p(lv.locs), p(lv.parent_inds), p(lv.num_ims), 0, p(lv.x_rows), p(r.zero_row), r.st)
    if getattr(r.batch, "masked", False):
        _lib.call("paths_level0_mask_rows", p(r.batch.mask_ptrs[0]), p(r.batch.gx[0]), p(r.batch.gy[0]), B, D, N, p(lv.fts), p(lv.x_rows),
                  p(r.zero_row), r.st)
    if r.stage_host:
        lv.staged = _stage_rows(r.batch, lv.x_rows, N, r.zero_row, r.st)
    return lv


def _aggregate(r, lvl_pack, sel, ctx_hist, N: int):
    mc, B, f32 = r.mc, r.B, r.f32
    ctx_prev = ctx_hist[-1] if (ctx_hist and mc.slide_ctx_mode == "residual") else None
    ctx_all = torch.stack(ctx_hist, dim=1) if (ctx_hist and mc.slide_ctx_mode == "concat") else None
    att = None
    if r.attention:
        Hh, Lt = mc.trans_heads, mc.trans_layers
        att = (torch.empty((B, Lt, Hh, N), **f32), torch.empty((B, Lt, Hh), **f32))
    ro = (torch.empty((B, N), **f32), torch.empty((B,), **f32)) if r.rollout else None
    agg = ops.aggregator_forward(mc, lvl_pack, sel["tokens"], sel["num_ims"], ctx_prev, ctx_all, status=r.status, qkv=sel, attention=att,
                                 rollout=ro)
    if att is not None:
        agg = dict(agg, attention=att[0], attention_self=att[1])
    if ro is not None:
        agg = dict(agg, rollout=ro[0], rollout_self=ro[1])
    return agg


def _child_step(r, i: int, lv, out, keep: int):
    B, D, Dp, N, p, st = r.B, r.D, r.Dp, lv.N, _lib.ptr, r.st
    batch, share_parent, rows_in_place = r.batch, r.share_parent, r.rows_in_place
    cap_keep, Nn = _child_capacity(N, keep)
    forked = r.overlap and share_parent
    keep_idx = torch.empty((B, cap_keep), **r.i32)
    keep_count = torch.empty((B,), **r.i32)
    kept_rows = None
    with (_lib.fork_behind([r.par_stream], r.main_stream) if forked else contextlib.nullcontext()):
        if rows_in_place:
            kept_rows = torch.empty((B, cap_keep), **r.i64)
            ops.timed("topk", lambda: _lib.call("paths_topk_rows", p(out["importance"]), N, p(lv.num_ims), B, N, keep, p(keep_idx), cap_keep,
                                                p(keep_count), p(out["ctx_patch"]), Dp, N, p(kept_rows), p(r.zero_row), st))
        else:
            _lib.call("paths_topk", p(out["importance"]), N, p(lv.num_ims), B, N, keep, p(keep_idx), cap_keep, p(keep_count), st)
    hp = ops.parent_partials(r.lstm_pack, out["ctx_patch"], keep_idx, keep_count, kept_rows) if share_parent else None
    st2 = r.par_stream.cuda_stream if forked else st
    nx = SimpleNamespace(fts=None, x_rows=None, staged=None, state_prev=None, parent=None)
    with (torch.cuda.stream(r.par_stream) if forked else contextlib.nullcontext()):
        Nn, num_next, locs_next, parent_next, src_row, src_cell, _, hp_row = _expand_children(
            batch, i + 1, r.mc.patch_size, keep_idx, keep_count, lv.locs, N, Nn, r.status, st2, r.careful, False, share_parent)
        nx.N, nx.num_ims, nx.locs, nx.parent_inds = Nn, num_next, locs_next, parent_next
        if batch.on_demand:
            rows_in_place = r.rows_in_place = _rows_in_place(r)
        grid = p(batch.grid_ptrs[i + 1])
        if share_parent:
            Hc = Dp - D
            c0 = torch.empty((B, Nn, Hc), **r.f32)
            if rows_in_place:
                nx.x_rows = torch.empty((B, Nn), **r.i64)
                ops.timed("gather", lambda: _lib.call(
                    "paths_gather_rows" + r.sfx, grid, p(src_cell), D, out["ctx_patch"].data_ptr() + 4 * D, N, Dp,
                    p(src_row), Hc, p(num_next), B, Nn, None, p(c0), 0, p(nx.x_rows), p(r.zero_row), st2))
                if r.stage_host:
                    nx.staged = _stage_rows(batch, nx.x_rows, Nn, r.zero_row, st2)
            else:
                nx.fts = torch.empty((B, Nn, D), **r.f32)
                _lib.call("paths_gather_rows" + r.sfx, grid, p(src_cell), D, out["ctx_patch"].data_ptr() + 4 * D, N, Dp,
                          p(src_row), Hc, p(num_next), B, Nn, p(nx.fts), p(c0), 0, None, None, st2)
            nx.parent = {"hp": hp, "hp_row": hp_row, "c0": c0}
        else:
            nx.fts = torch.empty((B, Nn, D), **r.f32)
            nx.state_prev = torch.empty((B, Nn, Dp), **r.f32)
            _lib.call("paths_gather_rows" + r.sfx, grid, p(src_cell), D, p(out["ctx_patch"]), N, Dp, p(src_row), Dp,
                      p(num_next), B, Nn, p(nx.fts), p(nx.state_prev), 0, None, None, st2)
        if forked:
            r.keepalive.append((nx, src_row, src_cell))
    return nx, keep_idx, keep_count


def _recurse_body(model, batch, keep_patches: Sequence[int], num_levels: int, trace: Optional[list], careful: bool, agg_stream,
                  par_stream, attention: bool = False, rollout: bool = False) -> Dict[str, torch.Tensor]:
    mc = model.procs[0].config
    ops.check_supported(mc)
    assert batch.num_levels >= num_levels
    B, dev, D = len(batch), batch.device, batch.dim
    Dp = model.procs[0].ctx_dim()[1]
    f32 = dict(device=dev, dtype=torch.float32)
    h16 = batch.dtype == torch.float16
    lstm_pack = ops.pack_lstm(model.lstm) if model.use_lstm else None
    share_parent = model.use_lstm
    overlap = agg_stream is not None
    main_stream = torch.cuda.current_stream(dev) if overlap else None
    keepalive = []
    r = SimpleNamespace(mc=mc, batch=batch, B=B, D=D, Dp=Dp, st=_lib.stream(), sfx="_h16" if h16 else "", f32=f32,
                        i32=dict(device=dev, dtype=torch.int32), i64=dict(device=dev, dtype=torch.int64),
                        lstm_pack=lstm_pack, share_parent=share_parent,
                        careful=careful, attention=attention, rollout=rollout, overlap=overlap, main_stream=main_stream,
                        par_stream=par_stream, keepalive=keepalive, status=None)
    if batch.on_demand:
        _mask_supplied(batch, batch.supply(0, batch.cells0, batch.n0), False, r.st)
        batch.read_back(None)
        _note_range(batch, 0.0)
    r.rows_in_place = rows_in_place = _rows_in_place(r)
    r.zero_row = torch.zeros((D,), **f32) if rows_in_place else None
    r.stage_host = batch.host_resident and rows_in_place
    lv = _level0(r)
    sizes = _level_sizes(lv.N, keep_patches, num_levels)
    zbuf = _lib.zeros((B * sum(sizes) + 64,), **f32)
    imp_all = zbuf[:B * sum(sizes)]
    r.status = status = zbuf[B * sum(sizes) + 32:B * sum(sizes) + 33].view(torch.int32)
    imp_off = [B * sum(sizes[:i]) for i in range(num_levels)]
    out, ctx_hist, fork_pending = None, [], False
    for i in range(num_levels):
        lvl_pack = ops.pack_level(model.procs[i])
        if fork_pending:
            _lib.stream_wait(main_stream, par_stream)
        N = lv.N
        imp_buf = imp_all[imp_off[i]:imp_off[i] + B * N].view(B, N) if N == sizes[i] else None
        last = i == num_levels - 1
        with _Range(f"level {i}: selection chain (LSTM gates, importance, projection)"), \
                (_lib.fork_behind([agg_stream], main_stream) if overlap else contextlib.nullcontext()):
            sel = ops.selection_forward(mc, lstm_pack, lvl_pack, lv.fts, lv.locs, lv.num_ims, lv.state_prev, True, parent=lv.parent,
                                        max_pos=batch.max_dim[i], x_rows=lv.x_rows, feat_dim=D, importance_out=imp_buf,
                                        last_level=last, x_rows_h16=h16 and r.rows_in_place)
        if overlap:
            keepalive.append((sel["tokens"], sel["num_ims"], sel.get("qkv_img"), sel.get("_qkv_ws")))
        with (torch.cuda.stream(agg_stream) if overlap else contextlib.nullcontext()), \
                _Range(f"level {i}: aggregator (second stream)" if overlap else f"level {i}: aggregator"):
            agg = _aggregate(r, lvl_pack, sel, ctx_hist, N)
        out = {"logits": agg["logits"], "ctx_slide": agg["ctx_slide"], "ctx_patch": sel["ctx_patch"], "importance": sel["importance"]}
        ctx_hist.append(out["ctx_slide"])
        rec = None
        if trace is not None:
            rec = {"num_ims": lv.num_ims, "locs": lv.locs, "parent_inds": lv.parent_inds, "importance": out["importance"],
                   "logits": out["logits"], "ctx_slide": out["ctx_slide"]}
            if attention:
                rec["attention"], rec["attention_self"] = agg["attention"], agg["attention_self"]
            if rollout:
                rec["rollout"], rec["rollout_self"] = agg["rollout"], agg["rollout_self"]
            trace.append(rec)
        if last:
            break
        lv, keep_idx, keep_count = _child_step(r, i, lv, out, int(keep_patches[i]))
        fork_pending = overlap and share_parent
        if rec is not None:
            rec["keep_idx"], rec["keep_count"] = keep_idx, keep_count
    if overlap:
        _lib.stream_wait(main_stream, agg_stream)
        _lib.stream_wait(main_stream, par_stream)
        keepalive.clear()
    out = dict(out)
    out["status"] = status
    return out


def recurse_train(model, slides, keep_patches: Sequence[int], num_levels: int, careful: bool = False,
                  trace: Optional[list] = None, path: Optional[Sequence] = None, points=None) -> Dict[str, torch.Tensor]:
    batch = _stored_batch(slides, "recurse_train")
    with ops.range_guard(batch.feat_absmax):
        return _recurse_train_body(model, batch, keep_patches, num_levels, careful, trace, path, points)


def _recurse_train_body(model, batch, keep_patches, num_levels, careful, trace=None, path=None, points=None):
    from . import autograd as pag
    mc = model.procs[0].config
    ops.check_supported(mc, training=True)
    B, dev, D = len(batch), batch.device, batch.dim
    st = _lib.stream()
    p = _lib.ptr
    i32 = dict(device=dev, dtype=torch.int32)
    i64 = dict(device=dev, dtype=torch.int64)
    f32 = dict(device=dev, dtype=torch.float32)
    status = torch.zeros(1, **i32)
    N = batch.n0
    fts = torch.empty((B, N, D), **f32)
    locs = torch.empty((B, N, 2), **i64)
    parent = torch.empty((B, N), **i64)
    num_ims = torch.empty((B,), **i64)
    h16 = batch.dtype == torch.float16
    _lib.call("paths_level0_batch_h16" if h16 else "paths_level0_batch", p(batch.grid_ptrs[0]), p(batch.gx[0]), p(batch.gy[0]), B, D, mc.patch_size, N,
              p(fts), p(locs), p(parent), p(num_ims), 1, None, None, st)
    if batch.masked:
        _lib.call("paths_level0_mask_rows", p(batch.mask_ptrs[0]), p(batch.gx[0]), p(batch.gy[0]), B, D, N, p(fts), None, None, st)
    state_prev, ctx_prev, ctx_hist = None, None, []
    logits = None
    parent_form = TRAIN_PARENT and model.use_lstm and not careful
    par = None
    for i in range(num_levels):
        if mc.slide_ctx_mode == "concat":
            ctx_prev = torch.stack(ctx_hist, dim=1) if ctx_hist else None
        if points is not None:
            new = points(i, fts, num_ims)
            assert new.shape == fts.shape and new.dtype == fts.dtype and new.is_contiguous(), "points: [B,N,D] fp32 rows like the level's"
            fts = new
        if trace is not None:
            fts = fts.detach().requires_grad_(True)
        logits, ctx_slide, state_out, importance = pag.level_apply(model.procs[i], model.lstm if model.use_lstm else None, fts, locs,
                                                                   num_ims, state_prev, ctx_prev, parent=par,
                                                                   detach_params=trace is not None)
        ctx_prev = ctx_slide
        ctx_hist.append(ctx_slide)
        rec = None
        if trace is not None:
            rec = {"num_ims": num_ims, "locs": locs, "parent_inds": parent, "importance": importance, "logits": logits.detach(),
                   "fts": fts}
            trace.append(rec)
        if i == num_levels - 1:
            break
        keep = int(keep_patches[i])
        cap_keep, Nn = _child_capacity(N, keep)
        if path is not None:
            keep_idx, keep_count = path[i]
            if not (keep_idx.shape == (B, cap_keep) and keep_count.shape == (B,) and keep_idx.dtype == keep_count.dtype == torch.int32
                    and keep_idx.is_contiguous() and keep_idx.device == keep_count.device == dev):
                raise ValueError(f"path[{i}]: (keep_idx [{B}, {cap_keep}] int32, keep_count [{B}] int32) on {dev} expected, got "
                                 f"{tuple(keep_idx.shape)} {keep_idx.dtype} / {tuple(keep_count.shape)} {keep_count.dtype}")
        else:
            keep_idx = torch.empty((B, cap_keep), **i32)
            keep_count = torch.empty((B,), **i32)
            _lib.call("paths_topk", p(importance), N, p(num_ims), B, N, keep, p(keep_idx), cap_keep, p(keep_count), st)
        Nn, num_next, locs_next, parent_next, src_row, src_cell, child_pos, hp_row = _expand_children(
            batch, i + 1, mc.patch_size, keep_idx, keep_count, locs, N, Nn, status, st, careful, True, parent_form)
# ... 93 lines not shown
```

Baseline: 3958 slides/s.

## Skip forget-gate GEMM at depth 0 and seed LSTM accumulators from raw parent partials

At level 0, where there is no previous cell state, the LSTM c-phase now runs a GEMM over only the r and m gate rows using a separately packed weight slice. The forget gate multiplies a zero c0, so its columns are dropped. Parent partial products are now stored unscaled (raw), and the child LSTM seeds its accumulators from them with buffer loads when the scales match. This removes a scale multiply and guarded loads. The epilogue also hoists the c0 loads ahead of the gate math when frm is not saved. The changes add a new kernel entry point and an extra packed weight copy, and the raw seeding depends on the power-of-two scales lining up.

```diff
diff --git a/include/paths_hip.h b/include/paths_hip.h
--- a/include/paths_hip.h
+++ b/include/paths_hip.h
@@ -56,6 +56,20 @@
                            const float* hp, const int* hp_row,
                            int M, int D, int Hc, const int64_t* num_ims, int rows_per_slide, int phases,
                            int planes, float wg_scale, float wm_scale, float a_scale, paths_stream_t stream);
+int paths_lstm_cell_x6_seeded(const float* x, int64_t ldx, const int64_t* x_rows, const float* h0, int64_t ldh0, const float* c0, int64_t ldc0,
+                              const void* w_gates_x6, const float* b_gates, const void* w_mem_x6, const float* b_mem,
+                              float* state_out, int64_t ldso, float* y, int64_t ldy, float* ws_o, float* save_frm, float* save_tc,
+                              const float* hp, const int* hp_row,
+                              int M, int D, int Hc, const int64_t* num_ims, int rows_per_slide, int phases,
+                              int planes, float wg_scale, float wm_scale, float a_scale, const void* w_rm0_x6, int hp_rows, float hp_scale,
+                              paths_stream_t stream);
+int paths_lstm_cell_x6_seeded_h16(const float* x, int64_t ldx, const int64_t* x_rows, const float* h0, int64_t ldh0, const float* c0, int64_t ldc0,
+                                  const void* w_gates_x6, const float* b_gates, const void* w_mem_x6, const float* b_mem,
+                                  float* state_out, int64_t ldso, float* y, int64_t ldy, float* ws_o, float* save_frm, float* save_tc,
+                                  const float* hp, const int* hp_row,
+                                  int M, int D, int Hc, const int64_t* num_ims, int rows_per_slide, int phases,
+                                  int planes, float wg_scale, float wm_scale, float a_scale, const void* w_rm0_x6, int hp_rows, float hp_scale,
+                                  paths_stream_t stream);
 int paths_importance_proj_x6(const float* y, int64_t ldy, const int64_t* y_rows, const float* y_add, int64_t ldya, const void* w_ip_x6, const float* b1, const float* w2, const float* b2 ,
                              const float* bp, const float* special, const float* div_term, const float* pe_table, int pe_rows,
                              const int64_t* locs,
@@ -92,6 +106,8 @@
                              int rows_per_slide, float w_scale, float a_scale, paths_stream_t stream);
 int paths_gemm_rows_nt_x6(const int64_t* a_rows, const void* w_x6, int Kpacked, int k0, float* out, int64_t ldo,
                           int M, int Npad, int K, int planes, float w_scale, float a_scale, paths_stream_t stream);
+int paths_gemm_rows_nt_x6_raw(const int64_t* a_rows, const void* w_x6, int Kpacked, int k0, float* out, int64_t ldo,
+                              int M, int Npad, int K, int planes, float w_scale, float a_scale, paths_stream_t stream);
 
 int paths_gemm_nt_f32(const float* a, int64_t lda, const float* w, int64_t ldw, const float* b, float* out, int64_t ldo,
                       int M, int N, int Npad, int K, int act, const float* residual, int64_t ldr, const float* mask,
diff --git a/paths_amd/_lib.py b/paths_amd/_lib.py
--- a/paths_amd/_lib.py
+++ b/paths_amd/_lib.py
@@ -22,6 +22,8 @@
     "paths_x6_pack_weights_t": [_vp, _i64, _vp, _i32, _i32, _i32, _i32, _i32, _vp],
     "paths_lstm_cell_x6": [_vp, _i64, _vp, _vp, _i64, _vp, _i64, _vp, _vp, _vp, _vp, _vp, _i64, _vp, _i64, _vp, _vp, _vp, _vp, _vp,
                            _i32, _i32, _i32, _vp, _i32, _i32, _i32, _f32, _f32, _f32, _vp],
+    "paths_lstm_cell_x6_seeded": [_vp, _i64, _vp, _vp, _i64, _vp, _i64, _vp, _vp, _vp, _vp, _vp, _i64, _vp, _i64, _vp, _vp, _vp, _vp, _vp,
+                                  _i32, _i32, _i32, _vp, _i32, _i32, _i32, _f32, _f32, _f32, _vp, _i32, _f32, _vp],
     "paths_importance_proj_x6": [_vp, _i64, _vp, _vp, _i64, _vp, _vp, _vp, _vp, _vp, _vp, _vp, _vp, _i32, _vp, _vp, _i32, _i32, _i32, _i32,
                                  _vp, _vp, _vp, _vp, _i32, _i32, _i32, _i32, _i32, _i32, _f32, _f32, _vp, _vp],
     "paths_importance_qkv_x6": [_vp, _i64, _vp, _vp, _i64, _vp, _vp, _vp, _vp, _vp, _vp, _vp, _i32, _vp, _vp, _i32, _i32, _i32, _i32, _i32,
@@ -97,6 +99,7 @@
     "paths_topk": [_vp, _i64, _vp, _i32, _i32, _i32, _vp, _i64, _vp, _vp],
     "paths_topk_rows": [_vp, _i64, _vp, _i32, _i32, _i32, _vp, _i64, _vp, _vp, _i64, _i64, _vp, _vp, _vp],
     "paths_gemm_rows_nt_x6": [_vp, _vp, _i32, _i32, _vp, _i64, _i32, _i32, _i32, _i32, _f32, _f32, _vp],
+    "paths_gemm_rows_nt_x6_raw": [_vp, _vp, _i32, _i32, _vp, _i64, _i32, _i32, _i32, _i32, _f32, _f32, _vp],
     "paths_expand_children": [_vp, _i64, _vp, _vp, _i64, _i32, _vp, _vp, _vp, _i32, _i64, _vp, _vp, _vp, _vp, _vp, _vp, _vp, _vp, _vp],
     "paths_candidate_children": [_vp, _i64, _vp, _vp, _i64, _i32, _vp, _vp, _i32, _vp, _vp, _vp, _vp],
     "paths_admit_children": [_vp, _vp, _vp, _vp, _vp, _i64, _vp, _i32, _i32, _i64, _vp, _vp, _vp, _vp, _vp, _vp, _vp, _vp, _vp],
@@ -133,7 +136,7 @@
     "paths_visited_overlap": [_vp, _i64, _vp, _vp, _vp, _vp, _i32, _i32, _i32, _i32, _vp, _vp],
     "paths_level0_mask_rows": [_vp, _vp, _vp, _i32, _i32, _i64, _vp, _vp, _vp, _vp],
 }
-for _n in ("paths_lstm_cell_x6", "paths_importance_proj_x6", "paths_importance_qkv_x6", "paths_gemm_add_nt_x6", "paths_gather_rows",
+for _n in ("paths_lstm_cell_x6", "paths_lstm_cell_x6_seeded", "paths_importance_proj_x6", "paths_importance_qkv_x6", "paths_gemm_add_nt_x6", "paths_gather_rows",
            "paths_level0_batch", "paths_tissue_mask_absmax", "paths_synth_grid"):
     SIGNATURES[_n + "_h16"] = SIGNATURES[_n]
 _PLAIN = {"paths_gemm_tn_workspace": (C.c_int64, [_i32, _i32, _i32]), "paths_x6_packed_bytes": (C.c_int64, [_i32, _i32, _i32]), "paths_tlayer_h3_image_bytes": (C.c_int64, [_i32]), "paths_tlayer_ws_image_bytes": (C.c_int64, [_i32, _i32]), "paths_token0_ws_image_bytes": (C.c_int64, []), "paths_token0_ws_partials": (C.c_int64, [_i32, _i32]), "paths_token0_ws_image_bytes_d": (C.c_int64, [_i32]), "paths_token0_ws_partials_d": (C.c_int64, [_i32, _i32, _i32]), "paths_token0_ws_supported": (_i32, [_i32, _i32, _i32, _i32]), "paths_attention_x6_workspace": (C.c_int64, [_i32, _i32, _i32, _i32, _i32]), "paths_attention_fp8_workspace": (C.c_int64, [_i32, _i32, _i32, _i32]), "paths_attention_bwd_x6_workspace": (C.c_int64, [_i32, _i32, _i32, _i32]), "paths_attention_token0_workspace": (C.c_int64, [_i32, _i32, _i32]), "paths_token0_attention_workspace": (C.c_int64, [_i32, _i32, _i32, _i32]), "paths_attention_rollout_workspace": (C.c_int64, [_i32, _i32, _i32, _i32]), "paths_attention_h3_any_workspace": (C.c_int64, [_i32, _i32, _i32, _i32]), "paths_importance_proj_x6_workspace": (C.c_int64, [_i32]), "paths_last_error": (C.c_char_p, []), "paths_build_info": (C.c_char_p, []), "paths_abi_version": (_i32, []), "paths_stop_event_pending": (_i32, []), "paths_clear_stop_event": (_i32, []), "paths_adamw_chunk": (_i32, []), "paths_rank_joint_tile": (_i32, []), "paths_attention_wide_workspace": (C.c_int64, [_i32, _i32]), "paths_event_create": (_vp, []), "paths_stream_create_masked": (_vp, [_vp, _i32])}
diff --git a/paths_amd/csrc/gemm_epi.h b/paths_amd/csrc/gemm_epi.h
--- a/paths_amd/csrc/gemm_epi.h
+++ b/paths_amd/csrc/gemm_epi.h
@@ -39,6 +39,30 @@
   else return trow + c32_row(r, lane) < M;
 }
 
+template <int WTM, int WTN>
+__device__ __forceinline__ void seed_raw(f32x16 (&acc)[WTM][WTN], const float* hp, int hp_bytes, uint32_t ldb, const int* hp_row,
+                                         uint32_t lane_col_bytes, const int (&soff)[WTN], int row0, int lane, int M) {
+  const auto rs = __builtin_amdgcn_make_buffer_rsrc(const_cast<float*>(hp), 0, hp_bytes, 0x00020000);
+  int pr[WTM][16];
+#pragma unroll
+  for (int i = 0; i < WTM; ++i)
+#pragma unroll
+    for (int r = 0; r < 16; ++r) pr[i][r] = hp_row[min(row0 + 32 * i + c32_row(r, lane), M - 1)];
+  __builtin_amdgcn_sched_barrier(0);
+  uint32_t off[WTM][16];
+#pragma unroll
+  for (int i = 0; i < WTM; ++i)
+#pragma unroll
+    for (int r = 0; r < 16; ++r) off[i][r] = pr[i][r] >= 0 ? (uint32_t)pr[i][r] * ldb + lane_col_bytes : 0x80000000u;
+#pragma unroll
+  for (int i = 0; i < WTM; ++i)
+#pragma unroll
+    for (int r = 0; r < 16; ++r)
+#pragma unroll
+      for (int j = 0; j < WTN; ++j)
+        acc[i][j][r] = __builtin_bit_cast(float, __builtin_amdgcn_raw_buffer_load_b32(rs, (int)off[i][r], soff[j], 0));
+}
+
 struct EpiLstmC {
   const float* bias;
   const float* c0; int64_t ldc0;
@@ -46,15 +70,22 @@
   float* frm; int64_t ldfrm;
   const float* hp; int64_t ldhp; const int* hp_row;
   float acc_scale = 1.0f;
+  float hp_seed = 1.0f;
+  int hp_bytes = 0;
   template <int WTM, int WTN>
   __device__ __forceinline__ void init(f32x16 (&acc)[WTM][WTN], int row0, int col0, int lane, int M) const {
     const int jj = lane & 31;
-    const float seed = 1.0f / acc_scale;
+    const float seed = hp_seed;
     if (hp == nullptr) {
 #pragma unroll
       for (int i = 0; i < WTM; ++i)
 #pragma unroll
         for (int r = 0; r < 16; ++r) { acc[i][0][r] = 0.f; acc[i][1][r] = 0.f; acc[i][2][r] = 0.f; }
+      return;
+    }
+    if (hp_bytes > 0) {
+      const int soff[3] = {0, 128, 256};
+      seed_raw(acc, hp, hp_bytes, (uint32_t)ldhp * 4u, hp_row, (uint32_t)(col0 + jj) * 4u, soff, row0, lane, M);
       return;
     }
     int pr[WTM][16];
@@ -91,19 +122,30 @@
     const int tcol = (col0 / 96) * 32;
     const float bf = bias[col0 + jj], br = bias[col0 + 32 + jj], bm = bias[col0 + 64 + jj];
     const TileView c0v(c0, ldc0, lane), c1v(c1, ldc1, lane), fv(frm, ldfrm, lane);
+    constexpr bool AHEAD = !WITH_FRM;
+    float cp[AHEAD ? WTM : 1][16];
+    auto load_c0 = [&](auto ic) __attribute__((always_inline)) {
+      constexpr int i = decltype(ic)::value;
+      const int trow = row0 + 32 * i;
+      char* o0 = c0v.tile(trow, tcol);
+#pragma unroll
+      for (int r = 0; r < 16; ++r) cp[AHEAD ? i : 0][r] = c0 ? *tile_elem_o<FULL>(c0v, o0, trow, tcol, r, lane, M) : 0.f;
+    };
+    if constexpr (AHEAD) {
+      static_for<0, WTM>([&](auto ic) __attribute__((always_inline)) { load_c0(ic); });
+      __builtin_amdgcn_sched_barrier(0);
+    }
     static_for<0, WTM>([&](auto ic) __attribute__((always_inline)) {
       constexpr int i = decltype(ic)::value;
       const int trow = row0 + 32 * i;
-      char* o0 = c0v.tile(trow, tcol); char* o1 = c1v.tile(trow, tcol); char* of = fv.tile(trow, col0);
-      float cp[16];
-#pragma unroll
-      for (int r = 0; r < 16; ++r) cp[r] = c0 ? *tile_elem_o<FULL>(c0v, o0, trow, tcol, r, lane, M) : 0.f;
+      char* o1 = c1v.tile(trow, tcol); char* of = fv.tile(trow, col0);
+      if constexpr (!AHEAD) load_c0(ic);
 #pragma unroll
       for (int r = 0; r < 16; ++r) {
         const float f = sigmoid_acc(fmaf(acc[i][0][r], acc_scale, bf));
         const float rg = sigmoid_acc(fmaf(acc[i][1][r], acc_scale, br));
         const float mp = tanh_acc(fmaf(acc[i][2][r], acc_scale, bm));
-        const float v = cp[r] * f + rg * mp;
+        const float v = cp[AHEAD ? i : 0][r] * f + rg * mp;
         if (tile_row_ok<FULL>(trow, r, lane, M)) {
           *tile_elem_o<FULL>(c1v, o1, trow, tcol, r, lane, M) = v;
           if constexpr (WITH_FRM) {
@@ -129,14 +171,54 @@
   }
 };
 
+struct EpiLstmC0 {
+  const float* bias; float* c1; int64_t ldc1; float acc_scale = 1.0f;
+  template <int WTM, int WTN>
+  __device__ __forceinline__ void init(f32x16 (&acc)[WTM][WTN], int, int, int, int) const {
+#pragma unroll
+    for (int i = 0; i < WTM; ++i)
+#pragma unroll
+      for (int j = 0; j < WTN; ++j)
+#pragma unroll
+        for (int r = 0; r < 16; ++r) acc[i][j][r] = 0.f;
+  }
+  template <bool FULL, int WTM, int WTN>
+  __device__ __forceinline__ void run_impl(f32x16 (&acc)[WTM][WTN], int row0, int col0, int lane, int M) const {
+    const int jj = lane & 31, jb = col0 / 64;
+    const int tcol = jb * 32;
+    const float br = bias[jb * 96 + 32 + jj], bm = bias[jb * 96 + 64 + jj];
+    const TileView c1v(c1, ldc1, lane);
+    static_for<0, WTM>([&](auto ic) __attribute__((always_inline)) {
+      constexpr int i = decltype(ic)::value;
+      const int trow = row0 + 32 * i;
+      char* o1 = c1v.tile(trow, tcol);
+#pragma unroll
+      for (int r = 0; r < 16; ++r) {
+        const float rg = sigmoid_acc(fmaf(acc[i][0][r], acc_scale, br));
+        const float mp = tanh_acc(fmaf(acc[i][1][r], acc_scale, bm));
+        const float v = fmaf(rg, mp, 0.f);
+        if (tile_row_ok<FULL>(trow, r, lane, M)) *tile_elem_o<FULL>(c1v, o1, trow, tcol, r, lane, M) = v;
+      }
+      __builtin_amdgcn_sched_barrier(0);
+    });
+  }
+  template <int WTM, int WTN, int WGM, int WGN>
+  __device__ __forceinline__ void run(f32x16 (&acc)[WTM][WTN], int row0, int col0, int lane, int, int, int M, float*) const {
+    static_assert(WTN == 2, "depth-0 LSTM c epilogue wants r|m tiles");
+    if (row0 + 32 * WTM <= M) run_impl<true>(acc, row0, col0, lane, M);
+    else run_impl<false>(acc, row0, col0, lane, M);
+  }
+};
+
 template <bool RAW>
 struct EpiLstmO_ {
   const float* bias; float* o; int64_t ldo; int N;
   const float* hp; int64_t ldhp; const int* hp_row; int hp_col0;
   float acc_scale = 1.0f;
+  float hp_seed = 1.0f; int hp_bytes = 0;
   template <int WTM, int WTN>
   __device__ __forceinline__ void init(f32x16 (&acc)[WTM][WTN], int row0, int col0, int lane, int M) const {
-    const float seed = 1.0f / acc_scale;
+    const float seed = hp_seed;
     if (hp == nullptr) {
 #pragma unroll
       for (int i = 0; i < WTM; ++i)
@@ -144,6 +226,13 @@
         for (int j = 0; j < WTN; ++j)
 #pragma unroll
           for (int r = 0; r < 16; ++r) acc[i][j][r] = 0.f;
+      return;
+    }
+    if (hp_bytes > 0) {
+      int soff[WTN];
+#pragma unroll
+      for (int j = 0; j < WTN; ++j) soff[j] = (min(col0 + 32 * j, N - 32) - col0) * 4;
+      seed_raw(acc, hp, hp_bytes, (uint32_t)ldhp * 4u, hp_row, (uint32_t)(hp_col0 + col0 + (lane & 31)) * 4u, soff, row0, lane, M);
       return;
     }
     int pr[WTM][16];
diff --git a/paths_amd/csrc/gemm_x6.hip b/paths_amd/csrc/gemm_x6.hip
--- a/paths_amd/csrc/gemm_x6.hip
+++ b/paths_amd/csrc/gemm_x6.hip
@@ -517,8 +517,10 @@
                  const void* w_gates_x6, const float* b_gates, const void* w_mem_x6, const float* b_mem,
                  float* state_out, int64_t ldso, float* y, int64_t ldy, float* ws_o, float* save_frm, float* save_tc,
                  const float* hp, const int* hp_row, int M, int D, int Hc, const int64_t* num_ims, int rows_per_slide,
-                 int phases, int planes, float wg_scale, float wm_scale, float a_scale, hipStream_t stream) {
+                 int phases, int planes, float wg_scale, float wm_scale, float a_scale, const void* w_rm0_x6, int hp_rows, float hp_scale,
+                 hipStream_t stream) {
   PATHS_REQUIRE(D % 256 == 0 && Hc % 64 == 0, "lstm_cell_x6: D (%d) must be a multiple of 256 and Hc (%d) of 64", D, Hc);
+  PATHS_REQUIRE(hp == nullptr || (hp_scale > 0.f && std::isfinite(hp_scale) && hp_rows >= 0), "lstm_cell_x6: hp_scale must be positive and finite, hp_rows >= 0");
   if constexpr (A16) {
     PATHS_REQUIRE(x_rows != nullptr && x == nullptr && planes == 2, "lstm_cell_x6_h16: fp16 rows are given as x_rows (planes = 2)");
     PATHS_REQUIRE(h16_scale_ok(a_scale), "lstm_cell_x6_h16: a_scale must be a power of two in [1, 2^15]");
@@ -532,11 +534,21 @@
   const char* wg = reinterpret_cast<const char*>(w_gates_x6);
   const int64_t gs = group_stride(planes, 2 * D);
   const float sg = 1.0f / (wg_scale * a_scale), sm = 1.0f / (wm_scale * a_scale);
+  const float hp_seed = hp ? 1.0f / (sg * hp_scale) : 1.0f;
+  const int64_t hp_b = (int64_t)hp_rows * (3 * Hc + D) * 4;
+  const int hp_bytes = (hp != nullptr && hp_scale * sg == 1.0f && hp_seed == 1.0f && hp_rows > 0 && hp_b < ((int64_t)1 << 31)) ? (int)hp_b : 0;
   X6Operands g{x, ldx, D, x_rows, h0, h0 ? ldh0 : 0, h0 ? D : 0, nullptr, 0, wg, gs, M, num_ims, rows_per_slide, a_scale};
   const bool small_m = planes == 2 && M <= 8192 && (h0 == nullptr);
   if (phases & 1) {
-    EpiLstmC e{b_gates, c0, ldc0, state_out + D, ldso, save_frm, (int64_t)3 * Hc, hp, (int64_t)3 * Hc + D, hp_row, sg};
+    EpiLstmC e{b_gates, c0, ldc0, state_out + D, ldso, save_frm, (int64_t)3 * Hc, hp, (int64_t)3 * Hc + D, hp_row, sg, hp_seed, hp_bytes};
     int rc;
+    if (!A16 && w_rm0_x6 != nullptr && planes == 2 && x_rows != nullptr && c0 == nullptr && hp == nullptr && h0 == nullptr && save_frm == nullptr) {
+      X6Operands g0 = g;
+      g0.Wt = reinterpret_cast<const char*>(w_rm0_x6); g0.w_group_stride = group_stride(2, D);
+      EpiLstmC0 e0{b_gates, state_out + D, ldso, sg};
+      rc = small_m ? launch_x6_np<2, 2, 2, 2, false, true>(g0, 2 * Hc, e0, stream, "lstm_cell_x6(c, depth 0, 128-row tiles)")
+                   : launch_x6_np<2, 4, 2, 2, false, true>(g0, 2 * Hc, e0, stream, "lstm_cell_x6(c, depth 0)");
+    } else
     if constexpr (A16) {
       rc = small_m ? launch_x6_np<2, 2, 3, 2, false, true, decltype(e), 1, true>(g, 3 * Hc, e, stream, "lstm_cell_x6_h16(c, 128-row tiles)")
                    : launch_x6_np<2, 4, 3, 1, false, true, decltype(e), 1, true>(g, 3 * Hc, e, stream, "lstm_cell_x6_h16(c)");
@@ -551,7 +563,7 @@
     go.Wt = wg + (int64_t)(3 * Hc / 32) * gs;
     int rc;
     if (o_raw) {
-      EpiLstmORaw e{b_gates + 3 * Hc, ws_o, D, D, hp, (int64_t)3 * Hc + D, hp_row, 3 * Hc, sg};
+      EpiLstmORaw e{b_gates + 3 * Hc, ws_o, D, D, hp, (int64_t)3 * Hc + D, hp_row, 3 * Hc, sg, hp_seed, hp_bytes};
       if constexpr (A16) {
         rc = small_m ? launch_x6_np<2, 2, 4, 2, false, true, decltype(e), 1, true>(go, D, e, stream, "lstm_cell_x6_h16(o, raw, 128-row tiles)")
                      : launch_x6_np<2, 4, 4, 1, false, true, decltype(e), 1, true>(go, D, e, stream, "lstm_cell_x6_h16(o, raw)");
@@ -559,7 +571,7 @@
                                : launch_x6_np<2, 2, 4, 2, false, false>(go, D, e, stream, "lstm_cell_x6(o, raw, 128-row tiles)");
       else rc = launch_x6<4, 4, 1, false>(planes, go, D, e, stream, "lstm_cell_x6(o, raw)");
     } else {
-      EpiLstmO e{b_gates + 3 * Hc, ws_o, D, D, hp, (int64_t)3 * Hc + D, hp_row, 3 * Hc, sg};
+      EpiLstmO e{b_gates + 3 * Hc, ws_o, D, D, hp, (int64_t)3 * Hc + D, hp_row, 3 * Hc, sg, hp_seed, hp_bytes};
       if constexpr (A16) rc = launch_x6_np<2, 4, 4, 1, false, true, decltype(e), 1, true>(go, D, e, stream, "lstm_cell_x6_h16(o)");
       else rc = launch_x6<4, 4, 1, false>(planes, go, D, e, stream, "lstm_cell_x6(o)");
     }
@@ -599,7 +611,7 @@
                        const float* hp, const int* hp_row, int M, int D, int Hc, const int64_t* num_ims, int rows_per_slide,
                        int phases, int planes, float wg_scale, float wm_scale, float a_scale, hipStream_t stream) {
   return lstm_cell_x6<false>(x, ldx, x_rows, h0, ldh0, c0, ldc0, w_gates_x6, b_gates, w_mem_x6, b_mem, state_out, ldso, y, ldy, ws_o, save_frm,
-                             save_tc, hp, hp_row, M, D, Hc, num_ims, rows_per_slide, phases, planes, wg_scale, wm_scale, a_scale, stream);
+                             save_tc, hp, hp_row, M, D, Hc, num_ims, rows_per_slide, phases, planes, wg_scale, wm_scale, a_scale, nullptr, 0, 1.0f, stream);
 }
 
 int paths_lstm_cell_x6_h16(const float* x, int64_t ldx, const int64_t* x_rows, const float* h0, int64_t ldh0, const float* c0, int64_t ldc0,
@@ -608,7 +620,29 @@
                            const float* hp, const int* hp_row, int M, int D, int Hc, const int64_t* num_ims, int rows_per_slide,
                            int phases, int planes, float wg_scale, float wm_scale, float a_scale, hipStream_t stream) {
   return lstm_cell_x6<true>(x, ldx, x_rows, h0, ldh0, c0, ldc0, w_gates_x6, b_gates, w_mem_x6, b_mem, state_out, ldso, y, ldy, ws_o, save_frm,
-                            save_tc, hp, hp_row, M, D, Hc, num_ims, rows_per_slide, phases, planes, wg_scale, wm_scale, a_scale, stream);
+                            save_tc, hp, hp_row, M, D, Hc, num_ims, rows_per_slide, phases, planes, wg_scale, wm_scale, a_scale, nullptr, 0, 1.0f, stream);
+}
+
+int paths_lstm_cell_x6_seeded(const float* x, int64_t ldx, const int64_t* x_rows, const float* h0, int64_t ldh0, const float* c0, int64_t ldc0,
+                              const void* w_gates_x6, const float* b_gates, const void* w_mem_x6, const float* b_mem,
+                              float* state_out, int64_t ldso, float* y, int64_t ldy, float* ws_o, float* save_frm, float* save_tc,
+                              const float* hp, const int* hp_row, int M, int D, int Hc, const int64_t* num_ims, int rows_per_slide,
+                              int phases, int planes, float wg_scale, float wm_scale, float a_scale, const void* w_rm0_x6, int hp_rows,
+                              float hp_scale, hipStream_t stream) {
+  return lstm_cell_x6<false>(x, ldx, x_rows, h0, ldh0, c0, ldc0, w_gates_x6, b_gates, w_mem_x6, b_mem, state_out, ldso, y, ldy, ws_o, save_frm,
+                             save_tc, hp, hp_row, M, D, Hc, num_ims, rows_per_slide, phases, planes, wg_scale, wm_scale, a_scale, w_rm0_x6, hp_rows,
+                             hp_scale, stream);
+}
+
+int paths_lstm_cell_x6_seeded_h16(const float* x, int64_t ldx, const int64_t* x_rows, const float* h0, int64_t ldh0, const float* c0, int64_t ldc0,
+                                  const void* w_gates_x6, const float* b_gates, const void* w_mem_x6, const float* b_mem,
+                                  float* state_out, int64_t ldso, float* y, int64_t ldy, float* ws_o, float* save_frm, float* save_tc,
+                                  const float* hp, const int* hp_row, int M, int D, int Hc, const int64_t* num_ims, int rows_per_slide,
+                                  int phases, int planes, float wg_scale, float wm_scale, float a_scale, const void* w_rm0_x6, int hp_rows,
+                                  float hp_scale, hipStream_t stream) {
+  return lstm_cell_x6<true>(x, ldx, x_rows, h0, ldh0, c0, ldc0, w_gates_x6, b_gates, w_mem_x6, b_mem, state_out, ldso, y, ldy, ws_o, save_frm,
+                            save_tc, hp, hp_row, M, D, Hc, num_ims, rows_per_slide, phases, planes, wg_scale, wm_scale, a_scale, w_rm0_x6, hp_rows,
+                            hp_scale, stream);
 }
 
 #endif
@@ -805,6 +839,16 @@
   return launch_x6<2, 4, 2, false>(planes, g, Npad, e, stream, "gemm_rows_nt_x6");
 }
 
+int paths_gemm_rows_nt_x6_raw(const int64_t* a_rows, const void* w_x6, int Kpacked, int k0, float* out, int64_t ldo,
+                              int M, int Npad, int K, int planes, float w_scale, float a_scale, hipStream_t stream) {
+  PATHS_REQUIRE(a_rows != nullptr && planes == 2 && pow2(w_scale) && pow2(a_scale), "gemm_rows_nt_x6_raw: row addresses need planes = 2 with power-of-two scales");
+  PATHS_REQUIRE(k0 % 16 == 0 && k0 >= 0 && k0 + K <= Kpacked, "gemm_rows_nt_x6_raw: bad k window");
+  X6Operands g{nullptr, K, K, a_rows, nullptr, 0, 0, nullptr, 0,
+               reinterpret_cast<const char*>(w_x6) + (int64_t)(k0 / 16) * planes * FRAG, group_stride(planes, Kpacked), M, nullptr, 0, a_scale};
+  EpiBias e{nullptr, out, ldo, Npad, 0, nullptr, 0, nullptr, 0, 0, 1.0f};
+  return launch_x6<2, 4, 2, false>(planes, g, Npad, e, stream, "gemm_rows_nt_x6_raw");
+}
+
 int paths_gemm_add_nt_x6(const float* a, int64_t lda, const int64_t* a_rows, const float* a_add, int64_t ld_add, const void* w_x6, int Kpacked,
                          const float* b, float* out, int64_t ldo, int M, int N, int Npad, int K, int act, const int64_t* num_ims,
                          int rows_per_slide, float w_scale, float a_scale, hipStream_t stream) {
diff --git a/paths_amd/ops.py b/paths_amd/ops.py
--- a/paths_amd/ops.py
+++ b/paths_amd/ops.py
@@ -14,6 +14,8 @@
 TLAYER_WS = os.environ.get("PATHS_TLAYER_WS", "1") != "0"
 SPLITK_IMPORTANCE = os.environ.get("PATHS_SPLITK_IMPORTANCE", "1") != "0"
 FUSE_QKV = int(os.environ.get("PATHS_FUSE_QKV", "2"))
+RAW_PARTIALS = os.environ.get("PATHS_RAW_PARTIALS", "1") != "0"
+DEPTH0_RM = os.environ.get("PATHS_DEPTH0_RM", "1") != "0"
 KERNEL_TIMER = None
 TIMER_ALL = False
 
@@ -183,6 +185,17 @@
         ws = _pow2_scale_lagged(pack[key], pack["_owner"], key) if (lagged and planes == 2) else None
         pack[k6] = x6_pack(pack[key], planes=planes, w_scale=ws)
     return pack[k6]
+
+
+def rm0_rows(w_gates: torch.Tensor, Hc: int, D: int) -> torch.Tensor:
+    return w_gates[:3 * Hc].view(Hc // 32, 3, 32, -1)[:, 1:, :, :D].reshape(2 * Hc, D).contiguous()
+
+
+def _rm0_of(lstm_pack: Dict[str, object], D: int):
+    wg, wg_s = _x6_of(lstm_pack, "w_gates", 2)
+    if "w_rm0_split2" not in lstm_pack:
+        lstm_pack["w_rm0_split2"] = x6_pack(rm0_rows(lstm_pack["w_gates"], lstm_pack["Hc"], D), planes=2, w_scale=wg_s)[0]
+    return lstm_pack["w_rm0_split2"]
 
 
 def pe_table(lvl_pack: Dict[str, object], pe_mode: int, d: int, rows: int) -> torch.Tensor:
@@ -923,7 +936,11 @@
         assert state_prev is None
         c0t = parent["c0"]
         assert c0t.shape == (B, N, Hc) and c0t.is_contiguous()
-        return Hc, None, c0t.data_ptr(), _lib.ptr(hp), _lib.ptr(parent["hp_row"])
+        base = (Hc, None, c0t.data_ptr(), _lib.ptr(hp), _lib.ptr(parent["hp_row"]))
+        if "hp_scale" in parent:
+            assert hp.dim() == 2 and hp.is_contiguous() and hp.shape[1] == 3 * Hc + D
+            return base + (hp.shape[0], float(parent["hp_scale"]))
+        return base
     if state_prev is not None:
         assert state_prev.shape[:2] == (B, N) and state_prev.shape[2] == D + Hc and state_prev.stride(2) == 1
         assert state_prev.stride(0) == N * state_prev.stride(1), "state rows must be uniformly strided"
@@ -934,16 +951,23 @@
 def lstm_cell(lstm_pack, fts, x_rows, prev, state_out, y, o, frm, tc, N: int, num_ims, phases: int, planes: int = 0, lagged: bool = False,
               h16: str = ""):
     p = _lib.ptr
-    ld, h0, c0, hp, hp_row = prev
+    ld, h0, c0, hp, hp_row = prev[:5]
+    hp_rows, hp_scale = prev[5:] if len(prev) > 5 else (0, 1.0)
     Dp = state_out.shape[2]
     Hc = lstm_pack["Hc"]
     D = Dp - Hc
     M = state_out.shape[0] * N
     if planes:
         (wg, wg_s), (wm, wm_s) = _x6_of(lstm_pack, "w_gates", planes, lagged=lagged), _x6_of(lstm_pack, "w_mem", planes, lagged=lagged)
-        _lib.call("paths_lstm_cell_x6" + h16, p(fts), D, p(x_rows), h0, ld, c0, ld, p(wg), p(lstm_pack["b_gates"]), p(wm), p(lstm_pack["b_mem"]),
-                  p(state_out), Dp, p(y), D, p(o), p(frm), p(tc), hp, hp_row, M, D, Hc, p(num_ims), N, phases,
-                  planes, wg_s, wm_s, A_SCALE if planes == 2 else 1.0, _lib.stream())
+        args = (p(fts), D, p(x_rows), h0, ld, c0, ld, p(wg), p(lstm_pack["b_gates"]), p(wm), p(lstm_pack["b_mem"]),
+                p(state_out), Dp, p(y), D, p(o), p(frm), p(tc), hp, hp_row, M, D, Hc, p(num_ims), N, phases,
+                planes, wg_s, wm_s, A_SCALE if planes == 2 else 1.0)
+        depth0 = (DEPTH0_RM and planes == 2 and not lagged and not h16 and x_rows is not None and hp is None and h0 is None and c0 is None
+                  and frm is None and not torch.is_grad_enabled())
+        if depth0 or len(prev) > 5:
+            _lib.call("paths_lstm_cell_x6_seeded" + h16, *args, p(_rm0_of(lstm_pack, D)) if depth0 else None, hp_rows, hp_scale, _lib.stream())
+        else:
+            _lib.call("paths_lstm_cell_x6" + h16, *args, _lib.stream())
     else:
         _lib.call("paths_lstm_cell", p(fts), D, h0, ld, c0, ld, p(lstm_pack["w_gates"]), p(lstm_pack["b_gates"]),
                   p(lstm_pack["w_mem"]), p(lstm_pack["b_mem"]), p(state_out), Dp, p(y), D,
@@ -964,7 +988,7 @@
 
 
 def parent_partials(lstm_pack, state_out: torch.Tensor, keep_idx: torch.Tensor, keep_count: torch.Tensor,
-                    kept_rows: Optional[torch.Tensor] = None) -> torch.Tensor:
+                    kept_rows: Optional[torch.Tensor] = None, raw: bool = False):
     B, N, Dp = state_out.shape
     Hc = lstm_pack["Hc"]
     D = Dp - Hc
@@ -977,8 +1001,10 @@
     if kept_rows is not None:
         assert use_x6(D, Hc) and G % 256 == 0 and split_planes() == 2 and kept_rows.shape == (B, cap) and kept_rows.dtype == torch.int64
         wg, wg_s = _x6_of(lstm_pack, "w_gates")
-        timed("parent_gemm", lambda: _lib.call("paths_gemm_rows_nt_x6", p(kept_rows), p(wg), 2 * D, D, p(hp), G, B * cap, G, D, 2, wg_s, a_scale(), st))
-        return hp
+        timed("parent_gemm", lambda: _lib.call("paths_gemm_rows_nt_x6_raw" if raw else "paths_gemm_rows_nt_x6", p(kept_rows), p(wg), 2 * D, D, p(hp), G,
+                                               B * cap, G, D, 2, wg_s, a_scale(), st))
+        return (hp, wg_s * a_scale()) if raw else hp
+    assert not raw, "raw partials come from the row-addressed parent GEMM"
     hk = torch.empty((B * cap, D), **f32)
     _lib.call("paths_gather_kept_rows", p(state_out), N, Dp, p(keep_idx), cap, p(keep_count), D, B, p(hk), st)
     parent_gate_product(lstm_pack, hk, hp, planes=split_planes() if use_x6(D, Hc) else 0)
diff --git a/paths_amd/utils.py b/paths_amd/utils.py
--- a/paths_amd/utils.py
+++ b/paths_amd/utils.py
@@ -468,7 +468,12 @@
                                                 p(keep_count), p(out["ctx_patch"]), Dp, N, p(kept_rows), p(r.zero_row), st))
         else:
             _lib.call("paths_topk", p(out["importance"]), N, p(lv.num_ims), B, N, keep, p(keep_idx), cap_keep, p(keep_count), st)
-    hp = ops.parent_partials(r.lstm_pack, out["ctx_patch"], keep_idx, keep_count, kept_rows) if share_parent else None
+    raw_hp = bool(share_parent and rows_in_place and ops.RAW_PARTIALS and not torch.is_grad_enabled())
+    hp = hp_scale = None
+    if raw_hp:
+        hp, hp_scale = ops.parent_partials(r.lstm_pack, out["ctx_patch"], keep_idx, keep_count, kept_rows, raw=True)
+    elif share_parent:
+        hp = ops.parent_partials(r.lstm_pack, out["ctx_patch"], keep_idx, keep_count, kept_rows)
     st2 = r.par_stream.cuda_stream if forked else st
     nx = SimpleNamespace(fts=None, x_rows=None, staged=None, state_prev=None, parent=None)
     with (torch.cuda.stream(r.par_stream) if forked else contextlib.nullcontext()):
@@ -493,6 +498,8 @@
                 _lib.call("paths_gather_rows" + r.sfx, grid, p(src_cell), D, out["ctx_patch"].data_ptr() + 4 * D, N, Dp,
                           p(src_row), Hc, p(num_next), B, Nn, p(nx.fts), p(c0), 0, None, None, st2)
             nx.parent = {"hp": hp, "hp_row": hp_row, "c0": c0}
+            if hp_scale is not None:
+                nx.parent["hp_scale"] = hp_scale
         else:
             nx.fts = torch.empty((B, Nn, D), **r.f32)
             nx.state_prev = torch.empty((B, Nn, Dp), **r.f32)
```

Result: no change. 3992 slides/s, median of 6 (+0.9%).
